# Enigmatisms/NeRF

Hardware: AMD Instinct MI355X
Metric: rays/s (64+128 samples), 800x800 (higher is better)
Workload: dtype bf16

## Files before the change

include/nerf_amd.h:

```cpp
#ifndef NERF_AMD_H
#define NERF_AMD_H

#include <stddef.h>
#include <stdint.h>

#ifdef __cplusplus
extern "C" {
#endif

#define NERF_AMD_OK            0
#define NERF_AMD_EINVAL       -1
#define NERF_AMD_EUNSUPPORTED -2
#define NERF_AMD_EHIP         -3

#define NERF_AMD_F32   0
#define NERF_AMD_BF16  1
#define NERF_AMD_BF16_F8 2

#define NERF_AMD_NET_PROPOSAL 0
#define NERF_AMD_NET_MIP      1
#define NERF_AMD_NET_REF      2
#define NERF_AMD_NET_PROPOSAL_128 3
#define NERF_AMD_PROP_W128 0x100
#define NERF_AMD_NET_MIP_128 4
#define NERF_AMD_FINE_W128 0x200

#define NERF_AMD_ACT_RELU     0
#define NERF_AMD_ACT_IDENTITY 1
#define NERF_AMD_ACT_SOFTPLUS 2

const char* nerf_amd_last_error(void);
int         nerf_amd_version(void);
int         nerf_amd_device_info(int* n_cu, int* arch_is_gfx950);

typedef struct nerf_amd_samples {
    int32_t      mode;
    int32_t      S;
    int64_t      M;
    const float* pts;
    int32_t      pts_stride;
    int32_t      z_stride;
    const float* rays;
    const float* z;
    const float* z_base;
    const float* u;
    float        z_jitter;
    int32_t      H, W;
    float        fx, fy;
    float        pose[12];
    int32_t      contract;
    int32_t      ipe;
    float        ipe_radius;
    const float* ipe_dir_norm;
    uint64_t     rng_seed;
    int64_t      rng_ray_offset;
} nerf_amd_samples;

size_t nerf_amd_packed_bytes(int net, int precision);
int    nerf_amd_pack_weights(int net, int precision, const float* const* weights, const float* const* biases,
                             int n_tensors, void* packed, void* stream);

int nerf_amd_proposal_forward(const void* packed, int precision, const nerf_amd_samples* src,
                              float* density, void* stream);
int nerf_amd_mip_forward(const void* packed, int precision, const nerf_amd_samples* src,
                         float* rgbo, void* stream);

int nerf_amd_mip_forward_composite(const void* packed, int precision, const nerf_amd_samples* src, int white_bkg,
                                   float near, float far, float* rgb, float* depth, float* weights, void* stream);

#define NERF_AMD_REF_SRGB 1
int nerf_amd_ref_forward(const void* packed, int precision, const nerf_amd_samples* src, int ref_flags,
                         float* rgbo, float* normal, void* stream);
int nerf_amd_ref_forward_train(const void* packed, int precision, const nerf_amd_samples* src, int ref_flags, const float* bn_noise,
                               float* rgbo, float* normal, void* stream);


int nerf_amd_positional_encoding(const float* x, int64_t M, int L, float* out, void* stream);

int nerf_amd_ipe_feature(const float* z, const float* rays, int64_t N, int S, int L, float r, const float* dir_norm,
                         float* feat, float* mu, float* mu_t, void* stream);
int nerf_amd_ipe_feature_contracted(const float* z, const float* rays, int64_t N, int S, int L, float r, const float* dir_norm,
                                    float* feat, float* mu, float* mu_t, void* stream);
int nerf_amd_cone_parameters(const float* z, int64_t N, int S, float r, float* mu_t, float* var_t, float* var_r, void* stream);
int nerf_amd_dirs_norm(const float* rays, int64_t N, float* out, void* stream);

int nerf_amd_generate_rays(const float* pose_host, int H, int W, float fx, float fy, int64_t ray_offset, int64_t N,
                           float* rays, void* stream);

int nerf_amd_length2pts(const float* rays, const float* z, int64_t N, int S, float* out, void* stream);

int nerf_amd_sigma_to_weights(const float* sigma, const float* z, const float* dirs, int64_t N, int S, int act,
                              float* w, void* stream);

int nerf_amd_max_blur(const float* w, int64_t N, int S, float alpha, float* out, void* stream);

int nerf_amd_inverse_sample(const float* w, const float* z, const float* u, int64_t N, int C, int K, int sort,
                            float* z_out, int64_t* below, void* stream);

int nerf_amd_sample_pdf(const float* bins, const float* weights, const float* u, int64_t N, int B, int K, float* samples,
                        int64_t* below, int64_t* above, void* stream);

int nerf_amd_pixel_rays(const float* pose_host, float fx, float fy, const int64_t* coords, int64_t N, float* rays, void* stream);

int nerf_amd_sample_training_rays(const float* rgbs, const int64_t* coords, int64_t n_pixels, const float* pose_host, float fx, float fy,
                                  float near, float far, int64_t N, int C, uint64_t rng_seed, float* pts, float* lengths, float* rgb,
                                  float* rays, void* stream);
int nerf_amd_sample_training_rays_dev(const float* rgbs, const int64_t* coords, int64_t n_pixels, const float* pose_dev, float fx, float fy,
                                      float near, float far, int64_t N, int C, const uint64_t* seed_dev, float* pts, float* lengths,
                                      float* rgb, float* rays, void* stream);
int nerf_amd_philox_uniforms(float* out, int64_t N, int K, uint64_t rng_seed, const uint64_t* seed_dev, void* stream);
#define NERF_AMD_PHILOX_INV 0
#define NERF_AMD_PHILOX_STRAT 1
int nerf_amd_philox_stream(float* out, int64_t N, int K, uint64_t rng_seed, const uint64_t* seed_dev, int64_t ray_offset, int stream_id,
                           void* stream);
int nerf_amd_advance_seed(uint64_t* seed_dev, void* stream);

int nerf_amd_stratified_points(const float* rays, const float* z_base, const float* u, float z_jitter, int64_t N, int S,
                               float* z_out, float* pts, void* stream);

int nerf_amd_resample(const float* density, const float* z, const float* z_base, const float* u_strat, float z_jitter,
                      const float* dirs, int dirs_stride, const float* u_inv, int64_t N, int C, int K,
                      int softplus_density, float blur_alpha, uint64_t rng_seed, int64_t rng_ray_offset,
                      float* z_fine, int64_t* below, float* w_prop, float* z_coarse, void* stream);

int nerf_amd_composite(const float* rgbo, const float* z, int z_stride, const float* dirs, int dirs_stride,
                       int64_t N, int S, int flags, int act, float sigma_shift, float near, float far,
                       const float* normal, const float* cam_dir,
                       float* rgb, float* weights, float* depth, float* normal_img, void* stream);

int nerf_amd_merge_depths(const float* z_fine, const float* z_coarse, int64_t N, int K, int C, float* z_out, void* stream);

int nerf_amd_merge_depths_order(const float* z_fine, const float* z_coarse, const int64_t* f_inds, int64_t N, int K, int C, float* z_out,
                                int64_t* order, int64_t* all_inds, void* stream);

int nerf_amd_coarse_grad_select(const float* grads, const int64_t* sort_inds, int64_t N, int T, int D, int c_pnum, float* out, void* stream);

#define NERF_AMD_DOT_LOSS_WORKSPACE_FLOATS 512
int nerf_amd_weighted_dot_loss(const float* w, const float* a, const float* b, int64_t M, int mode, float scale, float* out, float* workspace, void* stream);
int nerf_amd_weighted_dot_loss_backward(const float* g, const float* w, const float* a, const float* b, int64_t M, int mode, float scale, float* d_w,
                                        float* d_a, float* d_b, void* stream);

#define NERF_AMD_DISTORTION_MAX_S 1024
#define NERF_AMD_DISTORTION_WORKSPACE_FLOATS 4096
int nerf_amd_distortion_loss(const float* w, const float* t, int64_t N, int S, int mode, float scale, float* out, float* workspace, void* stream);
int nerf_amd_distortion_loss_backward(const float* w, const float* t, int64_t N, int S, int mode, float scale, const float* g, float* d_w,
                                      float* d_t, void* stream);

int nerf_amd_mfma_stream(int iters, int workgroups, int mode, float* sink, void* stream);

int nerf_amd_get_bounds(const float* w_prop, const int64_t* below, int64_t N, int C, int K, float* bounds, void* stream);

size_t nerf_amd_train_dump_bytes(int net, int precision, int64_t M);
int nerf_amd_proposal_forward_train(const void* packed, int precision, const nerf_amd_samples* src, float* density, void* dump,
                                    void* stream);
int nerf_amd_mip_forward_train(const void* packed, int precision, const nerf_amd_samples* src, float* rgbo, void* dump, void* stream);
int nerf_amd_train_dump_to_rows(const void* dump, int net, int precision, int64_t M, int layer, int n_features, void* out,
                                void* stream);
int nerf_amd_relu_mask(void* delta, const void* act, int precision, int64_t n, void* stream);
int64_t nerf_amd_relu_mask_bias_partials(int precision, int64_t rows, int cols);
int nerf_amd_relu_mask_bias(void* delta, const void* act, int precision, int64_t rows, int cols, float* col_sum, void* stream);

int64_t nerf_amd_train_dump_rows_mask_partials(void);
int nerf_amd_train_dump_rows_mask(const void* dump, int net, int precision, int64_t M, int layer, int n_features, void* act_out, void* delta,
                                  float* col_sum, void* stream);

int nerf_amd_encode_rows(const float* x, int x_stride, int64_t M, int L, int normalize, int precision, void* out, void* stream);

size_t nerf_amd_packed_backward_bytes(int net, int precision);
int    nerf_amd_pack_weights_backward(int net, int precision, const float* const* weights, int n_tensors, void* packed_bwd, void* stream);
int    nerf_amd_proposal_backward_chain(const void* packed_bwd, int precision, const float* g_density, int64_t M, const void* act_dump,
                                        void* delta_dump, void* stream);
int    nerf_amd_mip_backward_chain(const void* packed_bwd, int precision, const float* g_rgbo, const float* rgbo, int64_t M,
                                   const void* act_dump, void* delta_dump, void* stream);
size_t nerf_amd_weight_grads_workspace_bytes(int net, int precision, int64_t M);
int    nerf_amd_proposal_weight_grads(int precision, int64_t M, const void* act_dump, const void* delta_dump, float* const* d_weights,
                                      float* const* d_biases, void* workspace, void* stream);
int    nerf_amd_mip_weight_grads(int precision, int64_t M, const void* act_dump, const void* delta_dump, const float* const* weights,
                                 const float* const* biases, float* const* d_weights, float* const* d_biases, void* workspace, void* stream);
int    nerf_amd_ref_forward_train_dump(const void* packed, int precision, const nerf_amd_samples* src, int ref_flags, const float* bn_noise,
                                       float* rgbo, float* normal, void* dump, float* aux, void* stream);
int    nerf_amd_ref_forward_train_dump_rng(const void* packed, int precision, const nerf_amd_samples* src, int ref_flags, uint64_t noise_seed,
                                           const uint64_t* noise_seed_dev, float noise_std, float* rgbo, float* normal, void* dump, float* aux,
                                           void* stream);
int    nerf_amd_philox_normal(float* out, int64_t M, uint64_t rng_seed, const uint64_t* seed_dev, float std, int64_t sample_offset, void* stream);
#define NERF_AMD_CONTRACTED 0x100
size_t nerf_amd_density_grad_workspace_bytes(int net, int precision, int64_t M);
int    nerf_amd_density_grad(int net, const void* packed_bwd, int precision, int64_t M, const void* act_dump, const float* x, int x_stride,
                             const float* scale, int scale_stride, float* grad, void* workspace, void* stream);
size_t nerf_amd_ref_backward_workspace_bytes(int precision, int64_t M);
int    nerf_amd_ref_backward(const void* packed_bwd, int precision, int ref_flags, int64_t M, const void* act_dump, const float* aux,
                             const float* dirs, int dir_stride, const float* g_out, int g_stride, const float* ide_table,
                             float* const* d_weights, float* const* d_biases, void* workspace, void* stream);
int    nerf_amd_adam_step(float* const* params, const float* const* grads, float* const* exp_avg, float* const* exp_avg_sq,
                          const int64_t* numel, int n_tensors, float* step, double lr, const double* lr_dev, double beta1, double beta2,
                          double eps, float grad_scale, void* stream);

int nerf_amd_sigma_to_weights_backward(const float* sigma, const float* z, const float* dirs, int64_t N, int S, int act,
                                       const float* d_weights, float* d_sigma, void* stream);
int nerf_amd_composite_backward(const float* rgbo, const float* z, int z_stride, const float* dirs, int dirs_stride, int64_t N, int S,
                                int flags, int act, float sigma_shift, float near, float far, const float* d_rgb,
                                const float* d_weights, const float* d_depth, float* d_rgbo, void* stream);
int nerf_amd_max_blur_backward(const float* weights, const float* d_out, int64_t N, int S, float* d_weights, void* stream);
int nerf_amd_get_bounds_backward(const int64_t* below, const float* d_bounds, int64_t N, int C, int K, float* d_w_prop, void* stream);

size_t nerf_amd_render_workspace_bytes(int64_t N, int n_fine);
int    nerf_amd_render_rays(const void* packed_prop, const void* packed_mip, int precision,
                            const float* rays, const nerf_amd_samples* camera, int64_t ray_offset,
                            const float* z_base, const float* u_strat, const float* u_inv, int64_t N, int n_fine,
                            float near, float far, int white_bkg,
                            float* rgb, float* depth, float* weights, void* workspace, void* stream);

size_t nerf_amd_render_ref_workspace_bytes(int64_t N, int n_fine);
int    nerf_amd_render_rays_ref(const void* packed_prop, const void* packed_ref, int precision, int ref_flags, const float* rays,
                                const nerf_amd_samples* camera, int64_t ray_offset, const float* z_base, const float* u_strat,
                                const float* u_inv, int64_t N, int n_fine, float near, float far, int white_bkg, const float* cam_dir,
                                float* rgb, float* depth, float* normal_img, void* workspace, void* stream);

size_t nerf_amd_gemm_workspace_bytes(int64_t M, int64_t N, int64_t P);
// ... 31 lines not shown
```

nerf_amd/_lib.py:

```python
import ctypes as C
import os

import torch

_HERE = os.path.dirname(os.path.abspath(__file__))
LIB_PATH = os.environ.get("NERF_AMD_LIB") or os.path.join(_HERE, "libnerf_amd.so")

F32, BF16 = 0, 1
BF16_F8 = 2
EXPECTED_VERSION = 125
NET_PROPOSAL, NET_MIP, NET_REF, NET_PROPOSAL_128, NET_MIP_128 = 0, 1, 2, 3, 4
FINE_W128 = 0x200
PROP_W128 = 0x100
ACT_RELU, ACT_IDENTITY, ACT_SOFTPLUS = 0, 1, 2

c_float_p = C.POINTER(C.c_float)
c_void = C.c_void_p
i64 = C.c_int64


class Samples(C.Structure):
    _fields_ = [("mode", C.c_int32), ("S", C.c_int32), ("M", C.c_int64), ("pts", c_void), ("pts_stride", C.c_int32),
                ("z_stride", C.c_int32), ("rays", c_void), ("z", c_void), ("z_base", c_void), ("u", c_void),
                ("z_jitter", C.c_float), ("H", C.c_int32), ("W", C.c_int32), ("fx", C.c_float), ("fy", C.c_float),
                ("pose", C.c_float * 12), ("contract", C.c_int32), ("ipe", C.c_int32), ("ipe_radius", C.c_float),
                ("ipe_dir_norm", c_void), ("rng_seed", C.c_uint64), ("rng_ray_offset", C.c_int64)]


SIGNATURES = {
    "nerf_amd_last_error": (C.c_char_p, []),
    "nerf_amd_version": (C.c_int, []),
    "nerf_amd_device_info": (C.c_int, [C.POINTER(C.c_int), C.POINTER(C.c_int)]),
    "nerf_amd_packed_bytes": (C.c_size_t, [C.c_int, C.c_int]),
    "nerf_amd_pack_weights": (C.c_int, [C.c_int, C.c_int, C.POINTER(c_void), C.POINTER(c_void), C.c_int, c_void, c_void]),
    "nerf_amd_proposal_forward": (C.c_int, [c_void, C.c_int, C.POINTER(Samples), c_void, c_void]),
    "nerf_amd_mip_forward": (C.c_int, [c_void, C.c_int, C.POINTER(Samples), c_void, c_void]),
    "nerf_amd_mip_forward_composite": (C.c_int, [c_void, C.c_int, C.POINTER(Samples), C.c_int, C.c_float, C.c_float, c_void, c_void, c_void,
                                                 c_void]),
    "nerf_amd_ref_forward": (C.c_int, [c_void, C.c_int, C.POINTER(Samples), C.c_int, c_void, c_void, c_void]),
    "nerf_amd_ref_forward_train": (C.c_int, [c_void, C.c_int, C.POINTER(Samples), C.c_int, c_void, c_void, c_void, c_void]),
    "nerf_amd_positional_encoding": (C.c_int, [c_void, i64, C.c_int, c_void, c_void]),
    "nerf_amd_ipe_feature": (C.c_int, [c_void, c_void, i64, C.c_int, C.c_int, C.c_float, c_void, c_void, c_void, c_void, c_void]),
    "nerf_amd_ipe_feature_contracted": (C.c_int, [c_void, c_void, i64, C.c_int, C.c_int, C.c_float, c_void, c_void, c_void, c_void, c_void]),
    "nerf_amd_cone_parameters": (C.c_int, [c_void, i64, C.c_int, C.c_float, c_void, c_void, c_void, c_void]),
    "nerf_amd_dirs_norm": (C.c_int, [c_void, i64, c_void, c_void]),
    "nerf_amd_generate_rays": (C.c_int, [c_float_p, C.c_int, C.c_int, C.c_float, C.c_float, i64, i64, c_void, c_void]),
    "nerf_amd_length2pts": (C.c_int, [c_void, c_void, i64, C.c_int, c_void, c_void]),
    "nerf_amd_sigma_to_weights": (C.c_int, [c_void, c_void, c_void, i64, C.c_int, C.c_int, c_void, c_void]),
    "nerf_amd_max_blur": (C.c_int, [c_void, i64, C.c_int, C.c_float, c_void, c_void]),
    "nerf_amd_inverse_sample": (C.c_int, [c_void, c_void, c_void, i64, C.c_int, C.c_int, C.c_int, c_void, c_void, c_void]),
    "nerf_amd_sample_pdf": (C.c_int, [c_void, c_void, c_void, i64, C.c_int, C.c_int, c_void, c_void, c_void, c_void]),
    "nerf_amd_pixel_rays": (C.c_int, [c_float_p, C.c_float, C.c_float, c_void, i64, c_void, c_void]),
    "nerf_amd_sample_training_rays": (C.c_int, [c_void, c_void, i64, c_float_p, C.c_float, C.c_float, C.c_float, C.c_float, i64, C.c_int, C.c_uint64,
                                               c_void, c_void, c_void, c_void, c_void]),
    "nerf_amd_sample_training_rays_dev": (C.c_int, [c_void, c_void, i64, c_void, C.c_float, C.c_float, C.c_float, C.c_float, i64, C.c_int, c_void,
                                                   c_void, c_void, c_void, c_void, c_void]),
    "nerf_amd_philox_uniforms": (C.c_int, [c_void, i64, C.c_int, C.c_uint64, c_void, c_void]),
    "nerf_amd_philox_stream": (C.c_int, [c_void, i64, C.c_int, C.c_uint64, c_void, i64, C.c_int, c_void]),
    "nerf_amd_advance_seed": (C.c_int, [c_void, c_void]),
    "nerf_amd_stratified_points": (C.c_int, [c_void, c_void, c_void, C.c_float, i64, C.c_int, c_void, c_void, c_void]),
    "nerf_amd_resample": (C.c_int, [c_void, c_void, c_void, c_void, C.c_float, c_void, C.c_int, c_void, i64, C.c_int,
                                    C.c_int, C.c_int, C.c_float, C.c_uint64, i64, c_void, c_void, c_void, c_void, c_void]),
    "nerf_amd_composite": (C.c_int, [c_void, c_void, C.c_int, c_void, C.c_int, i64, C.c_int, C.c_int, C.c_int, C.c_float, C.c_float,
                                     C.c_float, c_void, c_void, c_void, c_void, c_void, c_void, c_void]),
    "nerf_amd_train_dump_rows_mask_partials": (i64, []),
    "nerf_amd_train_dump_rows_mask": (C.c_int, [c_void, C.c_int, C.c_int, i64, C.c_int, C.c_int, c_void, c_void, c_void, c_void]),
    "nerf_amd_render_ref_workspace_bytes": (C.c_size_t, [i64, C.c_int]),
    "nerf_amd_render_rays_ref": (C.c_int, [c_void, c_void, C.c_int, C.c_int, c_void, C.POINTER(Samples), i64, c_void, c_void, c_void, i64, C.c_int,
                                          C.c_float, C.c_float, C.c_int, c_void, c_void, c_void, c_void, c_void, c_void]),
    "nerf_amd_encode_rows": (C.c_int, [c_void, C.c_int, i64, C.c_int, C.c_int, C.c_int, c_void, c_void]),
    "nerf_amd_merge_depths": (C.c_int, [c_void, c_void, i64, C.c_int, C.c_int, c_void, c_void]),
    "nerf_amd_merge_depths_order": (C.c_int, [c_void, c_void, c_void, i64, C.c_int, C.c_int, c_void, c_void, c_void, c_void]),
    "nerf_amd_coarse_grad_select": (C.c_int, [c_void, c_void, i64, C.c_int, C.c_int, C.c_int, c_void, c_void]),
    "nerf_amd_mfma_stream": (C.c_int, [C.c_int, C.c_int, C.c_int, c_void, c_void]),
    "nerf_amd_weighted_dot_loss": (C.c_int, [c_void, c_void, c_void, i64, C.c_int, C.c_float, c_void, c_void, c_void]),
    "nerf_amd_weighted_dot_loss_backward": (C.c_int, [c_void, c_void, c_void, c_void, i64, C.c_int, C.c_float, c_void, c_void, c_void, c_void]),
    "nerf_amd_distortion_loss": (C.c_int, [c_void, c_void, i64, C.c_int, C.c_int, C.c_float, c_void, c_void, c_void]),
    "nerf_amd_distortion_loss_backward": (C.c_int, [c_void, c_void, i64, C.c_int, C.c_int, C.c_float, c_void, c_void, c_void, c_void]),
    "nerf_amd_get_bounds": (C.c_int, [c_void, c_void, i64, C.c_int, C.c_int, c_void, c_void]),
    "nerf_amd_train_dump_bytes": (C.c_size_t, [C.c_int, C.c_int, i64]),
    "nerf_amd_proposal_forward_train": (C.c_int, [c_void, C.c_int, C.POINTER(Samples), c_void, c_void, c_void]),
    "nerf_amd_mip_forward_train": (C.c_int, [c_void, C.c_int, C.POINTER(Samples), c_void, c_void, c_void]),
    "nerf_amd_train_dump_to_rows": (C.c_int, [c_void, C.c_int, C.c_int, i64, C.c_int, C.c_int, c_void, c_void]),
    "nerf_amd_relu_mask": (C.c_int, [c_void, c_void, C.c_int, i64, c_void]),
    "nerf_amd_relu_mask_bias_partials": (i64, [C.c_int, i64, C.c_int]),
    "nerf_amd_relu_mask_bias": (C.c_int, [c_void, c_void, C.c_int, i64, C.c_int, c_void, c_void]),
    "nerf_amd_packed_backward_bytes": (C.c_size_t, [C.c_int, C.c_int]),
    "nerf_amd_pack_weights_backward": (C.c_int, [C.c_int, C.c_int, C.POINTER(c_void), C.c_int, c_void, c_void]),
    "nerf_amd_proposal_backward_chain": (C.c_int, [c_void, C.c_int, c_void, i64, c_void, c_void, c_void]),
    "nerf_amd_mip_backward_chain": (C.c_int, [c_void, C.c_int, c_void, c_void, i64, c_void, c_void, c_void]),
    "nerf_amd_weight_grads_workspace_bytes": (C.c_size_t, [C.c_int, C.c_int, i64]),
    "nerf_amd_proposal_weight_grads": (C.c_int, [C.c_int, i64, c_void, c_void, C.POINTER(c_void), C.POINTER(c_void), c_void, c_void]),
    "nerf_amd_mip_weight_grads": (C.c_int, [C.c_int, i64, c_void, c_void, C.POINTER(c_void), C.POINTER(c_void), C.POINTER(c_void),
                                           C.POINTER(c_void), c_void, c_void]),
    "nerf_amd_ref_forward_train_dump": (C.c_int, [c_void, C.c_int, C.POINTER(Samples), C.c_int, c_void, c_void, c_void, c_void, c_void, c_void]),
    "nerf_amd_ref_forward_train_dump_rng": (C.c_int, [c_void, C.c_int, C.POINTER(Samples), C.c_int, C.c_uint64, c_void, C.c_float, c_void, c_void, c_void,
                                                      c_void, c_void]),
    "nerf_amd_philox_normal": (C.c_int, [c_void, i64, C.c_uint64, c_void, C.c_float, i64, c_void]),
    "nerf_amd_density_grad_workspace_bytes": (C.c_size_t, [C.c_int, C.c_int, i64]),
    "nerf_amd_density_grad": (C.c_int, [C.c_int, c_void, C.c_int, i64, c_void, c_void, C.c_int, c_void, C.c_int, c_void, c_void, c_void]),
    "nerf_amd_ref_backward_workspace_bytes": (C.c_size_t, [C.c_int, i64]),
    "nerf_amd_ref_backward": (C.c_int, [c_void, C.c_int, C.c_int, i64, c_void, c_void, c_void, C.c_int, c_void, C.c_int, c_void, C.POINTER(c_void),
                                       C.POINTER(c_void), c_void, c_void]),
    "nerf_amd_adam_step": (C.c_int, [C.POINTER(c_void), C.POINTER(c_void), C.POINTER(c_void), C.POINTER(c_void), C.POINTER(i64), C.c_int, c_void,
                                    C.c_double, c_void, C.c_double, C.c_double, C.c_double, C.c_float, c_void]),
    "nerf_amd_sigma_to_weights_backward": (C.c_int, [c_void, c_void, c_void, i64, C.c_int, C.c_int, c_void, c_void, c_void]),
    "nerf_amd_composite_backward": (C.c_int, [c_void, c_void, C.c_int, c_void, C.c_int, i64, C.c_int, C.c_int, C.c_int, C.c_float, C.c_float,
                                              C.c_float, c_void, c_void, c_void, c_void, c_void]),
    "nerf_amd_max_blur_backward": (C.c_int, [c_void, c_void, i64, C.c_int, c_void, c_void]),
    "nerf_amd_get_bounds_backward": (C.c_int, [c_void, c_void, i64, C.c_int, C.c_int, c_void, c_void]),
    "nerf_amd_render_workspace_bytes": (C.c_size_t, [i64, C.c_int]),
    "nerf_amd_render_rays": (C.c_int, [c_void, c_void, C.c_int, c_void, C.POINTER(Samples), i64, c_void, c_void, c_void, i64,
                                       C.c_int, C.c_float, C.c_float, C.c_int, c_void, c_void, c_void, c_void, c_void]),
    "nerf_amd_gemm_workspace_bytes": (C.c_size_t, [i64, i64, i64]),
    "nerf_amd_gemm": (C.c_int, [C.c_int, i64, i64, i64, c_void, i64, i64, c_void, i64, i64, c_void, i64, c_void, C.c_int, c_void, i64, c_void, c_void]),
    "nerf_amd_sigmoid_backward": (C.c_int, [c_void, i64, c_void, i64, i64, C.c_int, c_void, i64, c_void]),
    "nerf_amd_ref_dir_inputs": (C.c_int, [c_void, i64, c_void, i64, i64, C.c_int, c_void, c_void, i64, c_void, c_void]),
    "nerf_amd_ref_dir_inputs_backward": (C.c_int, [c_void, i64, c_void, i64, i64, C.c_int, c_void, c_void, i64, c_void, i64, c_void, i64, c_void]),
    "nerf_amd_ref_combine": (C.c_int, [c_void, i64, c_void, i64, i64, C.c_int, c_void, c_void]),
    "nerf_amd_ref_combine_backward": (C.c_int, [c_void, i64, c_void, i64, c_void, i64, i64, C.c_int, c_void, i64, c_void, i64, c_void]),
    "nerf_amd_positional_encoding_backward": (C.c_int, [c_void, i64, c_void, i64, i64, C.c_int, C.c_int, c_void, c_void]),
    "nerf_amd_contract_positions": (C.c_int, [c_void, i64, i64, c_void, i64, c_void, c_void]),
    "nerf_amd_add_rows": (C.c_int, [c_void, i64, c_void, i64, i64, C.c_int, c_void]),
    "nerf_amd_rows_gemm": (C.c_int, [i64, i64, i64, c_void, i64, c_void, i64, i64, c_void, C.c_int, c_void, i64, C.c_int, c_void]),
    "nerf_amd_rows_to_bf16": (C.c_int, [c_void, i64, i64, i64, C.c_int, C.c_int, c_void, i64, c_void]),
}


def _load():
    if not os.path.exists(LIB_PATH):
        raise ImportError(
            "nerf_amd: %s is missing. Build it with `python -c 'import __graft_entry__ as g; g.build()'` "
            "(or `make -C nerf_amd/csrc`). There is no CPU/torch fallback." % LIB_PATH)
    lib = C.CDLL(LIB_PATH)
    for name, (res, args) in SIGNATURES.items():
        fn = getattr(lib, name)
        fn.restype = res
        fn.argtypes = args
    got = lib.nerf_amd_version()
    if got != EXPECTED_VERSION and not os.environ.get("NERF_AMD_LIB"):
        raise ImportError("nerf_amd: %s is ABI version %d, this package expects %d -- rebuild it (`make -C nerf_amd/csrc`)" % (LIB_PATH, got, EXPECTED_VERSION))
    return lib


lib = _load()


class NerfAmdError(RuntimeError):
    pass


def check(rc: int, what: str = ""):
    if rc != 0:
        msg = lib.nerf_amd_last_error()
        raise NerfAmdError("%s failed (%d): %s" % (what or "nerf_amd call", rc, msg.decode() if msg else "?"))
```

nerf_amd/csrc/capi.hip:

```cpp
#include <hip/hip_runtime.h>
#include <stdio.h>
#include <string.h>

#include "../../include/nerf_amd.h"
#include "mlp_layout.h"

int mlp_launch_proposal(const void*, int, const nerf_amd_samples&, float*, hipStream_t);
int mlp_launch_proposal128(const void*, int, const nerf_amd_samples&, float*, hipStream_t);
int mlp_launch_mip(const void*, int, const nerf_amd_samples&, float*, hipStream_t);
int mlp_launch_mip128(const void*, int, const nerf_amd_samples&, float*, hipStream_t);
int mlp_launch_mip_composite(const void*, int, const nerf_amd_samples&, float*, float*, float*, int, float, float, hipStream_t);
int mlp_launch_ref(const void*, int, const nerf_amd_samples&, float*, float*, const float*, int, hipStream_t);
size_t mlp_train_layer_stride(int, int64_t);
size_t mlp_train_mask_stride(int, int64_t);
int mlp_launch_proposal_train(const void*, int, const nerf_amd_samples&, float*, void*, hipStream_t);
int mlp_launch_mip_train(const void*, int, const nerf_amd_samples&, float*, void*, hipStream_t);
int sk_frag_to_rows(const void*, int, int64_t, int, int64_t, void*, hipStream_t);
int sk_relu_mask(void*, const void*, int, int64_t, hipStream_t);
int sk_merge_sorted(const float*, const float*, int64_t, int, int, float*, hipStream_t);
int sk_merge_sorted_order(const float*, const float*, const int64_t*, int64_t, int, int, float*, int64_t*, int64_t*, hipStream_t);
int sk_coarse_grad_select(const float*, const int64_t*, int64_t, int, int, int, float*, hipStream_t);
int pack_mfma_stream(int, int, int, float*, hipStream_t);
int sk_weighted_dot_loss(const float*, const float*, const float*, int64_t, int, float, float*, float*, hipStream_t);
int sk_weighted_dot_loss_backward(const float*, const float*, const float*, const float*, int64_t, int, float, float*, float*, float*, hipStream_t);
int sk_distortion_loss(const float*, const float*, int64_t, int, int, float, float*, float*, hipStream_t);
int sk_distortion_loss_backward(const float*, const float*, int64_t, int, int, float, const float*, float*, float*, hipStream_t);
int sk_encode_rows(const float*, int, int64_t, int, int, int, void*, hipStream_t);
int sk_frag_rows_mask_blocks();
int sk_frag_rows_mask(const void*, int, int64_t, int, int64_t, void*, void*, float*, hipStream_t);
int sk_relu_mask_bias(void*, const void*, int, int64_t, int, float*, hipStream_t);
int pack_ref(int, const float* const*, const float* const*, void*, hipStream_t);
int pack_proposal_bwd(int, const float* const*, void*, hipStream_t);
int pack_mip_bwd(int, const float* const*, void*, hipStream_t);
int pack_ref_bwd(int, const float* const*, void*, hipStream_t);
int mlp_launch_ref_train(const void*, int, const nerf_amd_samples&, float*, float*, const float*, void*, float*, int, hipStream_t, unsigned long long, const unsigned long long*, float);
size_t bwd_density_grad_workspace_bytes(int, int64_t);
int bwd_density_grad(int, const void*, int, int64_t, const void*, const float*, int, const float*, int, float*, void*, hipStream_t, int);
size_t bwd_ref_workspace_bytes(int, int64_t);
int bwd_ref_backward(const void*, int, int64_t, const void*, const float*, const float*, int, const float*, int, const float*, float* const*,
                     float* const*, void*, int, hipStream_t);
int bwd_launch_prop_chain(const void*, int, const float*, int64_t, const void*, void*, hipStream_t);
int bwd_launch_mip_chain(const void*, int, const float*, const float*, int64_t, const void*, void*, hipStream_t);
size_t bwd_wgrad_workspace_bytes(int, int, int64_t);
int bwd_prop_weight_grads(int, int64_t, const void*, const void*, float* const*, float* const*, void*, hipStream_t);
int bwd_mip_weight_grads(int, int64_t, const void*, const void*, const float* const*, const float* const*, float* const*, float* const*, void*,
                         hipStream_t);
int bwd_launch_adam(float* const*, const float* const*, float* const*, float* const*, const long long*, int, float*, double, const double*, double,
                    double, double, float, hipStream_t);
int pack_proposal(int, const float* const*, const float* const*, void*, hipStream_t);
int pack_proposal128(int, const float* const*, const float* const*, void*, hipStream_t);
int pack_mip128(int, const float* const*, const float* const*, void*, hipStream_t);
int pack_mip(int, const float* const*, const float* const*, void*, hipStream_t);
int sk_positional_encoding(const float*, int64_t, int, float*, hipStream_t);
int sk_ipe_feature(const float*, const float*, int64_t, int, int, float, const float*, float*, float*, float*, int, hipStream_t);
int sk_dirs_norm(const float*, int64_t, float*, hipStream_t);
int sk_dirs_norm_scratch(const float*, int64_t, float*, void*, hipStream_t);
int sk_train_sampler(const float*, const int64_t*, int64_t, const float*, const float*, float, float, float, float, int64_t, int, uint64_t, const uint64_t*,
                     float*, float*, float*, float*, hipStream_t);
int sk_philox_uniforms(float*, int64_t, int, uint64_t, const uint64_t*, int64_t, int, hipStream_t);
int sk_philox_normal(float*, int64_t, uint64_t, const uint64_t*, float, int64_t, hipStream_t);
size_t gk_gemm_workspace_bytes(int64_t, int64_t, int64_t);
int gk_gemm(int, int64_t, int64_t, int64_t, const float*, int64_t, int64_t, const float*, int64_t, int64_t, float*, int64_t, const float*, int, const float*, int64_t,
            void*, hipStream_t);
int gk_sigmoid_backward(const float*, int64_t, const float*, int64_t, int64_t, int, float*, int64_t, hipStream_t);
int gr_dir_inputs(const float*, int64_t, const float*, int64_t, int64_t, int, const float*, float*, int64_t, float*, hipStream_t);
int gr_dir_inputs_backward(const float*, int64_t, const float*, int64_t, int64_t, int, const float*, const float*, int64_t, const float*, int64_t, float*, int64_t,
                           hipStream_t);
int gr_combine(const float*, int64_t, const float*, int64_t, int64_t, int, float*, hipStream_t);
int gr_combine_backward(const float*, int64_t, const float*, int64_t, const float*, int64_t, int64_t, int, float*, int64_t, float*, int64_t, hipStream_t);
int gr_pe_backward(const float*, int64_t, const float*, int64_t, int64_t, int, int, float*, hipStream_t);
int gr_add_rows(float*, int64_t, const float*, int64_t, int64_t, int, hipStream_t);
int gr_contract(const float*, int64_t, int64_t, const float*, int64_t, float*, hipStream_t);
int rg_rows_gemm(int64_t, int64_t, int64_t, const void*, int64_t, const void*, int64_t, int64_t, const float*, int, void*, int64_t, int, hipStream_t);
int rg_rows_to_bf16(const float*, int64_t, int64_t, int64_t, int, int, void*, int64_t, hipStream_t);
int sk_advance_seed(uint64_t*, hipStream_t);
int sk_cone_parameters(const float*, int64_t, int, float, float*, float*, float*, hipStream_t);
int sk_generate_rays(const float*, int, int, float, float, int64_t, int64_t, float*, hipStream_t);
int sk_length2pts(const float*, const float*, int64_t, int, float*, hipStream_t);
int sk_sigma_to_weights(const float*, const float*, const float*, int64_t, int, int, float*, hipStream_t);
int sk_max_blur(const float*, int64_t, int, float, float*, hipStream_t);
int sk_inverse_sample(const float*, const float*, const float*, int64_t, int, int, int, int, float*, int64_t*, int64_t*, hipStream_t);
int sk_pixel_rays(const float*, float, float, const int64_t*, int64_t, float*, hipStream_t);
int sk_stratified_points(const float*, const float*, const float*, float, int64_t, int, float*, float*, hipStream_t);
int sk_resample(const float*, const float*, const float*, const float*, float, const float*, int, const float*, int64_t, int,
                int, int, float, uint64_t, int64_t, float*, int64_t*, float*, float*, hipStream_t);
int sk_composite(const float*, const float*, int, const float*, int, int64_t, int, int, int, float, float, float, const float*,
                 const float*, float*, float*, float*, float*, hipStream_t);
int sk_get_bounds(const float*, const int64_t*, int64_t, int, int, float*, hipStream_t);
int sk_weights_backward(const float*, int, int, const float*, int, const float*, int, int64_t, int, int, int, float, const float*, const float*,
                        const float*, const float*, int, float, float, float*, int, int, float*, hipStream_t);
int sk_max_blur_backward(const float*, const float*, int64_t, int, float*, hipStream_t);
int sk_get_bounds_backward(const int64_t*, const float*, int64_t, int, int, float*, hipStream_t);

namespace {
thread_local char g_err[512] = "";

int fail(int code, const char* fmt, const char* a = "") {
    snprintf(g_err, sizeof(g_err), fmt, a);
    return code;
}
int hip_status(int e, const char* where) {
    if (e == 0) return NERF_AMD_OK;
    snprintf(g_err, sizeof(g_err), "%s: HIP error %d (%s)", where, e, hipGetErrorString((hipError_t)e));
    return NERF_AMD_EHIP;
}
inline hipStream_t S(void* s) { return reinterpret_cast<hipStream_t>(s); }

int check_samples(const nerf_amd_samples* s, bool need_dir) {
    if (!s) return fail(NERF_AMD_EINVAL, "samples descriptor is NULL");
    if (s->M < 0) return fail(NERF_AMD_EINVAL, "negative sample count");
    if (s->mode == 0) {
        if (!s->pts && s->M) return fail(NERF_AMD_EINVAL, "mode 0 needs pts");
        if (s->pts_stride < (need_dir ? 6 : 3)) return fail(NERF_AMD_EINVAL, "pts_stride too small for this network");
    } else if (s->mode == 1 || s->mode == 2) {
        if (s->S <= 0) return fail(NERF_AMD_EINVAL, "S must be positive");
        if (s->mode == 1 && !s->rays && s->M) return fail(NERF_AMD_EINVAL, "mode 1 needs rays");
        if (s->mode == 2 && (s->H <= 0 || s->W <= 0)) return fail(NERF_AMD_EINVAL, "mode 2 needs H, W");
        if (!s->z && !s->z_base && s->M) return fail(NERF_AMD_EINVAL, "need z, or z_base (with u, or without: in-kernel uniforms from rng_seed)");
    } else {
        return fail(NERF_AMD_EINVAL, "unknown sample mode");
    }
    if (s->ipe) {
        if (!need_dir) return fail(NERF_AMD_EUNSUPPORTED, "integrated PE is wired for the MipNeRF kernel only");
        if (s->mode != 1 || !s->z || s->z_stride < s->S + 1) return fail(NERF_AMD_EINVAL, "integrated PE needs mode 1 with S+1 depths per ray (z, z_stride > S)");
        if (!s->ipe_dir_norm || !(s->ipe_radius > 0.0f)) return fail(NERF_AMD_EINVAL, "integrated PE needs ipe_dir_norm (device) and a positive ipe_radius");
    }
    return NERF_AMD_OK;
}
bool bad_prec(int p) { return p != NERF_AMD_F32 && p != NERF_AMD_BF16; }
int check_distortion(int64_t N, int Sn, int mode) {
    if (N < 0) return fail(NERF_AMD_EINVAL, "negative ray count");
    if (mode != 0 && mode != 1) return fail(NERF_AMD_EINVAL, "unknown mode (0: Regularizer, 1: Mip-NeRF 360 L_dist)");
    if (Sn < 2 || Sn > NERF_AMD_DISTORTION_MAX_S) return fail(NERF_AMD_EINVAL, "bad size (S must be 2..1024 depths per row: a ray's rows live in LDS)");
    return NERF_AMD_OK;
}
}

extern "C" {

const char* nerf_amd_last_error(void) { return g_err; }
int nerf_amd_version(void) { return 125; }

int nerf_amd_device_info(int* n_cu, int* arch_is_gfx950) {
    int dev = 0;
    hipDeviceProp_t p;
    int e = (int)hipGetDevice(&dev);
    if (!e) e = (int)hipGetDeviceProperties(&p, dev);
    if (e) return hip_status(e, "nerf_amd_device_info");
    if (n_cu) *n_cu = p.multiProcessorCount;
    if (arch_is_gfx950) *arch_is_gfx950 = strncmp(p.gcnArchName, "gfx950", 6) == 0;
    return NERF_AMD_OK;
}

size_t nerf_amd_packed_bytes(int net, int precision) {
    if (bad_prec(precision)) return 0;
    if (net == NERF_AMD_NET_PROPOSAL) return PropLayout::packed_bytes(precision);
    if (net == NERF_AMD_NET_MIP) return MipLayout::packed_bytes(precision);
    if (net == NERF_AMD_NET_REF) return RefLayout::packed_bytes(precision);
    if (net == NERF_AMD_NET_PROPOSAL_128) return PropLayout128::packed_bytes(precision);
    if (net == NERF_AMD_NET_MIP_128) return MipLayout128::packed_bytes(precision);
    return 0;
}
static int launch_mip_any(int flags, const void* packed, int precision, const nerf_amd_samples& s, float* rgbo, hipStream_t st) {
    return (flags & NERF_AMD_FINE_W128) ? mlp_launch_mip128(packed, precision, s, rgbo, st) : mlp_launch_mip(packed, precision, s, rgbo, st);
}
static int launch_proposal_any(int flags, const void* packed, int precision, const nerf_amd_samples& s, float* density, hipStream_t st) {
    return (flags & NERF_AMD_PROP_W128) ? mlp_launch_proposal128(packed, precision, s, density, st) : mlp_launch_proposal(packed, precision, s, density, st);
}

int nerf_amd_pack_weights(int net, int precision, const float* const* weights, const float* const* biases, int n_tensors,
                          void* packed, void* stream) {
    if (bad_prec(precision)) return fail(NERF_AMD_EINVAL, "unknown precision");
    if (!weights || !biases || !packed) return fail(NERF_AMD_EINVAL, "NULL argument");
    const int want = (net == NERF_AMD_NET_PROPOSAL || net == NERF_AMD_NET_PROPOSAL_128) ? 5
                     : ((net == NERF_AMD_NET_MIP || net == NERF_AMD_NET_MIP_128) ? 11 : (net == NERF_AMD_NET_REF ? 20 : -1));
    if (want < 0) return fail(NERF_AMD_EINVAL, "unknown network");
    if (n_tensors != want) return fail(NERF_AMD_EINVAL, "wrong number of weight tensors for this network");
    for (int i = 0; i < want; ++i)
        if (!weights[i] || !biases[i]) return fail(NERF_AMD_EINVAL, "NULL weight or bias tensor");
    const int e = net == NERF_AMD_NET_PROPOSAL ? pack_proposal(precision, weights, biases, packed, S(stream))
                  : net == NERF_AMD_NET_PROPOSAL_128 ? pack_proposal128(precision, weights, biases, packed, S(stream))
                  : net == NERF_AMD_NET_MIP_128 ? pack_mip128(precision, weights, biases, packed, S(stream))
                  : (net == NERF_AMD_NET_MIP ? pack_mip(precision, weights, biases, packed, S(stream))
                                             : pack_ref(precision, weights, biases, packed, S(stream)));
    return hip_status(e, "nerf_amd_pack_weights");
}

int nerf_amd_proposal_forward(const void* packed, int precision, const nerf_amd_samples* src, float* density, void* stream) {
    const int lflags = precision & ~0xff;
    precision &= 0xff;
    if (bad_prec(precision) || (lflags & ~NERF_AMD_PROP_W128)) return fail(NERF_AMD_EINVAL, "unknown precision");
    if (int c = check_samples(src, false)) return c;
    if (src->M == 0) return NERF_AMD_OK;
    if (!packed || !density) return fail(NERF_AMD_EINVAL, "NULL argument");
    return hip_status(launch_proposal_any(lflags, packed, precision, *src, density, S(stream)), "nerf_amd_proposal_forward");
}

int nerf_amd_mip_forward(const void* packed, int precision, const nerf_amd_samples* src, float* rgbo, void* stream) {
    const int lflags = precision & ~0xff;
    precision &= 0xff;
    if (bad_prec(precision) || (lflags & ~NERF_AMD_FINE_W128)) return fail(NERF_AMD_EINVAL, "unknown precision");
    if (int c = check_samples(src, true)) return c;
    if (src->M == 0) return NERF_AMD_OK;
    if (!packed || !rgbo) return fail(NERF_AMD_EINVAL, "NULL argument");
    if ((lflags & NERF_AMD_FINE_W128) && src->ipe) return fail(NERF_AMD_EINVAL, "the 128-wide fine layout has no integrated-PE kernel: pack the network 256-wide");
    return hip_status(launch_mip_any(lflags, packed, precision, *src, rgbo, S(stream)), "nerf_amd_mip_forward");
}

int nerf_amd_mip_forward_composite(const void* packed, int precision, const nerf_amd_samples* src, int white_bkg, float near,
                                   float far, float* rgb, float* depth, float* weights, void* stream) {
    const int lflags = precision & ~0xff;
    precision &= 0xff;
    if (bad_prec(precision) || (lflags & ~NERF_AMD_FINE_W128)) return fail(NERF_AMD_EINVAL, "unknown precision");
    if (lflags & NERF_AMD_FINE_W128)
        return fail(NERF_AMD_EUNSUPPORTED, "the 128-wide fine layout has no fused-compositing kernel: use nerf_amd_mip_forward + nerf_amd_composite");
    if (int c = check_samples(src, true)) return c;
    if (src->mode != 1 || !src->z) return fail(NERF_AMD_EUNSUPPORTED, "fused compositing needs mode 1 (rays + z)");
    if (src->ipe) return fail(NERF_AMD_EUNSUPPORTED, "integrated PE: use nerf_amd_mip_forward + nerf_amd_composite");
    if (src->S != 32 && src->S != 64 && src->S != 128) return fail(NERF_AMD_EUNSUPPORTED, "fused compositing needs S in {32, 64, 128}");
    if (src->M == 0) return NERF_AMD_OK;
    if (!packed || !rgb) return fail(NERF_AMD_EINVAL, "NULL argument");
    return hip_status(mlp_launch_mip_composite(packed, precision, *src, rgb, depth, weights, white_bkg, near, far, S(stream)),
                      "nerf_amd_mip_forward_composite");
}

static bool bad_ref_flags(int f) { return (f & ~NERF_AMD_REF_SRGB) != 0; }
int nerf_amd_ref_forward(const void* packed, int precision, const nerf_amd_samples* src, int ref_flags, float* rgbo, float* normal, void* stream) {
    if (bad_prec(precision) || bad_ref_flags(ref_flags)) return fail(NERF_AMD_EINVAL, "unknown precision or ref_flags");
    if (int c = check_samples(src, true)) return c;
    if (src->M == 0) return NERF_AMD_OK;
    if (!packed || !rgbo) return fail(NERF_AMD_EINVAL, "NULL argument");
    return hip_status(mlp_launch_ref(packed, precision, *src, rgbo, normal, nullptr, ref_flags, S(stream)), "nerf_amd_ref_forward");
}
int nerf_amd_ref_forward_train(const void* packed, int precision, const nerf_amd_samples* src, int ref_flags, const float* bn_noise, float* rgbo,
                               float* normal, void* stream) {
    if (bad_prec(precision) || bad_ref_flags(ref_flags)) return fail(NERF_AMD_EINVAL, "unknown precision or ref_flags");
    if (int c = check_samples(src, true)) return c;
    if (src->M == 0) return NERF_AMD_OK;
    if (!packed || !rgbo || !bn_noise) return fail(NERF_AMD_EINVAL, "NULL argument");
    return hip_status(mlp_launch_ref(packed, precision, *src, rgbo, normal, bn_noise, ref_flags, S(stream)), "nerf_amd_ref_forward_train");
}

int nerf_amd_positional_encoding(const float* x, int64_t M, int L, float* out, void* stream) {
    if (M < 0 || L < 1 || L > 24) return fail(NERF_AMD_EINVAL, "bad M or L");
    if (M && (!x || !out)) return fail(NERF_AMD_EINVAL, "NULL argument");
    return hip_status(sk_positional_encoding(x, M, L, out, S(stream)), "nerf_amd_positional_encoding");
}

int nerf_amd_ipe_feature(const float* z, const float* rays, int64_t N, int Sn, int L, float r, const float* dir_norm, float* feat, float* mu,
                         float* mu_t, void* stream) {
    if (N < 0 || Sn < 0 || L < 1 || L > 15) return fail(NERF_AMD_EINVAL, "bad size or L (1..15)");
    if (N * Sn && (!z || !rays || !dir_norm || !feat)) return fail(NERF_AMD_EINVAL, "NULL argument");
    const float r2 = (float)((double)r * (double)r);
    return hip_status(sk_ipe_feature(z, rays, N, Sn, L, r2, dir_norm, feat, mu, mu_t, 0, S(stream)), "nerf_amd_ipe_feature");
}
int nerf_amd_ipe_feature_contracted(const float* z, const float* rays, int64_t N, int Sn, int L, float r, const float* dir_norm, float* feat, float* mu,
                                    float* mu_t, void* stream) {
    if (N < 0 || Sn < 0 || L < 1 || L > 15) return fail(NERF_AMD_EINVAL, "bad size or L (1..15)");
    if (N * Sn && (!z || !rays || !dir_norm || !feat)) return fail(NERF_AMD_EINVAL, "NULL argument");
    const float r2 = (float)((double)r * (double)r);
    return hip_status(sk_ipe_feature(z, rays, N, Sn, L, r2, dir_norm, feat, mu, mu_t, 1, S(stream)), "nerf_amd_ipe_feature_contracted");
}
int nerf_amd_cone_parameters(const float* z, int64_t N, int Sn, float r, float* mu_t, float* var_t, float* var_r, void* stream) {
    if (N < 0 || Sn < 0) return fail(NERF_AMD_EINVAL, "negative size");
    if (N * Sn && (!z || !mu_t || !var_t || !var_r)) return fail(NERF_AMD_EINVAL, "NULL argument");
    return hip_status(sk_cone_parameters(z, N, Sn, (float)((double)r * (double)r), mu_t, var_t, var_r, S(stream)), "nerf_amd_cone_parameters");
}
int nerf_amd_dirs_norm(const float* rays, int64_t N, float* out, void* stream) {
    if (N < 0 || !out || (N && !rays)) return fail(NERF_AMD_EINVAL, "bad argument");
    return hip_status(sk_dirs_norm(rays, N, out, S(stream)), "nerf_amd_dirs_norm");
}

int nerf_amd_generate_rays(const float* pose_host, int H, int W, float fx, float fy, int64_t ray_offset, int64_t N, float* rays,
                           void* stream) {
    if (!pose_host || !rays || H <= 0 || W <= 0) return fail(NERF_AMD_EINVAL, "bad argument");
    if (ray_offset < 0 || N < 0 || ray_offset + N > (int64_t)H * W) return fail(NERF_AMD_EINVAL, "ray range outside the image");
    return hip_status(sk_generate_rays(pose_host, H, W, fx, fy, ray_offset, N, rays, S(stream)), "nerf_amd_generate_rays");
}

int nerf_amd_length2pts(const float* rays, const float* z, int64_t N, int Sn, float* out, void* stream) {
    if (N < 0 || Sn < 0) return fail(NERF_AMD_EINVAL, "negative size");
    if (N * Sn && (!rays || !z || !out)) return fail(NERF_AMD_EINVAL, "NULL argument");
    return hip_status(sk_length2pts(rays, z, N, Sn, out, S(stream)), "nerf_amd_length2pts");
}

int nerf_amd_sigma_to_weights(const float* sigma, const float* z, const float* dirs, int64_t N, int Sn, int act, float* w,
                              void* stream) {
    if (N < 0 || Sn < 0 || act < 0 || act > 2) return fail(NERF_AMD_EINVAL, "bad size or activation");
    if (N * Sn && (!sigma || !z || !w)) return fail(NERF_AMD_EINVAL, "NULL argument");
    return hip_status(sk_sigma_to_weights(sigma, z, dirs, N, Sn, act, w, S(stream)), "nerf_amd_sigma_to_weights");
}

int nerf_amd_max_blur(const float* w, int64_t N, int Sn, float alpha, float* out, void* stream) {
    if (N < 0 || Sn < 0) return fail(NERF_AMD_EINVAL, "negative size");
    if (N * Sn && (!w || !out)) return fail(NERF_AMD_EINVAL, "NULL argument");
    return hip_status(sk_max_blur(w, N, Sn, alpha, out, S(stream)), "nerf_amd_max_blur");
}

int nerf_amd_inverse_sample(const float* w, const float* z, const float* u, int64_t N, int C, int K, int sort, float* z_out,
                            int64_t* below, void* stream) {
    if (N < 0 || C < 3 || C > 256 || K < 1 || K > 1024) return fail(NERF_AMD_EINVAL, "need 3 <= C <= 256 and 1 <= K <= 1024");
    if (N && (!w || !z || !u || !z_out)) return fail(NERF_AMD_EINVAL, "NULL argument");
    return hip_status(sk_inverse_sample(w, z, u, N, C, K, sort, 0, z_out, below, nullptr, S(stream)), "nerf_amd_inverse_sample");
}

int nerf_amd_sample_pdf(const float* bins, const float* weights, const float* u, int64_t N, int B, int K, float* samples,
                        int64_t* below, int64_t* above, void* stream) {
    if (N < 0 || B < 2 || B > 256 || K < 1 || K > 1024) return fail(NERF_AMD_EINVAL, "need 2 <= B <= 256 and 1 <= K <= 1024");
    if (N && (!bins || !weights || !u || !samples)) return fail(NERF_AMD_EINVAL, "NULL argument");
    return hip_status(sk_inverse_sample(weights, bins, u, N, B, K, 0, 1, samples, below, above, S(stream)), "nerf_amd_sample_pdf");
}

int nerf_amd_pixel_rays(const float* pose_host, float fx, float fy, const int64_t* coords, int64_t N, float* rays, void* stream) {
    if (!pose_host || N < 0 || (N && (!coords || !rays))) return fail(NERF_AMD_EINVAL, "bad argument");
    return hip_status(sk_pixel_rays(pose_host, fx, fy, coords, N, rays, S(stream)), "nerf_amd_pixel_rays");
}

int nerf_amd_sample_training_rays(const float* rgbs, const int64_t* coords, int64_t n_pixels, const float* pose_host, float fx, float fy,
                                  float near, float far, int64_t N, int C, uint64_t rng_seed, float* pts, float* lengths, float* rgb, float* rays,
                                  void* stream) {
    if (N < 0 || C < 0 || n_pixels < 1) return fail(NERF_AMD_EINVAL, "bad size");
    if (!pose_host || (N && (!rgbs || !coords || !rgb || !rays))) return fail(NERF_AMD_EINVAL, "NULL argument");
    if ((pts == nullptr) != (lengths == nullptr) || (pts && C < 1)) return fail(NERF_AMD_EINVAL, "pts and lengths go together (C >= 1)");
    return hip_status(sk_train_sampler(rgbs, coords, n_pixels, pose_host, nullptr, fx, fy, near, far, N, C, rng_seed, nullptr, pts, lengths, rgb, rays, S(stream)),
                      "nerf_amd_sample_training_rays");
}
int nerf_amd_sample_training_rays_dev(const float* rgbs, const int64_t* coords, int64_t n_pixels, const float* pose_dev, float fx, float fy,
                                      float near, float far, int64_t N, int C, const uint64_t* seed_dev, float* pts, float* lengths, float* rgb,
                                      float* rays, void* stream) {
    if (N < 0 || C < 0 || n_pixels < 1) return fail(NERF_AMD_EINVAL, "bad size");
    if (!pose_dev || !seed_dev || (N && (!rgbs || !coords || !rgb || !rays))) return fail(NERF_AMD_EINVAL, "NULL argument");
    if ((pts == nullptr) != (lengths == nullptr) || (pts && C < 1)) return fail(NERF_AMD_EINVAL, "pts and lengths go together (C >= 1)");
    return hip_status(sk_train_sampler(rgbs, coords, n_pixels, nullptr, pose_dev, fx, fy, near, far, N, C, 0, seed_dev, pts, lengths, rgb, rays, S(stream)),
                      "nerf_amd_sample_training_rays_dev");
}
int nerf_amd_philox_uniforms(float* out, int64_t N, int K, uint64_t rng_seed, const uint64_t* seed_dev, void* stream) {
    if (N < 0 || K < 0) return fail(NERF_AMD_EINVAL, "negative size");
    if (N * K && !out) return fail(NERF_AMD_EINVAL, "NULL argument");
    return hip_status(sk_philox_uniforms(out, N, K, rng_seed, seed_dev, 0, 0, S(stream)), "nerf_amd_philox_uniforms");
}
int nerf_amd_philox_stream(float* out, int64_t N, int K, uint64_t rng_seed, const uint64_t* seed_dev, int64_t ray_offset, int stream_id, void* stream) {
    if (N < 0 || K < 0 || ray_offset < 0) return fail(NERF_AMD_EINVAL, "negative size");
    if (stream_id != NERF_AMD_PHILOX_INV && stream_id != NERF_AMD_PHILOX_STRAT) return fail(NERF_AMD_EINVAL, "unknown stream_id");
    if (stream_id == NERF_AMD_PHILOX_STRAT && K > 64) return fail(NERF_AMD_EINVAL, "the stratified stream has 64 slots per ray");
    if (N * K && !out) return fail(NERF_AMD_EINVAL, "NULL argument");
    return hip_status(sk_philox_uniforms(out, N, K, rng_seed, seed_dev, ray_offset, stream_id == NERF_AMD_PHILOX_STRAT, S(stream)), "nerf_amd_philox_stream");
}
int nerf_amd_advance_seed(uint64_t* seed_dev, void* stream) {
    if (!seed_dev) return fail(NERF_AMD_EINVAL, "NULL argument");
    return hip_status(sk_advance_seed(seed_dev, S(stream)), "nerf_amd_advance_seed");
}

int nerf_amd_stratified_points(const float* rays, const float* z_base, const float* u, float z_jitter, int64_t N, int Sn,
                               float* z_out, float* pts, void* stream) {
    if (N < 0 || Sn < 0) return fail(NERF_AMD_EINVAL, "negative size");
    if (N * Sn && (!z_base || !u || !z_out || (pts && !rays))) return fail(NERF_AMD_EINVAL, "NULL argument");
    return hip_status(sk_stratified_points(rays, z_base, u, z_jitter, N, Sn, z_out, pts, S(stream)), "nerf_amd_stratified_points");
}

int nerf_amd_resample(const float* density, const float* z, const float* z_base, const float* u_strat, float z_jitter,
                      const float* dirs, int dirs_stride, const float* u_inv, int64_t N, int C, int K, int softplus_density,
// ... 155 lines not shown
    if (net == NERF_AMD_NET_MIP) return MipBwdLayout::packed_bytes(precision);
    if (net == NERF_AMD_NET_REF) return RefBwdLayout::packed_bytes(precision);
    return 0;
}
int nerf_amd_pack_weights_backward(int net, int precision, const float* const* weights, int n_tensors, void* packed_bwd, void* stream) {
    if (bad_prec(precision)) return fail(NERF_AMD_EINVAL, "unknown precision");
    if (!weights || !packed_bwd) return fail(NERF_AMD_EINVAL, "NULL argument");
    const int want = (net == NERF_AMD_NET_PROPOSAL || net == NERF_AMD_NET_PROPOSAL_128) ? 5 : (net == NERF_AMD_NET_MIP ? 11 : (net == NERF_AMD_NET_REF ? 20 : -1));
    if (want < 0) return fail(NERF_AMD_EINVAL, "unknown network");
    if (n_tensors != want) return fail(NERF_AMD_EINVAL, "wrong number of weight tensors for this network");
    for (int i = 0; i < want; ++i)
        if (!weights[i]) return fail(NERF_AMD_EINVAL, "NULL weight tensor");
    const int e = net == NERF_AMD_NET_PROPOSAL ? pack_proposal_bwd(precision, weights, packed_bwd, S(stream))
                  : (net == NERF_AMD_NET_MIP ? pack_mip_bwd(precision, weights, packed_bwd, S(stream)) : pack_ref_bwd(precision, weights, packed_bwd, S(stream)));
    return hip_status(e, "nerf_amd_pack_weights_backward");
}
int nerf_amd_proposal_backward_chain(const void* packed_bwd, int precision, const float* g_density, int64_t M, const void* act_dump,
                                     void* delta_dump, void* stream) {
    if (bad_train_prec(precision) || M < 0) return fail(NERF_AMD_EINVAL, "bad precision or size");
    if (M == 0) return NERF_AMD_OK;
    if (!packed_bwd || !g_density || !act_dump || !delta_dump) return fail(NERF_AMD_EINVAL, "NULL argument");
    return hip_status(bwd_launch_prop_chain(packed_bwd, precision, g_density, M, act_dump, delta_dump, S(stream)), "nerf_amd_proposal_backward_chain");
}
int nerf_amd_mip_backward_chain(const void* packed_bwd, int precision, const float* g_rgbo, const float* rgbo, int64_t M, const void* act_dump,
                                void* delta_dump, void* stream) {
    if (bad_train_prec(precision) || M < 0) return fail(NERF_AMD_EINVAL, "bad precision or size");
    if (M == 0) return NERF_AMD_OK;
    if (!packed_bwd || !g_rgbo || !rgbo || !act_dump || !delta_dump) return fail(NERF_AMD_EINVAL, "NULL argument");
    return hip_status(bwd_launch_mip_chain(packed_bwd, precision, g_rgbo, rgbo, M, act_dump, delta_dump, S(stream)), "nerf_amd_mip_backward_chain");
}
size_t nerf_amd_weight_grads_workspace_bytes(int net, int precision, int64_t M) {
    if (bad_train_prec(precision, net) || M < 0) return 0;
    return bwd_wgrad_workspace_bytes(net, precision == NERF_AMD_BF16_F8 ? NERF_AMD_BF16 : precision, M);
}
int nerf_amd_proposal_weight_grads(int precision, int64_t M, const void* act_dump, const void* delta_dump, float* const* d_weights,
                                   float* const* d_biases, void* workspace, void* stream) {
    if (bad_train_prec(precision) || M < 0) return fail(NERF_AMD_EINVAL, "bad precision or size");
    if (!d_weights || !d_biases) return fail(NERF_AMD_EINVAL, "NULL argument");
    for (int i = 0; i < 5; ++i)
        if (!d_weights[i] || !d_biases[i]) return fail(NERF_AMD_EINVAL, "NULL gradient tensor");
    if (M == 0) return fail(NERF_AMD_EINVAL, "no samples (the caller zero-fills the gradients of an empty batch)");
    if (!act_dump || !delta_dump || !workspace) return fail(NERF_AMD_EINVAL, "NULL argument");
    return hip_status(bwd_prop_weight_grads(precision, M, act_dump, delta_dump, d_weights, d_biases, workspace, S(stream)), "nerf_amd_proposal_weight_grads");
}
int nerf_amd_mip_weight_grads(int precision, int64_t M, const void* act_dump, const void* delta_dump, const float* const* weights,
                              const float* const* biases, float* const* d_weights, float* const* d_biases, void* workspace, void* stream) {
    if (bad_train_prec(precision) || M < 0) return fail(NERF_AMD_EINVAL, "bad precision or size");
    if (!weights || !biases || !d_weights || !d_biases) return fail(NERF_AMD_EINVAL, "NULL argument");
    for (int i = 0; i < 11; ++i)
        if (!weights[i] || !biases[i] || !d_weights[i] || !d_biases[i]) return fail(NERF_AMD_EINVAL, "NULL tensor");
    if (M == 0) return fail(NERF_AMD_EINVAL, "no samples (the caller zero-fills the gradients of an empty batch)");
    if (!act_dump || !delta_dump || !workspace) return fail(NERF_AMD_EINVAL, "NULL argument");
    return hip_status(bwd_mip_weight_grads(precision, M, act_dump, delta_dump, weights, biases, d_weights, d_biases, workspace, S(stream)),
                      "nerf_amd_mip_weight_grads");
}
int nerf_amd_ref_forward_train_dump(const void* packed, int precision, const nerf_amd_samples* src, int ref_flags, const float* bn_noise, float* rgbo,
                                    float* normal, void* dump, float* aux, void* stream) {
    if (bad_prec(precision) || bad_ref_flags(ref_flags)) return fail(NERF_AMD_EINVAL, "unknown precision or ref_flags");
    if (int c = check_samples(src, true)) return c;
    if (src->M == 0) return NERF_AMD_OK;
    if (!packed || !rgbo || !dump || !aux) return fail(NERF_AMD_EINVAL, "NULL argument");
    return hip_status(mlp_launch_ref_train(packed, precision, *src, rgbo, normal, bn_noise, dump, aux, ref_flags, S(stream), 0, nullptr, 0.0f), "nerf_amd_ref_forward_train_dump");
}
int nerf_amd_ref_forward_train_dump_rng(const void* packed, int precision, const nerf_amd_samples* src, int ref_flags, uint64_t noise_seed,
                                        const uint64_t* noise_seed_dev, float noise_std, float* rgbo, float* normal, void* dump, float* aux, void* stream) {
    if (bad_prec(precision) || bad_ref_flags(ref_flags)) return fail(NERF_AMD_EINVAL, "unknown precision or ref_flags");
    if (!(noise_std >= 0.0f)) return fail(NERF_AMD_EINVAL, "noise_std must be >= 0");
    if (int c = check_samples(src, true)) return c;
    if (src->M == 0) return NERF_AMD_OK;
    if (!packed || !rgbo || !dump || !aux) return fail(NERF_AMD_EINVAL, "NULL argument");
    return hip_status(mlp_launch_ref_train(packed, precision, *src, rgbo, normal, nullptr, dump, aux, ref_flags, S(stream), noise_seed,
                                           reinterpret_cast<const unsigned long long*>(noise_seed_dev), noise_std), "nerf_amd_ref_forward_train_dump_rng");
}
int nerf_amd_philox_normal(float* out, int64_t M, uint64_t rng_seed, const uint64_t* seed_dev, float std, int64_t sample_offset, void* stream) {
    if (M < 0 || sample_offset < 0 || !(std >= 0.0f)) return fail(NERF_AMD_EINVAL, "negative size or std");
    if (M && !out) return fail(NERF_AMD_EINVAL, "NULL argument");
    return hip_status(sk_philox_normal(out, M, rng_seed, seed_dev, std, sample_offset, S(stream)), "nerf_amd_philox_normal");
}
size_t nerf_amd_density_grad_workspace_bytes(int net, int precision, int64_t M) {
    if (bad_prec(precision) || M < 0 || (net != NERF_AMD_NET_PROPOSAL && net != NERF_AMD_NET_REF)) return 0;
    return bwd_density_grad_workspace_bytes(precision, M);
}
int nerf_amd_density_grad(int net, const void* packed_bwd, int precision, int64_t M, const void* act_dump, const float* x, int x_stride,
                          const float* scale, int scale_stride, float* grad, void* workspace, void* stream) {
    const int contract = (net & NERF_AMD_CONTRACTED) ? 1 : 0;
    net &= ~NERF_AMD_CONTRACTED;
    if (bad_prec(precision) || M < 0 || x_stride < 3) return fail(NERF_AMD_EINVAL, "bad precision, size or stride");
    if (net != NERF_AMD_NET_PROPOSAL && net != NERF_AMD_NET_REF) return fail(NERF_AMD_EUNSUPPORTED, "density gradients exist for the proposal and Ref-NeRF networks");
    if (M == 0) return NERF_AMD_OK;
    if (!packed_bwd || !act_dump || !x || !grad || !workspace) return fail(NERF_AMD_EINVAL, "NULL argument");
    return hip_status(bwd_density_grad(net, packed_bwd, precision, M, act_dump, x, x_stride, scale, scale_stride, grad, workspace, S(stream), contract), "nerf_amd_density_grad");
}
size_t nerf_amd_ref_backward_workspace_bytes(int precision, int64_t M) {
    if (bad_prec(precision) || M < 0) return 0;
    return bwd_ref_workspace_bytes(precision, M);
}
int nerf_amd_ref_backward(const void* packed_bwd, int precision, int ref_flags, int64_t M, const void* act_dump, const float* aux, const float* dirs,
                          int dir_stride, const float* g_out, int g_stride, const float* ide_table, float* const* d_weights, float* const* d_biases,
                          void* workspace, void* stream) {
    if (bad_prec(precision) || bad_ref_flags(ref_flags) || M < 0 || dir_stride < 3 || g_stride < 7) return fail(NERF_AMD_EINVAL, "bad precision, flags, size or stride");
    if (!d_weights || !d_biases) return fail(NERF_AMD_EINVAL, "NULL argument");
    for (int i = 0; i < 20; ++i)
        if (!d_weights[i] || !d_biases[i]) return fail(NERF_AMD_EINVAL, "NULL gradient tensor");
    if (M == 0) return fail(NERF_AMD_EINVAL, "no samples (the caller zero-fills the gradients of an empty batch)");
    if (!packed_bwd || !act_dump || !aux || !dirs || !g_out || !ide_table || !workspace) return fail(NERF_AMD_EINVAL, "NULL argument");
    return hip_status(bwd_ref_backward(packed_bwd, precision, M, act_dump, aux, dirs, dir_stride, g_out, g_stride, ide_table, d_weights, d_biases, workspace,
                                       ref_flags, S(stream)), "nerf_amd_ref_backward");
}

int nerf_amd_adam_step(float* const* params, const float* const* grads, float* const* exp_avg, float* const* exp_avg_sq, const int64_t* numel,
                       int n_tensors, float* step, double lr, const double* lr_dev, double beta1, double beta2, double eps, float grad_scale,
                       void* stream) {
    if (n_tensors < 0 || (n_tensors && (!params || !grads || !exp_avg || !exp_avg_sq || !numel)) || !step) return fail(NERF_AMD_EINVAL, "NULL argument");
    for (int i = 0; i < n_tensors; ++i)
        if (numel[i] < 0 || (numel[i] && (!params[i] || !grads[i] || !exp_avg[i] || !exp_avg_sq[i]))) return fail(NERF_AMD_EINVAL, "NULL tensor");
    static_assert(sizeof(long long) == sizeof(int64_t), "int64");
    return hip_status(bwd_launch_adam(params, grads, exp_avg, exp_avg_sq, reinterpret_cast<const long long*>(numel), n_tensors, step, lr, lr_dev,
                                      beta1, beta2, eps, grad_scale, S(stream)), "nerf_amd_adam_step");
}

int nerf_amd_sigma_to_weights_backward(const float* sigma, const float* z, const float* dirs, int64_t N, int Sn, int act,
                                       const float* d_weights, float* d_sigma, void* stream) {
    if (N < 0 || Sn < 1 || Sn > 1024) return fail(NERF_AMD_EINVAL, "bad size (S must be 1..1024)");
    if (N && (!sigma || !z || !d_weights || !d_sigma)) return fail(NERF_AMD_EINVAL, "NULL argument");
    return hip_status(sk_weights_backward(sigma, 1, 0, z, Sn, dirs, 3, N, Sn, dirs ? 1 : 0, act, 0.0f, nullptr, nullptr, d_weights, nullptr, 0, 0.0f,
                                          1.0f, d_sigma, 1, 0, nullptr, S(stream)), "nerf_amd_sigma_to_weights_backward");
}
int nerf_amd_composite_backward(const float* rgbo, const float* z, int z_stride, const float* dirs, int dirs_stride, int64_t N, int Sn,
                                int flags, int act, float sigma_shift, float near, float far, const float* d_rgb,
                                const float* d_weights, const float* d_depth, float* d_rgbo, void* stream) {
    if (N < 0 || Sn < 1 || Sn > 1024 || z_stride < Sn) return fail(NERF_AMD_EINVAL, "bad size (S must be 1..1024)");
    if (N && (!rgbo || !z || !dirs || !d_rgbo)) return fail(NERF_AMD_EINVAL, "NULL argument");
    if (N && !d_rgb) return fail(NERF_AMD_EINVAL, "d_rgb is required (pass zeros when only the weights carry a gradient)");
    return hip_status(sk_weights_backward(rgbo, 4, 3, z, z_stride, dirs, dirs_stride, N, Sn, flags & 1, act, sigma_shift, rgbo, d_rgb, d_weights,
                                          d_depth, (flags >> 1) & 1, near, far, d_rgbo, 4, 3, d_rgbo, S(stream)), "nerf_amd_composite_backward");
}
int nerf_amd_max_blur_backward(const float* weights, const float* d_out, int64_t N, int Sn, float* d_weights, void* stream) {
    if (N < 0 || Sn < 1) return fail(NERF_AMD_EINVAL, "bad size");
    if (N && (!weights || !d_out || !d_weights)) return fail(NERF_AMD_EINVAL, "NULL argument");
    return hip_status(sk_max_blur_backward(weights, d_out, N, Sn, d_weights, S(stream)), "nerf_amd_max_blur_backward");
}
int nerf_amd_get_bounds_backward(const int64_t* below, const float* d_bounds, int64_t N, int C, int K, float* d_w_prop, void* stream) {
    if (N < 0 || C < 1 || C > 4096 || K < 2 || K > 2048) return fail(NERF_AMD_EINVAL, "bad size (C <= 4096, 2 <= K <= 2048)");
    if (N && (!below || !d_bounds || !d_w_prop)) return fail(NERF_AMD_EINVAL, "NULL argument");
    return hip_status(sk_get_bounds_backward(below, d_bounds, N, C, K, d_w_prop, S(stream)), "nerf_amd_get_bounds_backward");
}

size_t nerf_amd_render_workspace_bytes(int64_t N, int n_fine) {
    if (N < 0 || n_fine < 1) return 0;
    const size_t a = ((size_t)N * 64 * 4 + 255) & ~(size_t)255;
    const size_t b = ((size_t)N * (n_fine + 1) * 4 + 255) & ~(size_t)255;
    const size_t c = ((size_t)N * n_fine * 16 + 255) & ~(size_t)255;
    const size_t d = ((size_t)N * 24 + 255) & ~(size_t)255;
    return a + b + c + d + 512;
}

int nerf_amd_render_rays(const void* packed_prop, const void* packed_mip, int precision, const float* rays,
                         const nerf_amd_samples* camera, int64_t ray_offset, const float* z_base, const float* u_strat,
                         const float* u_inv, int64_t N, int n_fine, float near, float far, int white_bkg, float* rgb,
                         float* depth, float* weights, void* workspace, void* stream) {
    const int lflags = precision & ~0xff;
    precision &= 0xff;
    if (bad_prec(precision) || (lflags & ~(NERF_AMD_PROP_W128 | NERF_AMD_FINE_W128))) return fail(NERF_AMD_EINVAL, "unknown precision");
    if ((lflags & NERF_AMD_FINE_W128) && camera && camera->ipe) return fail(NERF_AMD_EINVAL, "the 128-wide fine layout has no integrated-PE kernel: pack the network 256-wide");
    if (N < 0 || n_fine < 1 || n_fine > 1023) return fail(NERF_AMD_EINVAL, "bad N or n_fine");
    if (N == 0) return NERF_AMD_OK;
    if (!packed_prop || !packed_mip || !z_base || !rgb || !workspace) return fail(NERF_AMD_EINVAL, "NULL argument");
    if ((u_strat == nullptr) != (u_inv == nullptr)) return fail(NERF_AMD_EINVAL, "u_strat and u_inv are both given or both NULL (in-kernel uniforms)");
    if (!u_strat && !camera) return fail(NERF_AMD_EINVAL, "in-kernel uniforms need the descriptor (rng_seed, rng_ray_offset)");
    if (!rays && !camera) return fail(NERF_AMD_EINVAL, "need rays or camera");
    const uint64_t seed = camera ? camera->rng_seed : 0;
    const int64_t ray0 = camera ? camera->rng_ray_offset : 0;
    constexpr int C = 64;
    char* ws = reinterpret_cast<char*>((reinterpret_cast<uintptr_t>(workspace) + 255) & ~(uintptr_t)255);
    float* density = reinterpret_cast<float*>(ws);
    ws += ((size_t)N * C * 4 + 255) & ~(size_t)255;
    float* z_fine = reinterpret_cast<float*>(ws);
    ws += ((size_t)N * (n_fine + 1) * 4 + 255) & ~(size_t)255;
    float* rgbo = reinterpret_cast<float*>(ws);
    ws += ((size_t)N * n_fine * 16 + 255) & ~(size_t)255;
    hipStream_t st = S(stream);
    if (!rays) {
        if (camera->H <= 0 || camera->W <= 0 || ray_offset < 0 || ray_offset + N > (int64_t)camera->H * camera->W)
            return fail(NERF_AMD_EINVAL, "ray range outside the camera image");
        float* gen = reinterpret_cast<float*>(ws);
        if (int e = sk_generate_rays(camera->pose, camera->H, camera->W, camera->fx, camera->fy, ray_offset, N, gen, st))
            return hip_status(e, "ray generation");
        rays = gen;
    }
    ws += ((size_t)N * 24 + 255) & ~(size_t)255;
    float* dir_norm = reinterpret_cast<float*>(ws);
    const bool ipe = camera && camera->ipe;
    if (ipe) {
        if (!(camera->ipe_radius > 0.0f)) return fail(NERF_AMD_EINVAL, "integrated PE needs a positive ipe_radius");
        if (camera->ipe_dir_norm) dir_norm = const_cast<float*>(camera->ipe_dir_norm);
        else if (int e = (N >= 8) ? sk_dirs_norm_scratch(rays, N, dir_norm, density, st) : sk_dirs_norm(rays, N, dir_norm, st))
            return hip_status(e, "direction norm");
    }
    const float jitter = (far - near) / (float)n_fine;

    nerf_amd_samples sc{};
    sc.mode = 1; sc.rays = rays; sc.S = C; sc.M = N * C; sc.z = nullptr; sc.z_base = z_base; sc.u = u_strat;
    sc.z_jitter = jitter; sc.z_stride = C;
    sc.contract = camera ? camera->contract : 0;
    sc.rng_seed = seed; sc.rng_ray_offset = ray0;
    if (int e = launch_proposal_any(lflags, packed_prop, precision, sc, density, st)) return hip_status(e, "proposal MLP");
    if (int e = sk_resample(density, nullptr, z_base, u_strat, jitter, rays + 3, 6, u_inv, N, C, n_fine + 1, 0, 0.01f, seed, ray0, z_fine,
                            nullptr, nullptr, nullptr, st)) return hip_status(e, "resample");
    nerf_amd_samples sf{};
    sf.mode = 1; sf.rays = rays; sf.S = n_fine; sf.M = N * n_fine; sf.z = z_fine; sf.z_stride = n_fine + 1;
    sf.contract = sc.contract;
    if (ipe) { sf.ipe = 1; sf.ipe_radius = camera->ipe_radius; sf.ipe_dir_norm = dir_norm; }
    if (int e = launch_mip_any(lflags, packed_mip, precision, sf, rgbo, st)) return hip_status(e, "fine MLP");
    const int flags = 1 | (white_bkg ? 2 : 0);
    if (int e = sk_composite(rgbo, z_fine, n_fine + 1, rays + 3, 6, N, n_fine, flags, NERF_AMD_ACT_RELU, 0.0f, near, far, nullptr,
                             nullptr, rgb, weights, depth, nullptr, st)) return hip_status(e, "composite");
    return NERF_AMD_OK;
}

static size_t ref_ws_part(size_t bytes) { return (bytes + 255) & ~(size_t)255; }
size_t nerf_amd_render_ref_workspace_bytes(int64_t N, int n_fine) {
    if (N < 0 || n_fine < 1) return 0;
    const size_t n = (size_t)N, S = (size_t)n_fine + 64;
    return ref_ws_part(n * 64 * 4) * 2 + ref_ws_part(n * (n_fine + 1) * 4) + ref_ws_part(n * S * 4) + ref_ws_part(n * S * 16) + ref_ws_part(n * S * 12) +
           n * 24 + 256;
}

int nerf_amd_render_rays_ref(const void* packed_prop, const void* packed_ref, int precision, int ref_flags, const float* rays,
                             const nerf_amd_samples* camera, int64_t ray_offset, const float* z_base, const float* u_strat,
                             const float* u_inv, int64_t N, int n_fine, float near, float far, int white_bkg, const float* cam_dir,
                             float* rgb, float* depth, float* normal_img, void* workspace, void* stream) {
    const int lflags = precision & ~0xff;
    precision &= 0xff;
    if (bad_prec(precision) || (lflags & ~NERF_AMD_PROP_W128) || bad_ref_flags(ref_flags)) return fail(NERF_AMD_EINVAL, "unknown precision or ref_flags");
    if (N < 0 || n_fine < 1 || n_fine > 1023) return fail(NERF_AMD_EINVAL, "bad N or n_fine");
    if (N == 0) return NERF_AMD_OK;
    if (!packed_prop || !packed_ref || !z_base || !rgb || !workspace) return fail(NERF_AMD_EINVAL, "NULL argument");
    if ((u_strat == nullptr) != (u_inv == nullptr)) return fail(NERF_AMD_EINVAL, "u_strat and u_inv are both given or both NULL (in-kernel uniforms)");
    if (!u_strat && !camera) return fail(NERF_AMD_EINVAL, "in-kernel uniforms need the descriptor (rng_seed, rng_ray_offset)");
    if (!rays && !camera) return fail(NERF_AMD_EINVAL, "need rays or camera");
    const uint64_t seed = camera ? camera->rng_seed : 0;
    const int64_t ray0 = camera ? camera->rng_ray_offset : 0;
    if ((normal_img != nullptr) != (cam_dir != nullptr)) return fail(NERF_AMD_EINVAL, "normal_img and cam_dir go together");
    const int contract = camera ? camera->contract : 0;
    constexpr int C = 64;
    const int S_all = n_fine + C;
    char* ws = reinterpret_cast<char*>((reinterpret_cast<uintptr_t>(workspace) + 255) & ~(uintptr_t)255);
    auto take = [&](size_t bytes) { float* p = reinterpret_cast<float*>(ws); ws += ref_ws_part(bytes); return p; };
    float* density = take((size_t)N * C * 4);
    float* z_fine = take((size_t)N * (n_fine + 1) * 4);
    float* z_coarse = take((size_t)N * C * 4);
    float* z_all = take((size_t)N * S_all * 4);
    float* rgbo = take((size_t)N * S_all * 16);
    float* normals = take((size_t)N * S_all * 12);
    hipStream_t st = S(stream);
    if (!rays) {
        if (camera->H <= 0 || camera->W <= 0 || ray_offset < 0 || ray_offset + N > (int64_t)camera->H * camera->W)
            return fail(NERF_AMD_EINVAL, "ray range outside the camera image");
        float* gen = reinterpret_cast<float*>(ws);
        if (int e = sk_generate_rays(camera->pose, camera->H, camera->W, camera->fx, camera->fy, ray_offset, N, gen, st))
            return hip_status(e, "ray generation");
        rays = gen;
    }
    const float jitter = (far - near) / (float)n_fine;
    nerf_amd_samples sc{};
    sc.mode = 1; sc.rays = rays; sc.S = C; sc.M = N * C; sc.z = nullptr; sc.z_base = z_base; sc.u = u_strat;
    sc.z_jitter = jitter; sc.z_stride = C;
    sc.contract = contract;
    sc.rng_seed = seed; sc.rng_ray_offset = ray0;
    if (int e = launch_proposal_any(lflags, packed_prop, precision, sc, density, st)) return hip_status(e, "proposal MLP");
    if (int e = sk_resample(density, nullptr, z_base, u_strat, jitter, rays + 3, 6, u_inv, N, C, n_fine + 1, 0, 0.01f, seed, ray0, z_fine,
                            nullptr, nullptr, z_coarse, st)) return hip_status(e, "resample");
    if (int e = sk_merge_sorted(z_fine, z_coarse, N, n_fine + 1, C, z_all, st)) return hip_status(e, "depth merge");
    nerf_amd_samples sf{};
    sf.mode = 1; sf.rays = rays; sf.S = S_all; sf.M = N * S_all; sf.z = z_all; sf.z_stride = S_all;
    sf.contract = contract;
    if (int e = mlp_launch_ref(packed_ref, precision, sf, rgbo, normal_img ? normals : nullptr, nullptr, ref_flags, st)) return hip_status(e, "Ref-NeRF MLP");
    const int flags = 1 | (white_bkg ? 2 : 0);
    if (int e = sk_composite(rgbo, z_all, S_all, rays + 3, 6, N, S_all, flags, NERF_AMD_ACT_SOFTPLUS, 0.5f, near, far,
                             normal_img ? normals : nullptr, cam_dir, rgb, nullptr, depth, normal_img, st)) return hip_status(e, "composite");
    return NERF_AMD_OK;
}

size_t nerf_amd_gemm_workspace_bytes(int64_t M, int64_t N, int64_t P) {
    if (M <= 0 || N <= 0 || P <= 0) return 0;
    return gk_gemm_workspace_bytes(M, N, P);
}

int nerf_amd_gemm(int precision, int64_t M, int64_t N, int64_t P, const float* A, int64_t a_si, int64_t a_sp, const float* B, int64_t b_sp, int64_t b_sj,
                  float* C, int64_t ldc, const float* bias, int act, const float* mask, int64_t ldm, void* workspace, void* stream) {
    if (precision != NERF_AMD_F32 && precision != NERF_AMD_BF16) return fail(NERF_AMD_EINVAL, "nerf_amd_gemm: precision must be NERF_AMD_F32 or NERF_AMD_BF16");
    if (M < 0 || N < 0 || P < 0 || N > 65535LL * 128) return fail(NERF_AMD_EINVAL, "nerf_amd_gemm: bad size");
    if (M == 0 || N == 0) return 0;
    if (!C || (P && (!A || !B))) return fail(NERF_AMD_EINVAL, "nerf_amd_gemm: NULL argument");
    if ((a_si != 1 && a_sp != 1) || (b_sp != 1 && b_sj != 1)) return fail(NERF_AMD_EINVAL, "nerf_amd_gemm: one stride of each operand must be 1");
    if (ldc < N || (mask && ldm < N)) return fail(NERF_AMD_EINVAL, "nerf_amd_gemm: row stride smaller than N");
    if (act < 0 || act > 2) return fail(NERF_AMD_EINVAL, "nerf_amd_gemm: act must be 0 (none), 1 (ReLU) or 2 (sigmoid)");
    if (gk_gemm_workspace_bytes(M, N, P) && !workspace) return fail(NERF_AMD_EINVAL, "nerf_amd_gemm: this shape needs nerf_amd_gemm_workspace_bytes of workspace");
    return hip_status(gk_gemm(precision == NERF_AMD_BF16, M, N, P, A, a_si, a_sp, B, b_sp, b_sj, C, ldc, bias, act, mask, ldm, workspace, S(stream)), "nerf_amd_gemm");
}

int nerf_amd_sigmoid_backward(const float* g, int64_t g_stride, const float* y, int64_t y_stride, int64_t M, int cols, float* out, int64_t out_stride,
                              void* stream) {
    if (M < 0 || cols < 0) return fail(NERF_AMD_EINVAL, "nerf_amd_sigmoid_backward: bad size");
    if (M * cols && (!g || !y || !out)) return fail(NERF_AMD_EINVAL, "nerf_amd_sigmoid_backward: NULL argument");
    if (g_stride < cols || y_stride < cols || out_stride < cols) return fail(NERF_AMD_EINVAL, "nerf_amd_sigmoid_backward: row stride smaller than cols");
    return hip_status(gk_sigmoid_backward(g, g_stride, y, y_stride, M, cols, out, out_stride, S(stream)), "nerf_amd_sigmoid_backward");
}

int nerf_amd_ref_dir_inputs(const float* heads, int64_t heads_stride, const float* dirs, int64_t dirs_stride, int64_t M, int ide_level, const float* ide_table,
                            float* out, int64_t out_stride, float* normal, void* stream) {
    if (M < 0 || ide_level < 1 || ide_level > 5) return fail(NERF_AMD_EINVAL, "nerf_amd_ref_dir_inputs: bad size / ide_level (1..5)");
    if (M && (!heads || !dirs || !ide_table || !out || !normal)) return fail(NERF_AMD_EINVAL, "nerf_amd_ref_dir_inputs: NULL argument");
    const int T = (1 << ide_level) - 1 + ide_level;
    if (heads_stride < 11 || dirs_stride < 3 || out_stride < 2 * T + 1) return fail(NERF_AMD_EINVAL, "nerf_amd_ref_dir_inputs: row stride too small");
    return hip_status(gr_dir_inputs(heads, heads_stride, dirs, dirs_stride, M, ide_level, ide_table, out, out_stride, normal, S(stream)), "nerf_amd_ref_dir_inputs");
}

int nerf_amd_ref_dir_inputs_backward(const float* heads, int64_t heads_stride, const float* dirs, int64_t dirs_stride, int64_t M, int ide_level,
                                     const float* ide_table, const float* d_out, int64_t d_out_stride, const float* g_normal, int64_t g_normal_stride,
                                     float* d_heads, int64_t d_heads_stride, void* stream) {
    if (M < 0 || ide_level < 1 || ide_level > 5) return fail(NERF_AMD_EINVAL, "nerf_amd_ref_dir_inputs_backward: bad size / ide_level (1..5)");
    if (M && (!heads || !dirs || !ide_table || !d_out || !g_normal || !d_heads)) return fail(NERF_AMD_EINVAL, "nerf_amd_ref_dir_inputs_backward: NULL argument");
    const int T = (1 << ide_level) - 1 + ide_level;
    if (heads_stride < 11 || dirs_stride < 3 || d_out_stride < 2 * T + 1 || g_normal_stride < 3 || d_heads_stride < 11)
        return fail(NERF_AMD_EINVAL, "nerf_amd_ref_dir_inputs_backward: row stride too small");
    return hip_status(gr_dir_inputs_backward(heads, heads_stride, dirs, dirs_stride, M, ide_level, ide_table, d_out, d_out_stride, g_normal, g_normal_stride, d_heads,
                                             d_heads_stride, S(stream)), "nerf_amd_ref_dir_inputs_backward");
}

int nerf_amd_ref_combine(const float* heads, int64_t heads_stride, const float* spec, int64_t spec_stride, int64_t M, int ref_flags, float* rgbo, void* stream) {
    if (M < 0 || bad_ref_flags(ref_flags)) return fail(NERF_AMD_EINVAL, "nerf_amd_ref_combine: bad size / ref_flags");
    if (M && (!heads || !spec || !rgbo)) return fail(NERF_AMD_EINVAL, "nerf_amd_ref_combine: NULL argument");
    if (heads_stride < 11 || spec_stride < 3) return fail(NERF_AMD_EINVAL, "nerf_amd_ref_combine: row stride too small");
    return hip_status(gr_combine(heads, heads_stride, spec, spec_stride, M, (ref_flags & NERF_AMD_REF_SRGB) ? 1 : 0, rgbo, S(stream)), "nerf_amd_ref_combine");
}

int nerf_amd_ref_combine_backward(const float* g_rgbo, int64_t g_stride, const float* heads, int64_t heads_stride, const float* spec, int64_t spec_stride, int64_t M,
                                  int ref_flags, float* d_spec, int64_t d_spec_stride, float* d_heads, int64_t d_heads_stride, void* stream) {
    if (M < 0 || bad_ref_flags(ref_flags)) return fail(NERF_AMD_EINVAL, "nerf_amd_ref_combine_backward: bad size / ref_flags");
    if (M && (!g_rgbo || !heads || !spec || !d_spec || !d_heads)) return fail(NERF_AMD_EINVAL, "nerf_amd_ref_combine_backward: NULL argument");
    if (g_stride < 4 || heads_stride < 11 || spec_stride < 3 || d_spec_stride < 3 || d_heads_stride < 11)
        return fail(NERF_AMD_EINVAL, "nerf_amd_ref_combine_backward: row stride too small");
    return hip_status(gr_combine_backward(g_rgbo, g_stride, heads, heads_stride, spec, spec_stride, M, (ref_flags & NERF_AMD_REF_SRGB) ? 1 : 0, d_spec, d_spec_stride,
                                          d_heads, d_heads_stride, S(stream)), "nerf_amd_ref_combine_backward");
}

int nerf_amd_positional_encoding_backward(const float* d_enc, int64_t d_enc_stride, const float* x, int64_t x_stride, int64_t M, int L, int cat_origin, float* d_x,
                                          void* stream) {
    if (M < 0 || L < 0) return fail(NERF_AMD_EINVAL, "nerf_amd_positional_encoding_backward: bad size");
    if (M && (!d_enc || !x || !d_x)) return fail(NERF_AMD_EINVAL, "nerf_amd_positional_encoding_backward: NULL argument");
    if (d_enc_stride < 6 * L + (cat_origin ? 3 : 0) || x_stride < 3) return fail(NERF_AMD_EINVAL, "nerf_amd_positional_encoding_backward: row stride too small");
    return hip_status(gr_pe_backward(d_enc, d_enc_stride, x, x_stride, M, L, cat_origin ? 1 : 0, d_x, S(stream)), "nerf_amd_positional_encoding_backward");
}

int nerf_amd_contract_positions(const float* x, int64_t x_stride, int64_t M, const float* g, int64_t g_stride, float* out, void* stream) {
    if (M < 0 || x_stride < 3 || (g && g_stride < 3)) return fail(NERF_AMD_EINVAL, "nerf_amd_contract_positions: bad size or stride");
    if (M && (!x || !out)) return fail(NERF_AMD_EINVAL, "nerf_amd_contract_positions: NULL argument");
    return hip_status(gr_contract(x, x_stride, M, g, g_stride, out, S(stream)), "nerf_amd_contract_positions");
}

int nerf_amd_add_rows(float* dst, int64_t dst_stride, const float* src, int64_t src_stride, int64_t M, int cols, void* stream) {
    if (M < 0 || cols < 0) return fail(NERF_AMD_EINVAL, "nerf_amd_add_rows: bad size");
    if (M * cols && (!dst || !src)) return fail(NERF_AMD_EINVAL, "nerf_amd_add_rows: NULL argument");
    if (dst_stride < cols || src_stride < cols) return fail(NERF_AMD_EINVAL, "nerf_amd_add_rows: row stride smaller than cols");
    return hip_status(gr_add_rows(dst, dst_stride, src, src_stride, M, cols, S(stream)), "nerf_amd_add_rows");
// ... 28 lines not shown
```

nerf_amd/csrc/mlp_kernels.hip:

```cpp
#include "mlp_core.h"

namespace {

template <class P, int L, int NKG>
DEVINL void encode(float x, float y, float z, int h, typename P::BReg (&B)[NKG]) {
    if constexpr (P::FAST_PE) {
        float sv[3], cv[3];
        sincos_quadrant(x, sv[0], cv[0]); sincos_quadrant(y, sv[1], cv[1]); sincos_quadrant(z, sv[2], cv[2]);
#pragma unroll
        for (int f = 0; f < L; ++f) {
#pragma unroll
            for (int c = 0; c < 3; ++c) {
                const int q = 3 * f + c;
                P::set(B[q >> 3], q & 7, h ? cv[c] : sv[c]);
                if (f + 1 < L) {
                    const float s2 = 2.0f * sv[c];
                    const float ns = s2 * cv[c];
                    const float nc = __builtin_fmaf(-s2, sv[c], 1.0f);
                    sv[c] = ns; cv[c] = nc;
                }
            }
        }
#pragma unroll
        for (int q = 3 * L; q < 8 * NKG; ++q) {
            const float v = (q == 3 * L) ? (h ? z : x) : ((q == 3 * L + 1) ? (h ? 0.0f : y) : 0.0f);
            P::set(B[q >> 3], q & 7, v);
        }
        return;
    }
#pragma unroll
    for (int q = 0; q < 8 * NKG; ++q) {
        float v;
        if (q < 3 * L) {
            const int c = q % 3;
            const float comp = (c == 0) ? x : ((c == 1) ? y : z);
            v = sin_quadrant(comp * (float)(1 << (q / 3)), h);
        } else if (q == 3 * L) {
            v = h ? z : x;
        } else if (q == 3 * L + 1) {
            v = h ? 0.0f : y;
        } else {
            v = 0.0f;
        }
        P::set(B[q >> 3], q & 7, v);
    }
}

DEVINL void half_swap(uint32_t& a, uint32_t& b) {
    const auto r = __builtin_amdgcn_permlane32_swap(a, b, false, false);
    a = r[0]; b = r[1];
}
template <int NKG>
DEVINL void half_swap_groups(bf16x8 (&S)[NKG], bf16x8 (&C)[NKG]) {
    typedef __attribute__((ext_vector_type(4))) uint32_t u32x4_;
#pragma unroll
    for (int k = 0; k < NKG; ++k) {
        u32x4_ a = __builtin_bit_cast(u32x4_, S[k]), b = __builtin_bit_cast(u32x4_, C[k]);
#pragma unroll
        for (int i = 0; i < 4; ++i) { uint32_t x = a[i], y = b[i]; half_swap(x, y); a[i] = x; b[i] = y; }
        S[k] = __builtin_bit_cast(bf16x8, a); C[k] = __builtin_bit_cast(bf16x8, b);
    }
}
template <class P, int L, int NKG>
DEVINL void encode_pair(float x, float y, float z, typename P::BReg (&S)[NKG], typename P::BReg (&C)[NKG]) {
    static_assert(P::FAST_PE, "the paired prologue is the bf16 form (octaves by angle doubling)");
    float sv[3], cv[3];
    sincos_quadrant(x, sv[0], cv[0]); sincos_quadrant(y, sv[1], cv[1]); sincos_quadrant(z, sv[2], cv[2]);
#pragma unroll
    for (int f = 0; f < L; ++f) {
#pragma unroll
        for (int c = 0; c < 3; ++c) {
            const int q = 3 * f + c;
            P::set(S[q >> 3], q & 7, sv[c]);
            P::set(C[q >> 3], q & 7, cv[c]);
            if (f + 1 < L) {
                const float s2 = 2.0f * sv[c];
                const float ns = s2 * cv[c];
                const float nc = __builtin_fmaf(-s2, sv[c], 1.0f);
                sv[c] = ns; cv[c] = nc;
            }
        }
    }
#pragma unroll
    for (int q = 3 * L; q < 8 * NKG; ++q) {
        P::set(S[q >> 3], q & 7, (q == 3 * L) ? x : ((q == 3 * L + 1) ? y : 0.0f));
        P::set(C[q >> 3], q & 7, (q == 3 * L) ? z : 0.0f);
    }
}

template <class P, int L, int NKG>
DEVINL void encode_ipe(const float (&mu)[3], const float (&var)[3], int h, typename P::BReg (&B)[NKG]) {
    if constexpr (P::FAST_PE) {
        float sv[3], cv[3], at[3];
#pragma unroll
        for (int c = 0; c < 3; ++c) { sincos_quadrant(mu[c], sv[c], cv[c]); at[c] = expf(-0.5f * var[c]); }
#pragma unroll
        for (int f = 0; f < L; ++f) {
#pragma unroll
            for (int c = 0; c < 3; ++c) {
                const int q = 3 * f + c;
                P::set(B[q >> 3], q & 7, (h ? cv[c] : sv[c]) * at[c]);
                if (f + 1 < L) {
                    const float s2 = 2.0f * sv[c];
                    const float ns = s2 * cv[c];
                    const float nc = __builtin_fmaf(-s2, sv[c], 1.0f);
                    sv[c] = ns; cv[c] = nc;
                    const float a2 = at[c] * at[c];
                    at[c] = a2 * a2;
                }
            }
        }
    } else {
#pragma unroll
        for (int q = 0; q < 3 * L; ++q) {
            const int c = q % 3, f = q / 3;
            const float v = sin_quadrant(mu[c] * (float)(1 << f), h) * expf(-0.5f * (var[c] * (float)(1u << (2 * f))));
            P::set(B[q >> 3], q & 7, v);
        }
    }
#pragma unroll
    for (int q = 3 * L; q < 8 * NKG; ++q) {
        const float v = (q == 3 * L) ? (h ? mu[2] : mu[0]) : ((q == 3 * L + 1) ? (h ? 0.0f : mu[1]) : 0.0f);
        P::set(B[q >> 3], q & 7, v);
    }
}

struct Sample { float x, y, z, dx, dy, dz; };

DEVINL void contract_position(Sample& r) {
    const float n = norm3(r.x, r.y, r.z);
    if (n > 1.0f) {
        const float k = (2.0f - 1.0f / n) / n;
        r.x *= k; r.y *= k; r.z *= k;
    }
}

DEVINL void split_sample_index(const nerf_amd_samples& s, int64_t m, int64_t& n, int& si) {
    if (s.M <= 0x7fffffffll) {
        const uint32_t q = (uint32_t)m / (uint32_t)s.S;
        n = q; si = (int)((uint32_t)m - q * (uint32_t)s.S);
    } else {
        n = m / s.S; si = (int)(m - n * s.S);
    }
}
DEVINL Sample fetch_sample(const nerf_amd_samples& s, int64_t m, bool want_dir) {
    Sample r;
    if (s.mode == 0) {
        const float* p = s.pts + m * s.pts_stride;
        r.x = p[0]; r.y = p[1]; r.z = p[2];
        if (want_dir) { r.dx = p[3]; r.dy = p[4]; r.dz = p[5]; } else { r.dx = r.dy = r.dz = 0.0f; }
        if (s.contract) contract_position(r);
        return r;
    }
    int64_t n; int si;
    split_sample_index(s, m, n, si);
    float ox, oy, oz;
    if (s.mode == 1) {
        const float* ry = s.rays + n * 6;
        ox = ry[0]; oy = ry[1]; oz = ry[2]; r.dx = ry[3]; r.dy = ry[4]; r.dz = ry[5];
    } else {
        const int row = (int)(n / s.W), col = (int)(n - (int64_t)row * s.W);
        const float cx = (((float)col - (float)s.W * 0.5f) + 0.5f) / s.fx;
        const float cy = (((float)s.H * 0.5f - (float)row) + 0.5f) / s.fy;
        r.dx = (cx * s.pose[0] + cy * s.pose[1]) + (-1.0f) * s.pose[2];
        r.dy = (cx * s.pose[4] + cy * s.pose[5]) + (-1.0f) * s.pose[6];
        r.dz = (cx * s.pose[8] + cy * s.pose[9]) + (-1.0f) * s.pose[10];
        ox = s.pose[3]; oy = s.pose[7]; oz = s.pose[11];
    }
    float zv;
    if (s.z) zv = s.z[n * s.z_stride + si];
    else {
        const float uu = s.u ? s.u[n * s.S + si] : philox_u_strat(s.rng_seed, n + s.rng_ray_offset, si);
        zv = s.z_base[si] + uu * s.z_jitter;
    }
    r.x = ox + zv * r.dx; r.y = oy + zv * r.dy; r.z = oz + zv * r.dz;
    if (s.contract) contract_position(r);
    return r;
}

struct IpeSample { float mu[3], var[3], dx, dy, dz; };
DEVINL IpeSample fetch_sample_ipe(const nerf_amd_samples& s, int64_t m) {
    IpeSample r;
    int64_t n; int si;
    split_sample_index(s, m, n, si);
    const float* ry = s.rays + n * 6;
    const float* zz = s.z + n * s.z_stride + si;
    const float rr = s.ipe_radius;
    const ConeMoments c = cone_moments(zz[0], zz[1], (float)((double)rr * (double)rr));
    const float dn = s.ipe_dir_norm[0];
#pragma unroll
    for (int k = 0; k < 3; ++k) cone_mean_cov(c, ry[k], ry[3 + k], dn, r.mu[k], r.var[k]);
    r.dx = ry[3]; r.dy = ry[4]; r.dz = ry[5];
    if (s.contract) {
        Sample p{r.mu[0], r.mu[1], r.mu[2], 0.0f, 0.0f, 0.0f};
        contract_position(p);
        r.mu[0] = p.x; r.mu[1] = p.y; r.mu[2] = p.z;
    }
    return r;
}

constexpr uint32_t LDS_BIAS = MLP_RING_BYTES;
constexpr uint32_t LDS_STASH = MLP_RING_BYTES + 9216;
template <class P> constexpr uint32_t lds_dir() { return LDS_STASH + P::NW * P::NT * 4 * P::BREG_LDS; }
template <class P> constexpr uint32_t lds_tile() { return lds_dir<P>() + P::NW * P::NT * 1024; }
template <class P> constexpr uint32_t lds_total() { return lds_tile<P>() + P::NW * P::NT * 32 * 32 + P::NW * P::NT * 8 + 64; }

DEVINL void load_biases(const void* packed, size_t stream_bytes, int n_bias, uint32_t lds_off = MLP_RING_BYTES) {
    const float* b = reinterpret_cast<const float*>(reinterpret_cast<const char*>(packed) + stream_bytes);
    float* dst = reinterpret_cast<float*>(smem + lds_off);
    for (int i = threadIdx.x; i < n_bias; i += blockDim.x) dst[i] = b[i];
    __syncthreads();
}

struct ActDump {
    char* base;
    unsigned long long layer_stride;
    char* mask_base;
    unsigned long long mask_layer_stride;
};
template <class P>
DEVINL void dump_breg(const ActDump& d, int layer, int64_t subtile, int kg, int lane, const typename P::BReg& r) {
#ifndef ABL_NODUMPST
    P::store_global(d.base + (size_t)layer * d.layer_stride + ((size_t)subtile * 16 + kg) * (size_t)P::BREG_LDS, lane, r);
#endif
}

template <class P> constexpr uint32_t lds_maskacc() { return lds_total<P>(); }
template <class P> constexpr uint32_t lds_total_train() { return lds_total<P>() + P::NW * 2 * P::NT * 1024; }
template <class P> constexpr uint32_t lds_scaleacc() { return lds_total_train<P>(); }
template <class P> constexpr uint32_t lds_total_train_f8() { return lds_total_train<P>() + P::NW * 2 * P::NT * 1024; }
template <class P, bool F8>
DEVINL void dump_hidden(const ActDump& d, uint32_t sacc_wave, int layer, int64_t subtile, int t, int kg, int lane, const typename P::BReg& r) {
    if constexpr (F8) {
        const uint32_t E = f8_group_exponent<false>(r);
        f8_store_group(d.base + (size_t)layer * d.layer_stride + (size_t)subtile * F8_SUB_BYTES, kg, lane, f8_encode_group(r, E), E,
                       sacc_wave + ((layer & 1) * P::NT + t) * 1024);
    } else {
        dump_breg<P>(d, layer, subtile, kg, lane, r);
    }
}
DEVINL uint32_t breg_bits(const bf16x8& v) {
    typedef __attribute__((ext_vector_type(4))) uint32_t u32x4;
    const u32x4 d = __builtin_bit_cast(u32x4, v);
    uint32_t m = 0;
#pragma unroll
    for (int i = 0; i < 4; ++i) {
        const uint32_t x = d[i];
        uint32_t on;
        asm("v_pk_min_u16 %0, %1, %2" : "=v"(on) : "v"(x), "v"(0x00010001u));
        m |= on << i;
    }
    return m;
}
DEVINL uint32_t breg_bits(const f32x8& v) {
    uint32_t m = 0;
#pragma unroll
    for (int e = 0; e < 8; ++e) m |= (v[e] > 0.0f ? 1u : 0u) << ((e >> 1) + 16 * (e & 1));
    return m;
}
template <class P>
DEVINL void mask_or(uint32_t acc_wave, int layer, int t, int kg, int lane, const typename P::BReg& v) {
    unsigned* w = reinterpret_cast<unsigned*>(smem + acc_wave + ((layer & 1) * P::NT + t) * 1024 + lane * 16 + (kg >> 2) * 4);
    __hip_atomic_fetch_or(w, breg_bits(v) << (4 * (kg & 3)), __ATOMIC_RELAXED, __HIP_MEMORY_SCOPE_WORKGROUP);
}
template <class P, bool F8 = false>
DEVINL void mask_flush(const ActDump& d, uint32_t acc_wave, int layer, int64_t sub0, int lane, uint32_t sacc_wave = 0) {
    asm volatile("" ::: "memory");
#pragma unroll
    for (int t = 0; t < P::NT; ++t) {
        f32x4* rec = reinterpret_cast<f32x4*>(smem + acc_wave + ((layer & 1) * P::NT + t) * 1024 + lane * 16);
        const f32x4 v = *rec;
        *reinterpret_cast<f32x4*>(d.mask_base + (size_t)layer * d.mask_layer_stride + (size_t)(sub0 + t) * 1024 + lane * 16) = v;
        *rec = f32x4{0.0f, 0.0f, 0.0f, 0.0f};
        if constexpr (F8)
            f8_flush_scales(d.base + (size_t)layer * d.layer_stride + (size_t)(sub0 + t) * F8_SUB_BYTES, lane, sacc_wave + ((layer & 1) * P::NT + t) * 1024);
    }
    asm volatile("" ::: "memory");
}
template <class P>
DEVINL void mask_acc_init(uint32_t acc_wave, int lane) {
#pragma unroll
    for (int i = 0; i < 2 * P::NT; ++i) *reinterpret_cast<f32x4*>(smem + acc_wave + i * 1024 + lane * 16) = f32x4{0.0f, 0.0f, 0.0f, 0.0f};
}

template <class P, bool TRAIN, bool F8 = false>
__global__ __launch_bounds__(P::NW * 64) void proposal_kernel(const void* __restrict__ packed, nerf_amd_samples s,
                                                              float* __restrict__ density, ActDump dump) {
    using L = PropLayout;
    using BReg = typename P::BReg;
    constexpr int FPC = P::FPC;
    load_biases(packed, L::stream_bytes(P::PREC), L::N_BIAS);
    WeightStream<P, MLP_NSLOT> ws;
    ws.init(packed, L::N_FRAGS / FPC);
    const int lane = lane_id(), h = lane >> 5, j = lane & 31;
    const int wave = __builtin_amdgcn_readfirstlane((int)(threadIdx.x >> 6));
    constexpr int NT = P::NT;
    constexpr int TS = P::NW * NT * 32;
    const int64_t n_tiles = (s.M + TS - 1) / TS;
    const uint32_t bias0 = MLP_RING_BYTES;
    const uint32_t macc = lds_maskacc<P>() + wave * 2 * NT * 1024;
    const uint32_t sacc = lds_scaleacc<P>() + wave * 2 * NT * 1024;
    if constexpr (TRAIN) mask_acc_init<P>(macc, lane);

    for (int64_t tile = blockIdx.x; tile < n_tiles; tile += gridDim.x) {
        int64_t m[NT];
        BReg enc[NT][4];
        if constexpr (NT == 2 && P::FAST_PE) {
            m[0] = tile * TS + (wave * NT) * 32 + j;
            m[1] = m[0] + 32;
            const int64_t mo = h ? m[1] : m[0];
            const Sample sm = fetch_sample(s, mo < s.M ? mo : s.M - 1, false);
            encode_pair<P, 10, 4>(sm.x, sm.y, sm.z, enc[0], enc[1]);
            half_swap_groups<4>(enc[0], enc[1]);
            if constexpr (TRAIN) {
#pragma unroll
                for (int t = 0; t < NT; ++t)
#pragma unroll
                    for (int k = 0; k < 4; ++k) dump_breg<P>(dump, 4, tile * (TS / 32) + wave * NT + t, k, lane, enc[t][k]);
            }
        } else {
#pragma unroll
        for (int t = 0; t < NT; ++t) {
            m[t] = tile * TS + (wave * NT + t) * 32 + j;
            const Sample sm = fetch_sample(s, m[t] < s.M ? m[t] : s.M - 1, false);
            encode<P, 10, 4>(sm.x, sm.y, sm.z, h, enc[t]);
            if constexpr (TRAIN) {
#pragma unroll
                for (int k = 0; k < 4; ++k) dump_breg<P>(dump, 4, tile * (TS / 32) + wave * NT + t, k, lane, enc[t][k]);
            }
        }
        }
        BReg a[NT][16], b[NT][16];
        int lay = 0, lay_pend = 0;
        const int64_t sub0 = tile * (TS / 32) + wave * NT;
        auto put = [&](BReg (&buf)[NT][16], int layer, int fb, int t, const f32x16& acc, int half) {
            buf[t][2 * fb + half] = to_breg_half<P, true>(acc, half);
            if constexpr (TRAIN) {
                dump_hidden<P, F8>(dump, sacc, layer, sub0 + t, t, 2 * fb + half, lane, buf[t][2 * fb + half]);
                mask_or<P>(macc, layer, t, 2 * fb + half, lane, buf[t][2 * fb + half]);
            }
        };
        auto OA = [&](int fb, int t, const f32x16& acc, int half) { put(a, lay, fb, t, acc, half); };
        auto OB = [&](int fb, int t, const f32x16& acc, int half) { put(b, lay, fb, t, acc, half); };
        auto OA_pend = [&](int fb, int t, const f32x16& acc, int half) { put(a, lay_pend, fb, t, acc, half); };
        auto OB_pend = [&](int fb, int t, const f32x16& acc, int half) { put(b, lay_pend, fb, t, acc, half); };
        auto IN_A = [&](int kg, int t) -> BReg { return a[t][kg]; };
        Deferred<P, 6, 2> d = dense<P, 4, 8, L::START[0]>(ws, bias0 + L::BIAS_OFF[0] * 4,
            [&](int kg, int t) -> BReg { return enc[t][kg]; }, OA, NoPrev{});
        static_assert(L::START[1] % (2 * FPC) == L::START[3] % (2 * FPC), "chunk parity");
        auto IN_B = [&](int kg, int t) -> BReg { return b[t][kg]; };
#pragma unroll 1
        for (int r = 0; r < 2; ++r) {
            lay_pend = lay; lay = 1 + 2 * r;
            d = dense<P, 16, 8, L::START[1]>(ws, bias0 + (L::BIAS_OFF[1] + r * 512) * 4, IN_A, OB, prev_of(d, OA_pend));
            if constexpr (TRAIN) mask_flush<P, F8>(dump, macc, lay_pend, sub0, lane, sacc);
            if (r == 0) {
                lay_pend = lay; lay = 2;
                d = dense<P, 16, 8, L::START[2]>(ws, bias0 + L::BIAS_OFF[2] * 4, IN_B, OA, prev_of(d, OB_pend));
                if constexpr (TRAIN) mask_flush<P, F8>(dump, macc, lay_pend, sub0, lane, sacc);
            }
        }
        lay_pend = lay;
        float dens[NT];
        auto OH = [&](int, int t, const f32x16& acc, int half) { if (half == 0) dens[t] = acc[0]; };
        dense<P, 16, 1, L::START[4]>(ws, bias0 + L::BIAS_OFF[4] * 4, IN_B, OH, prev_of(d, OB_pend)).flush(OH);
        if constexpr (TRAIN) mask_flush<P, F8>(dump, macc, lay_pend, sub0, lane, sacc);
#pragma unroll
        for (int t = 0; t < NT; ++t)
            if (h == 0 && m[t] < s.M) density[m[t]] = dens[t];
    }
    ws.drain();
}

constexpr uint32_t lds_total_narrow() { return MLP_RING_BYTES + 9216; }
template <class P>
__global__ __launch_bounds__(P::NW * 64) void proposal128_kernel(const void* __restrict__ packed, nerf_amd_samples s, float* __restrict__ density) {
    using L = PropLayout128;
    using BReg = typename P::BReg;
    constexpr int HK = L::HK, HFB = L::HFB;
    load_biases(packed, L::stream_bytes(P::PREC), L::N_BIAS);
    WeightStream<P, MLP_NSLOT> ws;
    ws.init(packed, L::N_FRAGS / P::FPC);
    const int lane = lane_id(), h = lane >> 5, j = lane & 31;
    const int wave = __builtin_amdgcn_readfirstlane((int)(threadIdx.x >> 6));
    constexpr int NT = P::NT;
    constexpr int TS = P::NW * NT * 32;
    const int64_t n_tiles = (s.M + TS - 1) / TS;
    const uint32_t bias0 = MLP_RING_BYTES;
    for (int64_t tile = blockIdx.x; tile < n_tiles; tile += gridDim.x) {
        int64_t m[NT];
        BReg a[NT][HK], b[NT][HK];
        auto OA = [&](int fb, int t, const f32x16& acc, int half) { a[t][2 * fb + half] = to_breg_half<P, true>(acc, half); };
        auto OB = [&](int fb, int t, const f32x16& acc, int half) { b[t][2 * fb + half] = to_breg_half<P, true>(acc, half); };
        auto IN_A = [&](int kg, int t) -> BReg { return a[t][kg]; };
        auto IN_B = [&](int kg, int t) -> BReg { return b[t][kg]; };
        Deferred<P, HFB - 2, 2> d;
        {
            BReg enc[NT][4];
            constexpr int PAIRED = (NT >= 2 && P::FAST_PE) ? 2 : 0;
#pragma unroll
            for (int t = 0; t < NT; ++t) m[t] = tile * TS + (wave * NT + t) * 32 + j;
            if constexpr (PAIRED) {
                const int64_t mo = h ? m[1] : m[0];
                const Sample sm = fetch_sample(s, mo < s.M ? mo : s.M - 1, false);
                encode_pair<P, 10, 4>(sm.x, sm.y, sm.z, enc[0], enc[1]);
                half_swap_groups<4>(enc[0], enc[1]);
            }
#pragma unroll
            for (int t = PAIRED; t < NT; ++t) {
                const Sample sm = fetch_sample(s, m[t] < s.M ? m[t] : s.M - 1, false);
                encode<P, 10, 4>(sm.x, sm.y, sm.z, h, enc[t]);
            }
            d = dense<P, 4, HFB, L::START[0]>(ws, bias0 + L::BIAS_OFF[0] * 4, [&](int kg, int t) -> BReg { return enc[t][kg]; }, OA, NoPrev{});
        }
        d = dense<P, HK, HFB, L::START[1]>(ws, bias0 + L::BIAS_OFF[1] * 4, IN_A, OB, prev_of(d, OA));
        d = dense<P, HK, HFB, L::START[2]>(ws, bias0 + L::BIAS_OFF[2] * 4, IN_B, OA, prev_of(d, OB));
        d = dense<P, HK, HFB, L::START[3]>(ws, bias0 + L::BIAS_OFF[3] * 4, IN_A, OB, prev_of(d, OA));
        float dens[NT];
        auto OH = [&](int, int t, const f32x16& acc, int half) { if (half == 0) dens[t] = acc[0]; };
        dense<P, HK, 1, L::START[4]>(ws, bias0 + L::BIAS_OFF[4] * 4, IN_B, OH, prev_of(d, OB)).flush(OH);
        skip_frags<P, L::USED_FRAGS, L::N_FRAGS - L::USED_FRAGS>(ws);
#pragma unroll
        for (int t = 0; t < NT; ++t)
            if (h == 0 && m[t] < s.M) density[m[t]] = dens[t];
    }
    ws.drain();
}

struct FusedComposite {
    float* rgb;
    float* depth;
    float* weights;
    int white_bkg;
    float near, far;
};

template <class P, bool TRAIN, bool IPE = false, bool F8 = false, bool FUSED = false>
__global__ __launch_bounds__(P::NW * 64) void mip_kernel(const void* __restrict__ packed, nerf_amd_samples s,
                                                         float* __restrict__ rgbo, FusedComposite fc, ActDump dump) {
    using L = MipLayout;
    using BReg = typename P::BReg;
    constexpr int FPC = P::FPC;
#ifdef MLP_CLOCKPROBE
    const uint64_t probe_c0 = __builtin_readcyclecounter(), probe_r0 = __builtin_amdgcn_s_memrealtime();
#endif
    if constexpr (FUSED) { if (threadIdx.x < 16) reinterpret_cast<unsigned*>(smem + lds_tile<P>() + P::NW * P::NT * 32 * 32 + P::NW * P::NT * 8)[threadIdx.x] = 0u; }
    load_biases(packed, L::stream_bytes(P::PREC), L::N_BIAS);
    WeightStream<P, MLP_NSLOT> ws;
    ws.init(packed, L::N_FRAGS / FPC);
    const int lane = lane_id(), h = lane >> 5, j = lane & 31;
    const int wave = __builtin_amdgcn_readfirstlane((int)(threadIdx.x >> 6));
    constexpr int NT = P::NT;
    constexpr int TS = P::NW * NT * 32;
    const int64_t n_tiles = (s.M + TS - 1) / TS;
    const uint32_t bias0 = LDS_BIAS;
    const uint32_t macc = lds_maskacc<P>() + wave * 2 * NT * 1024;
    const uint32_t sacc = lds_scaleacc<P>() + wave * 2 * NT * 1024;
    if constexpr (TRAIN) mask_acc_init<P>(macc, lane);
    const uint32_t enc_lds0 = LDS_STASH + wave * NT * 4 * P::BREG_LDS + lane * 16;
    const uint32_t dir_lds0 = lds_dir<P>() + wave * NT * 1024 + lane * 16;
    auto enc_lds = [&](int t) -> uint32_t { return enc_lds0 + t * 4 * P::BREG_LDS; };
    auto dir_lds = [&](int t) -> uint32_t { return dir_lds0 + t * 1024; };

    for (int64_t tile = blockIdx.x; tile < n_tiles; tile += gridDim.x) {
        int64_t m[NT];
        BReg a[NT][16], b[NT][16];
        int lay = 0, lay_pend = 0;
        const int64_t sub0 = tile * (TS / 32) + wave * NT;
        auto put = [&](BReg (&buf)[NT][16], int layer, int fb, int t, const f32x16& acc, int half) {
            buf[t][2 * fb + half] = to_breg_half<P, true>(acc, half);
            if constexpr (TRAIN) {
                dump_hidden<P, F8>(dump, sacc, layer, sub0 + t, t, 2 * fb + half, lane, buf[t][2 * fb + half]);
                mask_or<P>(macc, layer, t, 2 * fb + half, lane, buf[t][2 * fb + half]);
            }
        };
        auto OA = [&](int fb, int t, const f32x16& acc, int half) { put(a, lay, fb, t, acc, half); };
        auto OB = [&](int fb, int t, const f32x16& acc, int half) { put(b, lay, fb, t, acc, half); };
        auto OA_pend = [&](int fb, int t, const f32x16& acc, int half) { put(a, lay_pend, fb, t, acc, half); };
        auto OB_pend = [&](int fb, int t, const f32x16& acc, int half) { put(b, lay_pend, fb, t, acc, half); };
        auto IN_A = [&](int kg, int t) -> BReg { return a[t][kg]; };
        Deferred<P, 6, 2> d;
        {
            BReg enc[NT][4];
            if constexpr (NT == 2 && P::FAST_PE && !IPE && !FUSED) {
                m[0] = tile * TS + (wave * NT) * 32 + j;
                m[1] = m[0] + 32;
                const int64_t mo = h ? m[1] : m[0];
                const Sample sm = fetch_sample(s, mo < s.M ? mo : s.M - 1, true);
                encode_pair<P, 10, 4>(sm.x, sm.y, sm.z, enc[0], enc[1]);
                half_swap_groups<4>(enc[0], enc[1]);
                uint32_t d0[3] = {__builtin_bit_cast(uint32_t, sm.dx), __builtin_bit_cast(uint32_t, sm.dy), __builtin_bit_cast(uint32_t, sm.dz)};
                uint32_t d1[3] = {d0[0], d0[1], d0[2]};
#pragma unroll
                for (int c = 0; c < 3; ++c) half_swap(d0[c], d1[c]);
#pragma unroll
                for (int t = 0; t < NT; ++t) {
#pragma unroll
                    for (int k = 0; k < 4; ++k) P::stash(enc_lds(t) + k * P::BREG_LDS, enc[t][k]);
                    if constexpr (TRAIN) {
#pragma unroll
                        for (int k = 0; k < 4; ++k) dump_breg<P>(dump, 8, sub0 + t, k, lane, enc[t][k]);
                    }
                    const uint32_t* dd = t ? d1 : d0;
                    const f32x4 dv = {__builtin_bit_cast(float, dd[0]), __builtin_bit_cast(float, dd[1]), __builtin_bit_cast(float, dd[2]), 0.0f};
                    *reinterpret_cast<f32x4*>(smem + dir_lds(t)) = dv;
                }
            } else {
#pragma unroll
            for (int t = 0; t < NT; ++t) {
                m[t] = tile * TS + (wave * NT + t) * 32 + j;
                Sample sm;
                if constexpr (IPE) {
                    const IpeSample is = fetch_sample_ipe(s, m[t] < s.M ? m[t] : s.M - 1);
                    encode_ipe<P, 10, 4>(is.mu, is.var, h, enc[t]);
                    sm.dx = is.dx; sm.dy = is.dy; sm.dz = is.dz;
                } else {
                    sm = fetch_sample(s, m[t] < s.M ? m[t] : s.M - 1, true);
                    encode<P, 10, 4>(sm.x, sm.y, sm.z, h, enc[t]);
                }
#pragma unroll
                for (int k = 0; k < 4; ++k) P::stash(enc_lds(t) + k * P::BREG_LDS, enc[t][k]);
                if constexpr (TRAIN) {
#pragma unroll
                    for (int k = 0; k < 4; ++k) dump_breg<P>(dump, 8, sub0 + t, k, lane, enc[t][k]);
                }
                f32x4 dv = {sm.dx, sm.dy, sm.dz, 0.0f};
                if constexpr (FUSED) {
                    const int64_t mm_ = m[t] < s.M ? m[t] : s.M - 1;
                    const int64_t n_ = mm_ / s.S;
                    const int si_ = (int)(mm_ - n_ * s.S);
                    const float nrm_ = norm3(sm.dx, sm.dy, sm.dz);
                    const float* zz_ = s.z + n_ * s.z_stride;
                    const float zn0 = zz_[si_] * nrm_;
                    const float dl = (si_ + 1 < s.S) ? (zz_[si_ + 1] * nrm_ - zn0) : 1e10f;
                    dv[3] = h ? dl : zn0;
                }
                *reinterpret_cast<f32x4*>(smem + dir_lds(t)) = dv;
            }
            }
            d = dense<P, 4, 8, L::START[0]>(ws, bias0 + L::BIAS_OFF[0] * 4,
                [&](int kg, int t) -> BReg { return enc[t][kg]; }, OA, NoPrev{});
        }
        static_assert(L::START[1] % (2 * FPC) == L::START[3] % (2 * FPC) && L::START[1] % (2 * FPC) == L::START[5] % (2 * FPC) &&
                      L::START[2] % (2 * FPC) == L::START[6] % (2 * FPC) && L::BIAS_OFF[6] == 6 * 256, "uniform layer loop");
        auto IN_B = [&](int kg, int t) -> BReg { return b[t][kg]; };
#pragma unroll 1
        for (int r = 0; r < 3; ++r) {
            lay_pend = lay; lay = 1 + 2 * r;
            d = dense<P, 16, 8, L::START[1]>(ws, bias0 + (1 + 2 * r) * 256 * 4, IN_A, OB, prev_of(d, OA_pend));
            if constexpr (TRAIN) mask_flush<P, F8>(dump, macc, lay_pend, sub0, lane, sacc);
            lay_pend = lay; lay = 2 + 2 * r;
            if (r == 1) {
                d = dense<P, 20, 8, L::START[4]>(ws, bias0 + L::BIAS_OFF[4] * 4,
                    [&](int kg, int t) -> BReg { if (kg < 4) return P::unstash(enc_lds(t) + kg * P::BREG_LDS); return b[t][kg >= 4 ? kg - 4 : 0]; },
                    OA, prev_of(d, OB_pend));
            } else {
                d = dense<P, 16, 8, L::START[2]>(ws, bias0 + (2 + 2 * r) * 256 * 4, IN_B, OA, prev_of(d, OB_pend));
            }
            if constexpr (TRAIN) mask_flush<P, F8>(dump, macc, lay_pend, sub0, lane, sacc);
        }
        lay_pend = lay;
        float sigma[NT];
        auto OSIG = [&](int, int t, const f32x16& acc, int half) { if (half == 0) sigma[t] = acc[0]; };
        const auto dsig = dense<P, 16, 1, L::START[7]>(ws, bias0 + L::BIAS_OFF[7] * 4, IN_A, OSIG, prev_of(d, OA_pend));
        if constexpr (TRAIN) mask_flush<P, F8>(dump, macc, 6, sub0, lane, sacc);
        BReg denc[NT][2];
#pragma unroll
        for (int t = 0; t < NT; ++t) {
            const f32x4 dv = *reinterpret_cast<const f32x4*>(smem + dir_lds(t));
            const float nrm = norm3(dv[0], dv[1], dv[2]);
            encode<P, 4, 2>(dv[0] / nrm, dv[1] / nrm, dv[2] / nrm, h, denc[t]);
            if constexpr (TRAIN) {
                dump_breg<P>(dump, 8, sub0 + t, 4, lane, denc[t][0]);
                dump_breg<P>(dump, 8, sub0 + t, 5, lane, denc[t][1]);
            }
        }
        BReg c[NT][8];
        auto OC = [&](int fb, int t, const f32x16& acc, int half) {
            c[t][2 * fb + half] = to_breg_half<P, true>(acc, half);
            if constexpr (TRAIN) {
                dump_hidden<P, F8>(dump, sacc, 7, sub0 + t, t, 2 * fb + half, lane, c[t][2 * fb + half]);
                mask_or<P>(macc, 7, t, 2 * fb + half, lane, c[t][2 * fb + half]);
            }
        };
        const auto dc = dense<P, 18, 4, L::START[8]>(ws, bias0 + L::BIAS_OFF[8] * 4,
            [&](int kg, int t) -> BReg { if (kg < 16) return a[t][kg < 16 ? kg : 0]; return denc[t][kg >= 16 ? kg - 16 : 0]; },
            OC, prev_of(dsig, OSIG));
        float r[NT], g[NT], bl[NT];
        auto ORGB = [&](int, int t, const f32x16& acc, int half) { if (half == 0) { r[t] = acc[0]; g[t] = acc[1]; bl[t] = acc[2]; } };
        dense<P, 8, 1, L::START[9]>(ws, bias0 + L::BIAS_OFF[9] * 4,
            [&](int kg, int t) -> BReg { return c[t][kg]; }, ORGB, prev_of(dc, OC)).flush(ORGB);
        if constexpr (TRAIN) mask_flush<P, F8>(dump, macc, 7, sub0, lane, sacc);
        f32x4 o[NT];
#pragma unroll
        for (int t = 0; t < NT; ++t) {
            o[t][0] = 1.0f / (1.0f + expf(-r[t]));
            o[t][1] = 1.0f / (1.0f + expf(-g[t]));
            o[t][2] = 1.0f / (1.0f + expf(-bl[t]));
            o[t][3] = sigma[t];
            if constexpr (!FUSED) {
                if (h == 0 && m[t] < s.M) *reinterpret_cast<f32x4*>(rgbo + m[t] * 4) = o[t];
            }
        }
        if constexpr (FUSED) {
            const int S = s.S;
            const int spr = S >> 5;
            char* tb = smem + lds_tile<P>();
            f32x4* t_ca = reinterpret_cast<f32x4*>(tb);
            u32x4* t_pz = reinterpret_cast<u32x4*>(tb + TS * 16);
            double* t_seg = reinterpret_cast<double*>(tb + TS * 32);
            unsigned* tickets = reinterpret_cast<unsigned*>(tb + TS * 32 + (TS / 32) * 8);
            {
                const int tt = (NT > 1) ? h : 0;
                const bool live = (NT > 1) || h == 0;
                const float k0 = (*reinterpret_cast<const f32x4*>(smem + dir_lds(0)))[3];
                const float k1 = (NT > 1) ? (*reinterpret_cast<const f32x4*>(smem + dir_lds(NT - 1)))[3] : 0.0f;
                float cr, cg, cb, sg, zn, dl;
                if (NT > 1) {
                    const float s0 = __shfl(o[NT - 1][0], j, 64), s1 = __shfl(o[NT - 1][1], j, 64), s2 = __shfl(o[NT - 1][2], j, 64),
                                s3 = __shfl(o[NT - 1][3], j, 64), sz = __shfl(k1, j, 64), d0 = __shfl(k0, j + 32, 64);
                    cr = h ? s0 : o[0][0]; cg = h ? s1 : o[0][1]; cb = h ? s2 : o[0][2]; sg = h ? s3 : o[0][3];
                    zn = h ? sz : k0;
                    dl = h ? k1 : d0;
                } else {
                    cr = o[0][0]; cg = o[0][1]; cb = o[0][2]; sg = o[0][3]; zn = k0; dl = __shfl(k0, j + 32, 64);
                }
                const float mm = expf(-fmaxf(sg, 0.0f) * dl);
                const float al = live ? 1.0f - mm : 0.0f;
                const double p = live ? (double)(mm + 1e-10f) : 1.0;
                const double incl = seg32_incl_scan_mul(p);
                double excl = wave_shift_up1(incl, 1.0);
                if (lane == 32) excl = 1.0;
                const int sub = wave * NT + tt;
                if (live) {
                    const int ts = sub * 32 + j;
                    t_ca[ts] = f32x4{cr, cg, cb, al};
                    const u32x2 eb = __builtin_bit_cast(u32x2, excl);
                    t_pz[ts] = u32x4{eb[0], eb[1], __builtin_bit_cast(uint32_t, zn), 0u};
                }
                if (j == 31 && live) t_seg[sub] = incl;
            }
            asm volatile("" ::: "memory");
#pragma unroll
            for (int t = 0; t < NT; ++t) {
                const int sub = wave * NT + t;
                const int ray_in_tile = sub / spr;
                const int64_t n = (tile * TS) / S + ray_in_tile;
                unsigned old = 0;
                if (lane == 0) old = __hip_atomic_fetch_add(&tickets[ray_in_tile], 1u, __ATOMIC_RELAXED, __HIP_MEMORY_SCOPE_WORKGROUP);
                old = __builtin_amdgcn_readfirstlane(old);
                asm volatile("" ::: "memory");
                if (((old + 1) % (unsigned)spr) != 0 || n * S >= s.M) continue;
                const int seg0 = ray_in_tile * spr;
                float ar = 0.0f, ag = 0.0f, abl = 0.0f, aw = 0.0f, ad = 0.0f;
                float* wout = fc.weights ? fc.weights + n * S : nullptr;
                double carry = 1.0;
                for (int base = 0; base < S; base += 64) {
                    const int q = base + lane;
                    const int sg0 = seg0 + (base >> 5);
                    const bool two = base + 32 < S;
                    const double T0 = t_seg[sg0], T1 = two ? t_seg[sg0 + (two ? 1 : 0)] : 1.0;
                    float w = 0.0f;
                    f32x4 ca = {0.0f, 0.0f, 0.0f, 0.0f};
                    float zn = 0.0f;
                    if (q < S) {
                        const int ts = seg0 * 32 + q;
                        ca = t_ca[ts];
                        const u32x4 pz = t_pz[ts];
                        const u32x2 eb = {pz[0], pz[1]};
                        double excl = __builtin_bit_cast(double, eb);
                        if (h) excl = excl * T0;
                        zn = __builtin_bit_cast(float, (uint32_t)pz[2]);
                        w = ca[3] * (float)(carry * excl);
                    }
                    carry *= (T1 * T0);
                    if (q < S) {
                        ar += w * ca[0]; ag += w * ca[1]; abl += w * ca[2]; aw += w; ad += w * zn;
                        if (wout) wout[q] = w;
                    }
                }
                ar = wave_sum(ar); ag = wave_sum(ag); abl = wave_sum(abl); aw = wave_sum(aw); ad = wave_sum(ad);
                if (lane == 0) {
                    if (fc.white_bkg) { const float bg = 1.0f - aw; ar += bg; ag += bg; abl += bg; }
                    fc.rgb[n * 3] = ar; fc.rgb[n * 3 + 1] = ag; fc.rgb[n * 3 + 2] = abl;
                    if (fc.depth) fc.depth[n] = (ad - fc.near) / (fc.far - fc.near);
                }
            }
        }
    }
    ws.drain();
#ifdef MLP_CLOCKPROBE
    if (blockIdx.x == 0 && threadIdx.x == 0 && rgbo != nullptr) {
        reinterpret_cast<uint64_t*>(rgbo)[0] = __builtin_readcyclecounter() - probe_c0;
        reinterpret_cast<uint64_t*>(rgbo)[1] = __builtin_amdgcn_s_memrealtime() - probe_r0;
    }
#endif
}


template <class P>
__global__ __launch_bounds__(P::NW * 64) void mip128_kernel(const void* __restrict__ packed, nerf_amd_samples s, float* __restrict__ rgbo) {
    using L = MipLayout128;
    using BReg = typename P::BReg;
    load_biases(packed, L::stream_bytes(P::PREC), L::N_BIAS);
    WeightStream<P, MLP_NSLOT> ws;
    ws.init(packed, L::N_FRAGS / P::FPC);
    const int lane = lane_id(), h = lane >> 5, j = lane & 31;
    const int wave = __builtin_amdgcn_readfirstlane((int)(threadIdx.x >> 6));
    constexpr int NT = P::NT;
    constexpr int TS = P::NW * NT * 32;
    const int64_t n_tiles = (s.M + TS - 1) / TS;
    const uint32_t bias0 = LDS_BIAS;
    const uint32_t enc_lds0 = LDS_STASH + wave * NT * 4 * P::BREG_LDS + lane * 16;
    const uint32_t dir_lds0 = lds_dir<P>() + wave * NT * 1024 + lane * 16;
    auto enc_lds = [&](int t) -> uint32_t { return enc_lds0 + t * 4 * P::BREG_LDS; };
    auto dir_lds = [&](int t) -> uint32_t { return dir_lds0 + t * 1024; };
    auto bias = [&](int l) -> uint32_t { return bias0 + L::BIAS_OFF[l] * 4; };
    for (int64_t tile = blockIdx.x; tile < n_tiles; tile += gridDim.x) {
        int64_t m[NT];
        BReg a[NT][8], b[NT][8], g[NT][16];
        auto OA = [&](int fb, int t, const f32x16& acc, int half) { a[t][2 * fb + half] = to_breg_half<P, true>(acc, half); };
        auto OB = [&](int fb, int t, const f32x16& acc, int half) { b[t][2 * fb + half] = to_breg_half<P, true>(acc, half); };
        auto OG = [&](int fb, int t, const f32x16& acc, int half) { g[t][2 * fb + half] = to_breg_half<P, true>(acc, half); };
        auto IN_A = [&](int kg, int t) -> BReg { return a[t][kg]; };
        auto IN_B = [&](int kg, int t) -> BReg { return b[t][kg]; };
        auto IN_G = [&](int kg, int t) -> BReg { return g[t][kg]; };
        Deferred<P, 2, 2> d;
        {
            BReg enc[NT][4];
#pragma unroll
            for (int t = 0; t < NT; ++t) m[t] = tile * TS + (wave * NT + t) * 32 + j;
            if constexpr (NT == 2 && P::FAST_PE) {
                const int64_t mo = h ? m[1] : m[0];
                const Sample sm = fetch_sample(s, mo < s.M ? mo : s.M - 1, true);
                encode_pair<P, 10, 4>(sm.x, sm.y, sm.z, enc[0], enc[1]);
                half_swap_groups<4>(enc[0], enc[1]);
                uint32_t d0[3] = {__builtin_bit_cast(uint32_t, sm.dx), __builtin_bit_cast(uint32_t, sm.dy), __builtin_bit_cast(uint32_t, sm.dz)};
                uint32_t d1[3] = {d0[0], d0[1], d0[2]};
#pragma unroll
                for (int c = 0; c < 3; ++c) half_swap(d0[c], d1[c]);
#pragma unroll
                for (int t = 0; t < NT; ++t) {
#pragma unroll
                    for (int k = 0; k < 4; ++k) P::stash(enc_lds(t) + k * P::BREG_LDS, enc[t][k]);
                    const uint32_t* dd = t ? d1 : d0;
                    const f32x4 dv = {__builtin_bit_cast(float, dd[0]), __builtin_bit_cast(float, dd[1]), __builtin_bit_cast(float, dd[2]), 0.0f};
                    *reinterpret_cast<f32x4*>(smem + dir_lds(t)) = dv;
                }
            } else {
#pragma unroll
                for (int t = 0; t < NT; ++t) {
                    const Sample sm = fetch_sample(s, m[t] < s.M ? m[t] : s.M - 1, true);
                    encode<P, 10, 4>(sm.x, sm.y, sm.z, h, enc[t]);
#pragma unroll
                    for (int k = 0; k < 4; ++k) P::stash(enc_lds(t) + k * P::BREG_LDS, enc[t][k]);
                    const f32x4 dv = {sm.dx, sm.dy, sm.dz, 0.0f};
                    *reinterpret_cast<f32x4*>(smem + dir_lds(t)) = dv;
                }
            }
            d = dense<P, 4, 4, L::START[0]>(ws, bias(0), [&](int kg, int t) -> BReg { return enc[t][kg]; }, OA, NoPrev{});
        }
        static_assert(L::START[1] % (2 * P::FPC) == L::START[3] % (2 * P::FPC) && L::BIAS_OFF[3] == L::BIAS_OFF[1] + 256, "shared a -> b instance");
#pragma unroll 1
        for (int r = 0; r < 2; ++r) {
            d = dense<P, 8, 4, L::START[1]>(ws, bias0 + (L::BIAS_OFF[1] + r * 256) * 4, IN_A, OB, prev_of(d, OA));
            if (r == 0) d = dense<P, 8, 4, L::START[2]>(ws, bias(2), IN_B, OA, prev_of(d, OB));
        }
        d = dense<P, 12, 4, L::START[4]>(ws, bias(4),
            [&](int kg, int t) -> BReg { if (kg < 4) return P::unstash(enc_lds(t) + kg * P::BREG_LDS); return b[t][kg >= 4 ? kg - 4 : 0]; }, OA, prev_of(d, OB));
        d = dense<P, 8, 4, L::START[5]>(ws, bias(5), IN_A, OB, prev_of(d, OA));
        const auto dg = dense<P, 8, 8, L::START[6]>(ws, bias(6), IN_B, OG, prev_of(d, OB));
        float sigma[NT];
        auto OSIG = [&](int, int t, const f32x16& acc, int half) { if (half == 0) sigma[t] = acc[0]; };
        const auto dsig = dense<P, 16, 1, L::START[7]>(ws, bias(7), IN_G, OSIG, prev_of(dg, OG));
        BReg denc[NT][2];
#pragma unroll
        for (int t = 0; t < NT; ++t) {
            const f32x4 dv = *reinterpret_cast<const f32x4*>(smem + dir_lds(t));
            const float nrm = norm3(dv[0], dv[1], dv[2]);
            encode<P, 4, 2>(dv[0] / nrm, dv[1] / nrm, dv[2] / nrm, h, denc[t]);
        }
        BReg c[NT][8];
        auto OC = [&](int fb, int t, const f32x16& acc, int half) { c[t][2 * fb + half] = to_breg_half<P, true>(acc, half); };
        const auto dc = dense<P, 18, 4, L::START[8]>(ws, bias(8),
            [&](int kg, int t) -> BReg { if (kg < 16) return g[t][kg < 16 ? kg : 0]; return denc[t][kg >= 16 ? kg - 16 : 0]; }, OC, prev_of(dsig, OSIG));
        float r[NT], gg[NT], bl[NT];
        auto ORGB = [&](int, int t, const f32x16& acc, int half) { if (half == 0) { r[t] = acc[0]; gg[t] = acc[1]; bl[t] = acc[2]; } };
        dense<P, 8, 1, L::START[9]>(ws, bias(9), [&](int kg, int t) -> BReg { return c[t][kg]; }, ORGB, prev_of(dc, OC)).flush(ORGB);
#pragma unroll
        for (int t = 0; t < NT; ++t) {
            f32x4 o;
            o[0] = 1.0f / (1.0f + expf(-r[t]));
            o[1] = 1.0f / (1.0f + expf(-gg[t]));
            o[2] = 1.0f / (1.0f + expf(-bl[t]));
            o[3] = sigma[t];
            if (h == 0 && m[t] < s.M) *reinterpret_cast<f32x4*>(rgbo + m[t] * 4) = o;
        }
    }
    ws.drain();
}

constexpr uint32_t REF_LDS_BIAS = MLP_CHUNK_BYTES * MLP_NSLOT_REF;
constexpr uint32_t REF_LDS_STASH = REF_LDS_BIAS + RefLayout::N_BIAS * 4;
template <class P> constexpr uint32_t ref_lds_total() { return REF_LDS_STASH + P::NW * P::NT * 11 * P::BREG_LDS; }

template <class P>
DEVINL void ide_encode(float x, float y, float z, float kappa_inv, float nv_dot, int h, const float* __restrict__ mat,
                       typename P::BReg (&out)[3]) {
    constexpr int TM[19] = {0, 1, 0, 1, 2, 0, 1, 2, 3, 4, 0, 1, 2, 3, 4, 5, 6, 7, 8};
    constexpr int TL[19] = {1, 1, 2, 2, 2, 4, 4, 4, 4, 4, 8, 8, 8, 8, 8, 8, 8, 8, 8};
    float zp[9], re[9], im[9];
    zp[0] = 1.0f; re[0] = 1.0f; im[0] = 0.0f;
#pragma unroll
    for (int k = 1; k < 9; ++k) {
        zp[k] = zp[k - 1] * z;
        re[k] = re[k - 1] * x - im[k - 1] * y;
        im[k] = re[k - 1] * y + im[k - 1] * x;
    }
    const float att1 = expf(-1.0f * kappa_inv), att2 = expf(-3.0f * kappa_inv), att4 = expf(-10.0f * kappa_inv),
                att8 = expf(-36.0f * kappa_inv);
#pragma unroll
    for (int t = 0; t < 19; ++t) {
        const int m = TM[t], l = TL[t];
        float poly = 0.0f;
#pragma unroll
        for (int k = 0; k <= l - m; ++k) poly = __builtin_fmaf(mat[k * 19 + t], zp[k], poly);
        const float att = (l == 1) ? att1 : ((l == 2) ? att2 : ((l == 4) ? att4 : att8));
        const float v = ((h ? im[m] : re[m]) * poly) * att;
        P::set(out[t >> 3], t & 7, v);
    }
    P::set(out[2], 3, h ? 0.0f : nv_dot);
#pragma unroll
    for (int e = 4; e < 8; ++e) P::set(out[2], e, 0.0f);
}

template <class P, bool TRAIN>
__global__ __launch_bounds__(P::NW * 64) void ref_kernel(const void* __restrict__ packed, nerf_amd_samples s,
                                                         float* __restrict__ rgbo, float* __restrict__ normal_out,
                                                         const float* __restrict__ bn_noise, ActDump dump, float* __restrict__ aux, int flags,
                                                         unsigned long long noise_seed, const unsigned long long* __restrict__ noise_seed_dev, float noise_std) {
    using L = RefLayout;
    if (noise_seed_dev != nullptr) noise_seed = noise_seed_dev[0];
    using BReg = typename P::BReg;
    constexpr int FPC = P::FPC;
    load_biases(packed, L::stream_bytes(P::PREC), L::N_BIAS, REF_LDS_BIAS);
    const float* ide_mat = reinterpret_cast<const float*>(reinterpret_cast<const char*>(packed) + L::stream_bytes(P::PREC)) + L::N_BIAS;
    WeightStream<P, MLP_NSLOT_REF> ws;
    ws.init(packed, L::N_FRAGS / FPC);
// ... 76 lines not shown
                    for (int k = 0; k < 4; ++k) dump_breg<P>(dump, 8, sub0 + t, 11 + k, lane, enc[t][k]);
                }
                f32x4 dv = {sm.dx, sm.dy, sm.dz, 0.0f};
                *reinterpret_cast<f32x4*>(smem + dir_lds(t)) = dv;
            }
            }
            d = dense<P, 4, 8, L::START[0]>(ws, bias0 + L::BIAS_OFF[0] * 4,
                [&](int kg, int t) -> BReg { return enc[t][kg]; }, OA, NoPrev{});
        }
        static_assert(L::START[1] % (2 * FPC) == L::START[3] % (2 * FPC) && L::START[5] % (2 * FPC) == L::START[7] % (2 * FPC) &&
                      L::BIAS_OFF[3] == L::BIAS_OFF[1] + 512 && L::BIAS_OFF[7] == L::BIAS_OFF[5] + 512, "chunk parity / bias spacing of the shared a -> b instance");
#pragma unroll 1
        for (int r = 0; r < 2; ++r) {
            lay_pend = lay; lay = 1 + 2 * r;
            d = dense<P, 16, 8, L::START[1]>(ws, bias0 + (L::BIAS_OFF[1] + 2 * r * 256) * 4, IN_A, OB, prev_of(d, OA_pend));
            if (r == 0) {
                lay_pend = lay; lay = 2;
                d = dense<P, 16, 8, L::START[2]>(ws, bias0 + L::BIAS_OFF[2] * 4, IN_B, OA, prev_of(d, OB_pend));
            }
        }
        lay_pend = lay; lay = 4;
        d = dense<P, 20, 8, L::START[4]>(ws, bias0 + L::BIAS_OFF[4] * 4,
            [&](int kg, int t) -> BReg { if (kg < 4) return P::unstash(stash(t) + kg * P::BREG_LDS); return b[t][kg >= 4 ? kg - 4 : 0]; },
            OA, prev_of(d, OB_pend));
#pragma unroll 1
        for (int r = 0; r < 2; ++r) {
            lay_pend = lay; lay = 5 + 2 * r;
            d = dense<P, 16, 8, L::START[5]>(ws, bias0 + (L::BIAS_OFF[5] + 2 * r * 256) * 4, IN_A, OB, prev_of(d, OA_pend));
            if (r == 0) {
                lay_pend = lay; lay = 6;
                d = dense<P, 16, 8, L::START[6]>(ws, bias0 + L::BIAS_OFF[6] * 4, IN_B, OA, prev_of(d, OB_pend));
            }
        }
        lay_pend = lay;
        BReg bn[NT][8];
        f32x16 hd[NT];
        auto OHD = [&](int fb, int t, const f32x16& acc, int half) {
            if (fb < 4) {
                f32x16 v = acc;
                if (bn_noise != nullptr) {
                    const int64_t mm = m[t] < s.M ? m[t] : s.M - 1;
                    const float* np_ = bn_noise + mm * 128 + 32 * (fb < 4 ? fb : 0) + 16 * half + 4 * h;
                    const f32x4 n0 = *reinterpret_cast<const f32x4*>(np_), n1 = *reinterpret_cast<const f32x4*>(np_ + 8);
#pragma unroll
                    for (int e = 0; e < 4; ++e) { v[8 * half + e] += n0[e]; v[8 * half + 4 + e] += n1[e]; }
                } else if (noise_std > 0.0f) {
                    float z[8];
                    philox_normal8(noise_seed, m[t] < s.M ? m[t] : s.M - 1, 2 * (2 * (fb < 4 ? fb : 0) + half) + h, noise_std, z);
#pragma unroll
                    for (int e = 0; e < 8; ++e) v[8 * half + e] += z[e];
                }
                bn[t][2 * (fb < 4 ? fb : 0) + half] = to_breg_half<P, false>(v, half);
                if constexpr (TRAIN) dump_breg<P>(dump, 8, sub0 + t, 2 * (fb < 4 ? fb : 0) + half, lane, bn[t][2 * (fb < 4 ? fb : 0) + half]);
            } else if (half == 0) hd[t] = acc;
        };
        dense<P, 16, 5, L::START[8]>(ws, bias0 + L::BIAS_OFF[8] * 4, IN_B, OHD, prev_of(d, OB_pend)).flush(OHD);
        float keep[NT][4];
        BReg ide[NT][3];
#pragma unroll
        for (int t = 0; t < NT; ++t) {
            const float nx0 = __shfl(hd[t][0], j, 64), ny0 = __shfl(hd[t][1], j, 64), nz0 = __shfl(hd[t][2], j, 64);
            const float rough = softplus_f(__shfl(hd[t][3], j, 64) - 1.0f);
            const float nn = norm3(nx0, ny0, nz0) + 1e-7f;
            const float nx = -nx0 / nn, ny = -ny0 / nn, nz = -nz0 / nn;
            const f32x4 dv = *reinterpret_cast<const f32x4*>(smem + dir_lds(t));
            const float dot = (dv[0] * nx + dv[1] * ny) + dv[2] * nz;
            const float t2 = 2.0f * dot;
            const float rx = dv[0] - t2 * nx, ry = dv[1] - t2 * ny, rz = dv[2] - t2 * nz;
            ide_encode<P>(rx, ry, rz, rough, dot, h, ide_mat, ide[t]);
            if (normal_out && h == 0 && m[t] < s.M) { normal_out[m[t] * 3] = nx; normal_out[m[t] * 3 + 1] = ny; normal_out[m[t] * 3 + 2] = nz; }
            keep[t][0] = h ? hd[t][0] : hd[t][4]; keep[t][1] = h ? hd[t][1] : hd[t][5]; keep[t][2] = h ? hd[t][2] : hd[t][6]; keep[t][3] = hd[t][3];
            if constexpr (TRAIN) {
#pragma unroll
                for (int k = 0; k < 3; ++k) dump_breg<P>(dump, 8, sub0 + t, 8 + k, lane, ide[t][k]);
                if (m[t] < s.M) {
                    float* ax = aux + m[t] * 16;
                    if (h == 0) {
                        *reinterpret_cast<f32x4*>(ax) = f32x4{hd[t][0], hd[t][1], hd[t][2], hd[t][3]};
                        ax[8] = hd[t][4]; ax[9] = hd[t][5]; ax[10] = hd[t][6];
                    } else {
                        *reinterpret_cast<f32x4*>(ax + 4) = f32x4{hd[t][0], hd[t][1], hd[t][2], hd[t][3]};
                    }
                }
            }
#pragma unroll
            for (int k = 0; k < 8; ++k) P::stash(stash(t) + k * P::BREG_LDS, bn[t][k]);
#pragma unroll
            for (int k = 0; k < 3; ++k) P::stash(stash(t) + (8 + k) * P::BREG_LDS, ide[t][k]);
        }
        lay = lay_pend = 9;
        d = dense<P, 11, 8, L::START[9]>(ws, bias0 + L::BIAS_OFF[9] * 4,
            [&](int kg, int t) -> BReg { if (kg < 8) return bn[t][kg < 8 ? kg : 0]; return ide[t][kg >= 8 ? kg - 8 : 0]; },
            OA, NoPrev{});
        static_assert(L::START[10] % (2 * FPC) == L::START[12] % (2 * FPC) && L::START[14] % (2 * FPC) == L::START[16] % (2 * FPC) &&
                      L::BIAS_OFF[12] == L::BIAS_OFF[10] + 512 && L::BIAS_OFF[16] == L::BIAS_OFF[14] + 512, "chunk parity / bias spacing of the shared a -> b instance");
#pragma unroll 1
        for (int r = 0; r < 2; ++r) {
            lay_pend = lay; lay = 10 + 2 * r;
            d = dense<P, 16, 8, L::START[10]>(ws, bias0 + (L::BIAS_OFF[10] + 2 * r * 256) * 4, IN_A, OB, prev_of(d, OA_pend));
            if (r == 0) {
                lay_pend = lay; lay = 11;
                d = dense<P, 16, 8, L::START[11]>(ws, bias0 + L::BIAS_OFF[11] * 4, IN_B, OA, prev_of(d, OB_pend));
            }
        }
        lay_pend = lay; lay = 13;
        d = dense<P, 27, 8, L::START[13]>(ws, bias0 + L::BIAS_OFF[13] * 4,
            [&](int kg, int t) -> BReg { if (kg < 11) return P::unstash(stash(t) + kg * P::BREG_LDS); return b[t][kg >= 11 ? kg - 11 : 0]; },
            OA, prev_of(d, OB_pend));
#pragma unroll 1
        for (int r = 0; r < 2; ++r) {
            lay_pend = lay; lay = 14 + 2 * r;
            d = dense<P, 16, 8, L::START[14]>(ws, bias0 + (L::BIAS_OFF[14] + 2 * r * 256) * 4, IN_A, OB, prev_of(d, OA_pend));
            if (r == 0) {
                lay_pend = lay; lay = 15;
                d = dense<P, 16, 8, L::START[15]>(ws, bias0 + L::BIAS_OFF[15] * 4, IN_B, OA, prev_of(d, OB_pend));
            }
        }
        lay_pend = lay;
        float sr[NT], sg[NT], sb[NT];
        auto OSPEC = [&](int, int t, const f32x16& acc, int half) { if (half == 0) { sr[t] = acc[0]; sg[t] = acc[1]; sb[t] = acc[2]; } };
        dense<P, 16, 1, L::START[17]>(ws, bias0 + L::BIAS_OFF[17] * 4, IN_B, OSPEC, prev_of(d, OB_pend)).flush(OSPEC);
#pragma unroll
        for (int t = 0; t < NT; ++t) {
            const float d0 = __shfl(keep[t][0], j + 32, 64), d1 = __shfl(keep[t][1], j + 32, 64), d2 = __shfl(keep[t][2], j + 32, 64),
                        dens = __shfl(keep[t][3], j + 32, 64);
            if (h == 0 && m[t] < s.M) {
                auto sig = [](float v) { return 1.0f / (1.0f + expf(-v)); };
                f32x4 o;
                if (flags & NERF_AMD_REF_SRGB) {
                    o[0] = srgb_from_linear(sig(sr[t]) * sig(keep[t][0]) + sig(d0 - SRGB_LOG3));
                    o[1] = srgb_from_linear(sig(sg[t]) * sig(keep[t][1]) + sig(d1 - SRGB_LOG3));
                    o[2] = srgb_from_linear(sig(sb[t]) * sig(keep[t][2]) + sig(d2 - SRGB_LOG3));
                } else {
                    o[0] = sig(sr[t]) * sig(keep[t][0]) + sig(d0);
                    o[1] = sig(sg[t]) * sig(keep[t][1]) + sig(d1);
                    o[2] = sig(sb[t]) * sig(keep[t][2]) + sig(d2);
                }
                o[3] = dens;
                *reinterpret_cast<f32x4*>(rgbo + m[t] * 4) = o;
                if constexpr (TRAIN) { float* ax = aux + m[t] * 16; ax[11] = sr[t]; ax[12] = sg[t]; ax[13] = sb[t]; ax[14] = 0.0f; ax[15] = 0.0f; }
            }
        }
    }
    ws.drain();
}

int grid_for(int64_t n_tiles) {
    const int n_cu = nerf_host::cu_count();
    return (int)(n_tiles < n_cu ? n_tiles : n_cu);
}

int allow_dynamic_lds(const void* fn, size_t lds) { return nerf_host::allow_dynamic_lds(fn, lds); }

template <class P, class Lay, bool TRAIN = false, bool F8 = false, class K, class... Extra>
int launch(K kernel, const void* packed, const nerf_amd_samples& s, float* out, hipStream_t st, Extra... extra) {
    constexpr int TS = P::NW * P::NT * 32;
    const int64_t n_tiles = (s.M + TS - 1) / TS;
    if (n_tiles == 0) return 0;
    const size_t lds = F8 ? lds_total_train_f8<P>() : (TRAIN ? lds_total_train<P>() : lds_total<P>());
    if (int e = allow_dynamic_lds(reinterpret_cast<const void*>(kernel), lds)) return e;
    hipLaunchKernelGGL(kernel, dim3(grid_for(n_tiles)), dim3(P::NW * 64), lds, st, packed, s, out, extra...);
    return (int)hipGetLastError();
}
const ActDump NO_DUMP{nullptr, 0ull, nullptr, 0ull};

using PB16 = PBF16W;

}

#ifndef MLP_TU
#define MLP_TU 0
#endif
#if MLP_TU == 0 || MLP_TU == 1
int mlp_launch_proposal(const void* packed, int precision, const nerf_amd_samples& s, float* density, hipStream_t st) {
    if (precision == NERF_AMD_BF16) return launch<PB16, PropLayout>(proposal_kernel<PB16, false>, packed, s, density, st, NO_DUMP);
    return launch<PF32, PropLayout>(proposal_kernel<PF32, false>, packed, s, density, st, NO_DUMP);
}
#endif
#if MLP_TU == 0 || MLP_TU == 2
int mlp_launch_mip(const void* packed, int precision, const nerf_amd_samples& s, float* rgbo, hipStream_t st) {
    const FusedComposite off{nullptr, nullptr, nullptr, 0, 0.0f, 1.0f};
    if (s.ipe) {
        if (precision == NERF_AMD_BF16) return launch<PB16, MipLayout>(mip_kernel<PB16, false, true>, packed, s, rgbo, st, off, NO_DUMP);
        return launch<PF32, MipLayout>(mip_kernel<PF32, false, true>, packed, s, rgbo, st, off, NO_DUMP);
    }
    if (precision == NERF_AMD_BF16) return launch<PB16, MipLayout>(mip_kernel<PB16, false>, packed, s, rgbo, st, off, NO_DUMP);
    return launch<PF32, MipLayout>(mip_kernel<PF32, false>, packed, s, rgbo, st, off, NO_DUMP);
}
int mlp_launch_mip128(const void* packed, int precision, const nerf_amd_samples& s, float* rgbo, hipStream_t st) {
    if (precision == NERF_AMD_BF16) return launch<PB16, MipLayout128>(mip128_kernel<PB16>, packed, s, rgbo, st);
    return launch<PF32, MipLayout128>(mip128_kernel<PF32>, packed, s, rgbo, st);
}
int mlp_launch_mip_composite(const void* packed, int precision, const nerf_amd_samples& s, float* rgb, float* depth, float* weights,
                             int white_bkg, float near, float far, hipStream_t st) {
    const FusedComposite fc{rgb, depth, weights, white_bkg, near, far};
    if (precision == NERF_AMD_BF16) return launch<PB16, MipLayout>(mip_kernel<PB16, false, false, false, true>, packed, s, (float*)nullptr, st, fc, NO_DUMP);
    return launch<PF32, MipLayout>(mip_kernel<PF32, false, false, false, true>, packed, s, (float*)nullptr, st, fc, NO_DUMP);
}
#endif
#if MLP_TU == 0 || MLP_TU == 1
template <class P>
static int launch_proposal128(const void* packed, const nerf_amd_samples& s, float* density, hipStream_t st) {
    constexpr int TS = P::NW * P::NT * 32;
    const int64_t n_tiles = (s.M + TS - 1) / TS;
    if (n_tiles == 0) return 0;
    const size_t lds = lds_total_narrow();
    if (int e = allow_dynamic_lds(reinterpret_cast<const void*>(proposal128_kernel<P>), lds)) return e;
    hipLaunchKernelGGL(proposal128_kernel<P>, dim3(grid_for(n_tiles)), dim3(P::NW * 64), lds, st, packed, s, density);
    return (int)hipGetLastError();
}
int mlp_launch_proposal128(const void* packed, int precision, const nerf_amd_samples& s, float* density, hipStream_t st) {
    if (precision == NERF_AMD_BF16) return launch_proposal128<PBF16N>(packed, s, density, st);
    return launch_proposal128<PF32>(packed, s, density, st);
}
#endif
#if MLP_TU == 0 || MLP_TU == 1
size_t mlp_train_layer_stride(int precision, int64_t M) {
    const int64_t ts = (precision != NERF_AMD_F32) ? (int64_t)PB16::NW * PB16::NT * 32 : (int64_t)PF32::NW * PF32::NT * 32;
    const int64_t n_sub = ((M + ts - 1) / ts) * (ts / 32);
    return (size_t)n_sub * 16 * (precision != NERF_AMD_F32 ? 1024 : 2048);
}
size_t mlp_train_mask_stride(int precision, int64_t M) { return mlp_train_layer_stride(precision, M) / (16 * (precision != NERF_AMD_F32 ? 1024 : 2048)) * 1024; }
#else
size_t mlp_train_layer_stride(int precision, int64_t M);
size_t mlp_train_mask_stride(int precision, int64_t M);
#endif
static ActDump make_dump(void* dump, int precision, int64_t M, int slots) {
    const unsigned long long ls = mlp_train_layer_stride(precision, M);
    return ActDump{reinterpret_cast<char*>(dump), ls, reinterpret_cast<char*>(dump) + (size_t)slots * ls, (unsigned long long)mlp_train_mask_stride(precision, M)};
}
#if MLP_TU == 0 || MLP_TU == 1
int mlp_launch_proposal_train(const void* packed, int precision, const nerf_amd_samples& s, float* density, void* dump, hipStream_t st) {
    if (precision == NERF_AMD_BF16_F8) {
        const ActDump d8 = make_dump(dump, NERF_AMD_BF16, s.M, PROP_DUMP_SLOTS);
        return launch<PB16, PropLayout, true, true>(proposal_kernel<PB16, true, true>, packed, s, density, st, d8);
    }
    const ActDump d = make_dump(dump, precision, s.M, PROP_DUMP_SLOTS);
    if (precision == NERF_AMD_BF16) return launch<PBF16, PropLayout, true>(proposal_kernel<PBF16, true>, packed, s, density, st, d);
    return launch<PF32, PropLayout, true>(proposal_kernel<PF32, true>, packed, s, density, st, d);
}
#endif
#if MLP_TU == 0 || MLP_TU == 2
int mlp_launch_mip_train(const void* packed, int precision, const nerf_amd_samples& s, float* rgbo, void* dump, hipStream_t st) {
    const FusedComposite off{nullptr, nullptr, nullptr, 0, 0.0f, 1.0f};
    if (precision == NERF_AMD_BF16_F8) {
        const ActDump d8 = make_dump(dump, NERF_AMD_BF16, s.M, MIP_DUMP_SLOTS);
        if (s.ipe) return launch<PB16, MipLayout, true, true>(mip_kernel<PB16, true, true, true>, packed, s, rgbo, st, off, d8);
        return launch<PB16, MipLayout, true, true>(mip_kernel<PB16, true, false, true>, packed, s, rgbo, st, off, d8);
    }
    const ActDump d = make_dump(dump, precision, s.M, MIP_DUMP_SLOTS);
    if (s.ipe) {
        if (precision == NERF_AMD_BF16) return launch<PB16, MipLayout, true>(mip_kernel<PB16, true, true>, packed, s, rgbo, st, off, d);
        return launch<PF32, MipLayout, true>(mip_kernel<PF32, true, true>, packed, s, rgbo, st, off, d);
    }
    if (precision == NERF_AMD_BF16) return launch<PB16, MipLayout, true>(mip_kernel<PB16, true>, packed, s, rgbo, st, off, d);
    return launch<PF32, MipLayout, true>(mip_kernel<PF32, true>, packed, s, rgbo, st, off, d);
}

#endif
#if MLP_TU == 0 || MLP_TU == 3
template <class P, bool TRAIN>
static int launch_ref(const void* packed, const nerf_amd_samples& s, float* rgbo, float* normal, const float* bn_noise, ActDump dump, float* aux,
                      int flags, hipStream_t st, unsigned long long seed = 0, const unsigned long long* seed_dev = nullptr, float noise_std = 0.0f) {
    constexpr int TS = P::NW * P::NT * 32;
    const int64_t n_tiles = (s.M + TS - 1) / TS;
    if (n_tiles == 0) return 0;
    const size_t lds = ref_lds_total<P>();
    if (int e = allow_dynamic_lds(reinterpret_cast<const void*>(ref_kernel<P, TRAIN>), lds)) return e;
    hipLaunchKernelGGL((ref_kernel<P, TRAIN>), dim3(grid_for(n_tiles)), dim3(P::NW * 64), lds, st, packed, s, rgbo, normal, bn_noise, dump, aux, flags, seed, seed_dev, noise_std);
    return (int)hipGetLastError();
}
int mlp_launch_ref(const void* packed, int precision, const nerf_amd_samples& s, float* rgbo, float* normal, const float* bn_noise,
                   int flags, hipStream_t st) {
    if (precision == NERF_AMD_BF16) return launch_ref<PB16, false>(packed, s, rgbo, normal, bn_noise, NO_DUMP, nullptr, flags, st);
    return launch_ref<PF32, false>(packed, s, rgbo, normal, bn_noise, NO_DUMP, nullptr, flags, st);
}
int mlp_launch_ref_train(const void* packed, int precision, const nerf_amd_samples& s, float* rgbo, float* normal, const float* bn_noise,
                         void* dump, float* aux, int flags, hipStream_t st, unsigned long long seed, const unsigned long long* seed_dev, float noise_std) {
    const ActDump d = make_dump(dump, precision, s.M, REF_DUMP_SLOTS);
#ifndef REF_TRAIN_WIDE
    if (precision == NERF_AMD_BF16) return launch_ref<PBF16, true>(packed, s, rgbo, normal, bn_noise, d, aux, flags, st, seed, seed_dev, noise_std);
#endif
    if (precision == NERF_AMD_BF16) return launch_ref<PB16, true>(packed, s, rgbo, normal, bn_noise, d, aux, flags, st, seed, seed_dev, noise_std);
    return launch_ref<PF32, true>(packed, s, rgbo, normal, bn_noise, d, aux, flags, st, seed, seed_dev, noise_std);
}
#endif
```

nerf_amd/ops.py:

```python
import ctypes as C
from typing import Optional, Sequence

import torch

from . import _lib
from ._lib import lib, check, Samples, F32, BF16, BF16_F8, NET_PROPOSAL, NET_MIP, NET_REF, NET_PROPOSAL_128, NET_MIP_128, PROP_W128, FINE_W128, ACT_RELU, ACT_IDENTITY, ACT_SOFTPLUS

_PRECISION_OVERRIDE = None


def set_precision(p: Optional[str]):
    global _PRECISION_OVERRIDE
    if p not in (None, "fp32", "bf16"):
        raise ValueError("precision must be None, 'fp32' or 'bf16'")
    _PRECISION_OVERRIDE = p


_TRAIN_DUMPS = __import__("os").environ.get("NERF_AMD_TRAIN_DUMPS", "bf16")


def set_train_dumps(fmt: str):
    global _TRAIN_DUMPS
    if fmt not in ("bf16", "fp8"):
        raise ValueError("train dumps: 'bf16' or 'fp8'")
# ... 40 lines not shown
_ARENA = {}
_ARENA_BUSY = {}
ARENA_STATS = {"persistent": 0, "fresh": 0, "grown": 0}


def set_persistent_buffers(on: bool) -> None:
    global _PERSISTENT
    _PERSISTENT = bool(on)
    if not on:
        release_buffers()


def release_buffers() -> None:
    _ARENA.clear()
    _ARENA_BUSY.clear()


def _arena_key(tag, device):
    return (device.index if device.index is not None else torch.cuda.current_device(), torch.cuda.current_stream(device).cuda_stream, tag)


def _arena_buffer(key, nbytes: int, device) -> torch.Tensor:
    buf = _ARENA.get(key)
    if buf is None or buf.numel() < nbytes:
        _ARENA.pop(key, None)
        buf = None
        buf = _ARENA[key] = torch.empty(nbytes, dtype=torch.uint8, device=device)
        ARENA_STATS["grown"] += 1
    return buf


def scratch(tag, nbytes: int, device) -> torch.Tensor:
    nbytes = int(nbytes)
    device = torch.device(device)
    if nbytes == 0 or not _PERSISTENT or torch.cuda.is_current_stream_capturing():
        ARENA_STATS["fresh"] += 1
        return torch.empty(nbytes, dtype=torch.uint8, device=device)
    ARENA_STATS["persistent"] += 1
    return _arena_buffer(_arena_key(tag, device), nbytes, device)[:nbytes]


class _Lease:
    __slots__ = ("key",)

    def __init__(self, key):
        self.key = key
        _ARENA_BUSY[key] = id(self)

    def __del__(self):
        try:
            if _ARENA_BUSY.get(self.key) == id(self):
                del _ARENA_BUSY[self.key]
        except Exception:
            pass


def leased(tag, nbytes: int, device) -> torch.Tensor:
    nbytes = int(nbytes)
    device = torch.device(device)
    if nbytes == 0 or not _PERSISTENT or torch.cuda.is_current_stream_capturing():
        ARENA_STATS["fresh"] += 1
        return torch.empty(nbytes, dtype=torch.uint8, device=device)
    key = _arena_key(tag, device)
    if key in _ARENA_BUSY:
        ARENA_STATS["fresh"] += 1
        return torch.empty(nbytes, dtype=torch.uint8, device=device)
    view = _arena_buffer(key, nbytes, device)[:nbytes]
    view._nerf_amd_lease = _Lease(key)
    ARENA_STATS["persistent"] += 1
    return view


def _raw(t: torch.Tensor, name: str) -> torch.Tensor:
    if t.is_cuda and t.dtype is torch.float32 and t.is_contiguous():
        return t
    return _dev(t.detach(), name)


def pack_weights(net: int, precision: int, weights: Sequence[torch.Tensor], biases: Sequence[torch.Tensor]) -> torch.Tensor:
    ws = [_raw(w, "weight") for w in weights]
    bs = [_raw(b, "bias") for b in biases]
    nbytes = lib.nerf_amd_packed_bytes(net, precision)
    packed = torch.empty(nbytes, dtype=torch.uint8, device=ws[0].device)
    n = len(ws)
    wp = (C.c_void_p * n)(*[w.data_ptr() for w in ws])
    bp = (C.c_void_p * n)(*[b.data_ptr() for b in bs])
    check(lib.nerf_amd_pack_weights(net, precision, wp, bp, n, _ptr(packed), _stream()), "nerf_amd_pack_weights")
    return packed


def _samples_pts(pts: torch.Tensor, stride: int, contract: bool = False) -> Samples:
    s = Samples()
    s.mode = 0
    s.M = pts.numel() // stride
    s.pts = pts.data_ptr()
    s.pts_stride = stride
    s.contract = int(bool(contract))
    return s


def samples_rays(rays: torch.Tensor, S: int, z: Optional[torch.Tensor] = None, z_base: Optional[torch.Tensor] = None,
                 u: Optional[torch.Tensor] = None, z_jitter: float = 0.0, contract: bool = False, ipe_radius: Optional[float] = None,
                 ipe_dir_norm: Optional[torch.Tensor] = None, seed: int = 0, rng_ray_offset: int = 0) -> Samples:
    s = Samples()
    s.contract = int(bool(contract))
    if ipe_radius is not None:
        if z is None or z.shape[-1] < S + 1 or ipe_dir_norm is None:
            raise ValueError("nerf_amd: integrated PE needs explicit z with S+1 depths per ray and ipe_dir_norm")
        s.ipe, s.ipe_radius, s.ipe_dir_norm = 1, float(ipe_radius), ipe_dir_norm.data_ptr()
    s.mode = 1
    s.S = S
    s.M = rays.shape[0] * S
    s.rays = rays.data_ptr()
    if z is not None:
        s.z = z.data_ptr()
        s.z_stride = z.shape[-1]
    else:
        s.z_base = z_base.data_ptr()
        if u is not None:
            s.u = u.data_ptr()
        else:
            s.rng_seed, s.rng_ray_offset = int(seed) & 0xFFFFFFFFFFFFFFFF, int(rng_ray_offset)
        s.z_jitter = z_jitter
        s.z_stride = S
    return s


def proposal_forward(packed: torch.Tensor, precision: int, pts: torch.Tensor, contract: bool = False) -> torch.Tensor:
    pts = _dev(pts, "pts")
    out = torch.empty(pts.shape[:-1], dtype=torch.float32, device=pts.device)
    if out.numel() == 0:
        return out
    s = _samples_pts(pts, 3, contract)
    check(lib.nerf_amd_proposal_forward(_ptr(packed), _prop_prec(packed, precision), C.byref(s), _ptr(out), _stream()), "nerf_amd_proposal_forward")
    return out


def proposal_forward_samples(packed, precision, s: Samples, shape, device) -> torch.Tensor:
    out = torch.empty(shape, dtype=torch.float32, device=device)
    check(lib.nerf_amd_proposal_forward(_ptr(packed), _prop_prec(packed, precision), C.byref(s), _ptr(out), _stream()), "nerf_amd_proposal_forward")
    return out


def mip_forward(packed: torch.Tensor, precision: int, pts: torch.Tensor, contract: bool = False) -> torch.Tensor:
    pts = _dev(pts, "pts")
    out = torch.empty(pts.shape[:-1] + (4,), dtype=torch.float32, device=pts.device)
    if out.numel() == 0:
        return out
    s = _samples_pts(pts, 6, contract)
    check(lib.nerf_amd_mip_forward(_ptr(packed), _prop_prec(None, precision, packed), C.byref(s), _ptr(out), _stream()), "nerf_amd_mip_forward")
    return out


def mip_forward_samples(packed, precision, s: Samples, shape, device) -> torch.Tensor:
    out = torch.empty(tuple(shape) + (4,), dtype=torch.float32, device=device)
    check(lib.nerf_amd_mip_forward(_ptr(packed), _prop_prec(None, precision, packed), C.byref(s), _ptr(out), _stream()), "nerf_amd_mip_forward")
    return out


def mip_forward_composite(packed, precision, rays: torch.Tensor, z: torch.Tensor, n_samples: int, white_bkg: bool, near: float,
                          far: float, want_depth: bool = True, want_weights: bool = False):
    N = rays.shape[0]
    dev = rays.device
    if int(getattr(packed, "_nerf_amd_layout", 0)) & FINE_W128:
        rgbo = mip_forward_samples(packed, precision, samples_rays(rays, n_samples, z=z), (N, n_samples), dev)
        rgb, w, depth, _ = composite(rgbo, z, rays, True, bool(white_bkg), ACT_RELU, (near, far), want_weights=want_weights)
        return rgb, (depth if want_depth else None), (w if want_weights else None)
    rgb = torch.empty((N, 3), dtype=torch.float32, device=dev)
    depth = torch.empty((N,), dtype=torch.float32, device=dev) if want_depth else None
    w = torch.empty((N, n_samples), dtype=torch.float32, device=dev) if want_weights else None
    s = samples_rays(rays, n_samples, z=z)
    check(lib.nerf_amd_mip_forward_composite(_ptr(packed), _prop_prec(None, precision, packed), C.byref(s), int(white_bkg), float(near), float(far), _ptr(rgb),
                                             _ptr(depth), _ptr(w), _stream()), "nerf_amd_mip_forward_composite")
    return rgb, depth, w


def _ref_out(shape, device, want_normal):
    rgbo = torch.empty(tuple(shape) + (4,), dtype=torch.float32, device=device)
    normal = torch.empty(tuple(shape) + (3,), dtype=torch.float32, device=device) if want_normal else None
    return rgbo, normal


REF_SRGB = 1


def ref_forward(packed: torch.Tensor, precision: int, pts: torch.Tensor, want_normal: bool = True, noise: Optional[torch.Tensor] = None,
                flags: int = 0, contract: bool = False):
    pts = _dev(pts, "pts")
    rgbo, normal = _ref_out(pts.shape[:-1], pts.device, want_normal)
    if rgbo.numel() == 0:
        return rgbo, normal
    s = _samples_pts(pts, 6, contract)
    if noise is None:
        check(lib.nerf_amd_ref_forward(_ptr(packed), precision, C.byref(s), int(flags), _ptr(rgbo), _ptr(normal), _stream()), "nerf_amd_ref_forward")
    else:
        noise = _dev(noise, "noise")
        if noise.numel() != s.M * 128:
            raise ValueError("nerf_amd: bottle-neck noise must be (..., 128) over the same samples")
        check(lib.nerf_amd_ref_forward_train(_ptr(packed), precision, C.byref(s), int(flags), _ptr(noise), _ptr(rgbo), _ptr(normal), _stream()),
              "nerf_amd_ref_forward_train")
    return rgbo, normal


def ref_forward_samples(packed, precision, s: Samples, shape, device, want_normal: bool = True, flags: int = 0):
    rgbo, normal = _ref_out(shape, device, want_normal)
    check(lib.nerf_amd_ref_forward(_ptr(packed), precision, C.byref(s), int(flags), _ptr(rgbo), _ptr(normal), _stream()), "nerf_amd_ref_forward")
    return rgbo, normal


def positional_encoding(x: torch.Tensor, L: int) -> torch.Tensor:
    x = _dev(x, "x")
    out = torch.empty(x.shape[:-1] + (6 * L,), dtype=torch.float32, device=x.device)
    check(lib.nerf_amd_positional_encoding(_ptr(x), x.numel() // 3, L, _ptr(out), _stream()), "nerf_amd_positional_encoding")
    return out


def dirs_norm(rays: torch.Tensor) -> torch.Tensor:
    rays = _dev(rays, "rays")
    out = torch.empty((1,), dtype=torch.float32, device=rays.device)
    check(lib.nerf_amd_dirs_norm(_ptr(rays), rays.shape[0], _ptr(out), _stream()), "nerf_amd_dirs_norm")
    return out


def cone_parameters(z: torch.Tensor, r: float):
    z = _dev(z, "zvals")
    N, S = z.shape[0], z.shape[1] - 1
    out = [torch.empty((N, S), dtype=torch.float32, device=z.device) for _ in range(3)]
    check(lib.nerf_amd_cone_parameters(_ptr(z), N, S, float(r), _ptr(out[0]), _ptr(out[1]), _ptr(out[2]), _stream()), "nerf_amd_cone_parameters")
    return tuple(out)


def ipe_feature(z: torch.Tensor, rays: torch.Tensor, L: int, r: float, dir_norm: Optional[torch.Tensor] = None, contract: bool = False):
    z, rays = _dev(z, "zvals"), _dev(rays, "cam_rays")
    N, S = z.shape[0], z.shape[1] - 1
    if dir_norm is None:
        dir_norm = dirs_norm(rays)
    feat = torch.empty((N, S, 6 * L), dtype=torch.float32, device=z.device)
    mu = torch.empty((N, S, 3), dtype=torch.float32, device=z.device)
    mu_t = torch.empty((N, S), dtype=torch.float32, device=z.device)
    fn, name = (lib.nerf_amd_ipe_feature_contracted, "nerf_amd_ipe_feature_contracted") if contract else (lib.nerf_amd_ipe_feature, "nerf_amd_ipe_feature")
    check(fn(_ptr(z), _ptr(rays), N, S, L, float(r), _ptr(dir_norm), _ptr(feat), _ptr(mu), _ptr(mu_t), _stream()), name)
    return feat, mu, mu_t


def generate_rays(pose: torch.Tensor, H: int, W: int, fx: float, fy: float, device, ray_offset: int = 0,
                  n: Optional[int] = None) -> torch.Tensor:
    n = H * W - ray_offset if n is None else n
    host = (C.c_float * 12)(*pose.detach().float().cpu().reshape(-1).tolist()[:12])
    rays = torch.empty((n, 6), dtype=torch.float32, device=device)
    check(lib.nerf_amd_generate_rays(host, H, W, float(fx), float(fy), ray_offset, n, _ptr(rays), _stream()), "nerf_amd_generate_rays")
    return rays


def length2pts(rays: torch.Tensor, z: torch.Tensor) -> torch.Tensor:
    rays, z = _dev(rays, "rays"), _dev(z, "z")
    N, S = z.shape
    out = torch.empty((N, S, 6), dtype=torch.float32, device=z.device)
    check(lib.nerf_amd_length2pts(_ptr(rays), _ptr(z), N, S, _ptr(out), _stream()), "nerf_amd_length2pts")
    return out


def sigma_to_weights(sigma: torch.Tensor, z: torch.Tensor, dirs: Optional[torch.Tensor], act: int = ACT_RELU) -> torch.Tensor:
    sigma, z = _dev(sigma, "sigma"), _dev(z, "z")
    dirs = None if dirs is None else _dev(dirs, "dirs")
    N, S = z.shape
    w = torch.empty((N, S), dtype=torch.float32, device=z.device)
    check(lib.nerf_amd_sigma_to_weights(_ptr(sigma), _ptr(z), _ptr(dirs), N, S, act, _ptr(w), _stream()), "nerf_amd_sigma_to_weights")
    return w


def max_blur(w: torch.Tensor, alpha: float) -> torch.Tensor:
    w = _dev(w, "weights")
    S = w.shape[-1]
    out = torch.empty_like(w)
    check(lib.nerf_amd_max_blur(_ptr(w), w.numel() // S, S, float(alpha), _ptr(out), _stream()), "nerf_amd_max_blur")
    return out


def inverse_sample(w: torch.Tensor, z: torch.Tensor, u: torch.Tensor, sort: bool, want_below: bool = True):
    w, z, u = _dev(w, "weights"), _dev(z, "z"), _dev(u, "u")
    N, Cn = z.shape
    K = u.shape[-1]
    z_out = torch.empty((N, K), dtype=torch.float32, device=z.device)
    below = torch.empty((N, K), dtype=torch.int64, device=z.device) if want_below else None
    check(lib.nerf_amd_inverse_sample(_ptr(w), _ptr(z), _ptr(u), N, Cn, K, int(sort), _ptr(z_out), _ptr(below), _stream()),
          "nerf_amd_inverse_sample")
    return z_out, below


def sample_pdf(bins: torch.Tensor, weights: torch.Tensor, u: torch.Tensor):
    bins, weights, u = _dev(bins, "bins"), _dev(weights, "weights"), _dev(u, "u")
    N, B = bins.shape
    K = u.shape[-1]
    out = torch.empty((N, K), dtype=torch.float32, device=bins.device)
    below = torch.empty((N, K), dtype=torch.int64, device=bins.device)
    above = torch.empty((N, K), dtype=torch.int64, device=bins.device)
    check(lib.nerf_amd_sample_pdf(_ptr(bins), _ptr(weights), _ptr(u), N, B, K, _ptr(out), _ptr(below), _ptr(above), _stream()),
          "nerf_amd_sample_pdf")
    return out, below, above


def pixel_rays(coords: torch.Tensor, pose: torch.Tensor, fx: float, fy: float) -> torch.Tensor:
    if not coords.is_cuda:
        raise RuntimeError("nerf_amd: 'coords' must live on the HIP device")
    coords = coords.to(torch.int64).contiguous()
    host = (C.c_float * 12)(*pose.detach().float().cpu().reshape(-1).tolist()[:12])
    rays = torch.empty((coords.shape[0], 6), dtype=torch.float32, device=coords.device)
    check(lib.nerf_amd_pixel_rays(host, float(fx), float(fy), _ptr(coords), coords.shape[0], _ptr(rays), _stream()), "nerf_amd_pixel_rays")
    return rays
# ... 760 lines not shown
```

Before: 9.195 million.

## Precompute per-ray direction encoding table for the bf16 fine MLP

Adds a small pre-pass kernel that normalizes each ray direction and stores its bf16 positional encoding in a 64-byte-per-ray table. The fine MIP kernel then loads the encoded direction from this table instead of recomputing the direction encoding for every sample, removing redundant per-sample transcendental work. In exchange it costs an extra kernel launch, extra global memory traffic, and more LDS per block, which may lower occupancy. It also adds workspace APIs and clock-probe instrumentation behind an ifdef.

```diff
diff --git a/include/nerf_amd.h b/include/nerf_amd.h
--- a/include/nerf_amd.h
+++ b/include/nerf_amd.h
@@ -64,6 +64,11 @@
                               float* density, void* stream);
 int nerf_amd_mip_forward(const void* packed, int precision, const nerf_amd_samples* src,
                          float* rgbo, void* stream);
+
+size_t nerf_amd_mip_forward_workspace_bytes(int64_t n_rays);
+int nerf_amd_mip_forward_ws(const void* packed, int precision, const nerf_amd_samples* src,
+                            float* rgbo, void* workspace, size_t workspace_bytes, void* stream);
+int nerf_amd_mip_dir_table(const nerf_amd_samples* src, void* table, void* stream);
 
 int nerf_amd_mip_forward_composite(const void* packed, int precision, const nerf_amd_samples* src, int white_bkg,
                                    float near, float far, float* rgb, float* depth, float* weights, void* stream);
diff --git a/nerf_amd/_lib.py b/nerf_amd/_lib.py
--- a/nerf_amd/_lib.py
+++ b/nerf_amd/_lib.py
@@ -35,6 +35,9 @@
     "nerf_amd_pack_weights": (C.c_int, [C.c_int, C.c_int, C.POINTER(c_void), C.POINTER(c_void), C.c_int, c_void, c_void]),
     "nerf_amd_proposal_forward": (C.c_int, [c_void, C.c_int, C.POINTER(Samples), c_void, c_void]),
     "nerf_amd_mip_forward": (C.c_int, [c_void, C.c_int, C.POINTER(Samples), c_void, c_void]),
+    "nerf_amd_mip_forward_workspace_bytes": (C.c_size_t, [i64]),
+    "nerf_amd_mip_forward_ws": (C.c_int, [c_void, C.c_int, C.POINTER(Samples), c_void, c_void, C.c_size_t, c_void]),
+    "nerf_amd_mip_dir_table": (C.c_int, [C.POINTER(Samples), c_void, c_void]),
     "nerf_amd_mip_forward_composite": (C.c_int, [c_void, C.c_int, C.POINTER(Samples), C.c_int, C.c_float, C.c_float, c_void, c_void, c_void,
                                                  c_void]),
     "nerf_amd_ref_forward": (C.c_int, [c_void, C.c_int, C.POINTER(Samples), C.c_int, c_void, c_void, c_void]),
diff --git a/nerf_amd/csrc/capi.hip b/nerf_amd/csrc/capi.hip
--- a/nerf_amd/csrc/capi.hip
+++ b/nerf_amd/csrc/capi.hip
@@ -9,6 +9,9 @@
 int mlp_launch_proposal128(const void*, int, const nerf_amd_samples&, float*, hipStream_t);
 int mlp_launch_mip(const void*, int, const nerf_amd_samples&, float*, hipStream_t);
 int mlp_launch_mip128(const void*, int, const nerf_amd_samples&, float*, hipStream_t);
+size_t mlp_mip_dir_table_bytes(int64_t);
+int mlp_launch_mip_dir_table(const nerf_amd_samples&, void*, hipStream_t);
+int mlp_launch_mip_dirtab(const void*, const nerf_amd_samples&, float*, void*, hipStream_t);
 int mlp_launch_mip_composite(const void*, int, const nerf_amd_samples&, float*, float*, float*, int, float, float, hipStream_t);
 int mlp_launch_ref(const void*, int, const nerf_amd_samples&, float*, float*, const float*, int, hipStream_t);
 size_t mlp_train_layer_stride(int, int64_t);
@@ -164,6 +167,10 @@
 static int launch_mip_any(int flags, const void* packed, int precision, const nerf_amd_samples& s, float* rgbo, hipStream_t st) {
     return (flags & NERF_AMD_FINE_W128) ? mlp_launch_mip128(packed, precision, s, rgbo, st) : mlp_launch_mip(packed, precision, s, rgbo, st);
 }
+static bool dir_table_applies(int flags, int precision, const nerf_amd_samples& s) {
+    return precision == NERF_AMD_BF16 && !(flags & NERF_AMD_FINE_W128) && !s.ipe && (s.mode == 1 || s.mode == 2);
+}
+static void* align256(void* p) { return reinterpret_cast<void*>((reinterpret_cast<uintptr_t>(p) + 255) & ~(uintptr_t)255); }
 static int launch_proposal_any(int flags, const void* packed, int precision, const nerf_amd_samples& s, float* density, hipStream_t st) {
     return (flags & NERF_AMD_PROP_W128) ? mlp_launch_proposal128(packed, precision, s, density, st) : mlp_launch_proposal(packed, precision, s, density, st);
 }
@@ -207,6 +214,33 @@
     return hip_status(launch_mip_any(lflags, packed, precision, *src, rgbo, S(stream)), "nerf_amd_mip_forward");
 }
 
+size_t nerf_amd_mip_forward_workspace_bytes(int64_t n_rays) {
+    return n_rays > 0 ? mlp_mip_dir_table_bytes(n_rays) + 256 : 0;
+}
+
+int nerf_amd_mip_forward_ws(const void* packed, int precision, const nerf_amd_samples* src, float* rgbo, void* workspace,
+                            size_t workspace_bytes, void* stream) {
+    if (!workspace) return nerf_amd_mip_forward(packed, precision, src, rgbo, stream);
+    const int lflags = precision & ~0xff;
+    const int prec = precision & 0xff;
+    if (bad_prec(prec) || (lflags & ~NERF_AMD_FINE_W128)) return fail(NERF_AMD_EINVAL, "unknown precision");
+    if (int c = check_samples(src, true)) return c;
+    if (!dir_table_applies(lflags, prec, *src)) return nerf_amd_mip_forward(packed, precision, src, rgbo, stream);
+    if (src->M == 0) return NERF_AMD_OK;
+    if (!packed || !rgbo) return fail(NERF_AMD_EINVAL, "NULL argument");
+    if (workspace_bytes < nerf_amd_mip_forward_workspace_bytes((src->M + src->S - 1) / src->S))
+        return fail(NERF_AMD_EINVAL, "workspace smaller than nerf_amd_mip_forward_workspace_bytes(rays)");
+    return hip_status(mlp_launch_mip_dirtab(packed, *src, rgbo, align256(workspace), S(stream)), "nerf_amd_mip_forward_ws");
+}
+
+int nerf_amd_mip_dir_table(const nerf_amd_samples* src, void* table, void* stream) {
+    if (int c = check_samples(src, true)) return c;
+    if (src->mode != 1 && src->mode != 2) return fail(NERF_AMD_EINVAL, "the direction table is per ray: modes 1 and 2 only");
+    if (src->M == 0) return NERF_AMD_OK;
+    if (!table) return fail(NERF_AMD_EINVAL, "NULL argument");
+    return hip_status(mlp_launch_mip_dir_table(*src, table, S(stream)), "nerf_amd_mip_dir_table");
+}
+
 int nerf_amd_mip_forward_composite(const void* packed, int precision, const nerf_amd_samples* src, int white_bkg, float near,
                                    float far, float* rgb, float* depth, float* weights, void* stream) {
     const int lflags = precision & ~0xff;
@@ -668,7 +702,8 @@
     const size_t b = ((size_t)N * (n_fine + 1) * 4 + 255) & ~(size_t)255;
     const size_t c = ((size_t)N * n_fine * 16 + 255) & ~(size_t)255;
     const size_t d = ((size_t)N * 24 + 255) & ~(size_t)255;
-    return a + b + c + d + 512;
+    const size_t e = (mlp_mip_dir_table_bytes(N) + 255) & ~(size_t)255;
+    return a + b + c + d + 512 + e;
 }
 
 int nerf_amd_render_rays(const void* packed_prop, const void* packed_mip, int precision, const float* rays,
@@ -706,6 +741,7 @@
     }
     ws += ((size_t)N * 24 + 255) & ~(size_t)255;
     float* dir_norm = reinterpret_cast<float*>(ws);
+    void* dir_table = ws + 256;
     const bool ipe = camera && camera->ipe;
     if (ipe) {
         if (!(camera->ipe_radius > 0.0f)) return fail(NERF_AMD_EINVAL, "integrated PE needs a positive ipe_radius");
@@ -727,7 +763,9 @@
     sf.mode = 1; sf.rays = rays; sf.S = n_fine; sf.M = N * n_fine; sf.z = z_fine; sf.z_stride = n_fine + 1;
     sf.contract = sc.contract;
     if (ipe) { sf.ipe = 1; sf.ipe_radius = camera->ipe_radius; sf.ipe_dir_norm = dir_norm; }
-    if (int e = launch_mip_any(lflags, packed_mip, precision, sf, rgbo, st)) return hip_status(e, "fine MLP");
+    if (dir_table_applies(lflags, precision, sf)) {
+        if (int e = mlp_launch_mip_dirtab(packed_mip, sf, rgbo, dir_table, st)) return hip_status(e, "fine MLP");
+    } else if (int e = launch_mip_any(lflags, packed_mip, precision, sf, rgbo, st)) return hip_status(e, "fine MLP");
     const int flags = 1 | (white_bkg ? 2 : 0);
     if (int e = sk_composite(rgbo, z_fine, n_fine + 1, rays + 3, 6, N, n_fine, flags, NERF_AMD_ACT_RELU, 0.0f, near, far, nullptr,
                              nullptr, rgb, weights, depth, nullptr, st)) return hip_status(e, "composite");
diff --git a/nerf_amd/csrc/mlp_kernels.hip b/nerf_amd/csrc/mlp_kernels.hip
--- a/nerf_amd/csrc/mlp_kernels.hip
+++ b/nerf_amd/csrc/mlp_kernels.hip
@@ -143,8 +143,22 @@
         n = m / s.S; si = (int)(m - n * s.S);
     }
 }
-DEVINL Sample fetch_sample(const nerf_amd_samples& s, int64_t m, bool want_dir) {
+DEVINL void ray_direction(const nerf_amd_samples& s, int64_t n, float& dx, float& dy, float& dz) {
+    if (s.mode == 1) {
+        const float* ry = s.rays + n * 6;
+        dx = ry[3]; dy = ry[4]; dz = ry[5];
+    } else {
+        const int row = (int)(n / s.W), col = (int)(n - (int64_t)row * s.W);
+        const float cx = (((float)col - (float)s.W * 0.5f) + 0.5f) / s.fx;
+        const float cy = (((float)s.H * 0.5f - (float)row) + 0.5f) / s.fy;
+        dx = (cx * s.pose[0] + cy * s.pose[1]) + (-1.0f) * s.pose[2];
+        dy = (cx * s.pose[4] + cy * s.pose[5]) + (-1.0f) * s.pose[6];
+        dz = (cx * s.pose[8] + cy * s.pose[9]) + (-1.0f) * s.pose[10];
+    }
+}
+DEVINL Sample fetch_sample(const nerf_amd_samples& s, int64_t m, bool want_dir, int64_t* ray = nullptr) {
     Sample r;
+    if (ray) *ray = 0;
     if (s.mode == 0) {
         const float* p = s.pts + m * s.pts_stride;
         r.x = p[0]; r.y = p[1]; r.z = p[2];
@@ -154,17 +168,13 @@
     }
     int64_t n; int si;
     split_sample_index(s, m, n, si);
+    if (ray) *ray = n;
     float ox, oy, oz;
+    ray_direction(s, n, r.dx, r.dy, r.dz);
     if (s.mode == 1) {
         const float* ry = s.rays + n * 6;
-        ox = ry[0]; oy = ry[1]; oz = ry[2]; r.dx = ry[3]; r.dy = ry[4]; r.dz = ry[5];
+        ox = ry[0]; oy = ry[1]; oz = ry[2];
     } else {
-        const int row = (int)(n / s.W), col = (int)(n - (int64_t)row * s.W);
-        const float cx = (((float)col - (float)s.W * 0.5f) + 0.5f) / s.fx;
-        const float cy = (((float)s.H * 0.5f - (float)row) + 0.5f) / s.fy;
-        r.dx = (cx * s.pose[0] + cy * s.pose[1]) + (-1.0f) * s.pose[2];
-        r.dy = (cx * s.pose[4] + cy * s.pose[5]) + (-1.0f) * s.pose[6];
-        r.dz = (cx * s.pose[8] + cy * s.pose[9]) + (-1.0f) * s.pose[10];
         ox = s.pose[3]; oy = s.pose[7]; oz = s.pose[11];
     }
     float zv;
@@ -204,6 +214,23 @@
 template <class P> constexpr uint32_t lds_dir() { return LDS_STASH + P::NW * P::NT * 4 * P::BREG_LDS; }
 template <class P> constexpr uint32_t lds_tile() { return lds_dir<P>() + P::NW * P::NT * 1024; }
 template <class P> constexpr uint32_t lds_total() { return lds_tile<P>() + P::NW * P::NT * 32 * 32 + P::NW * P::NT * 8 + 64; }
+
+template <class P> constexpr uint32_t lds_dir2() { return lds_total<P>(); }
+template <class P> constexpr uint32_t lds_total_dirtab() { return lds_total<P>() + P::NW * P::NT * 1024; }
+constexpr int DIR_TABLE_RAY_BYTES = 64;
+static_assert(lds_total_dirtab<PBF16W>() <= 160 * 1024, "LDS of the DIRTAB fine kernel");
+
+#ifdef MLP_CLOCKPROBE
+__device__ unsigned long long mlp_probe_phase[8];
+DEVINL uint64_t probe_now() {
+    uint64_t t;
+    asm volatile("s_memtime %0\n\ts_waitcnt lgkmcnt(0)" : "=s"(t) : : "memory");
+    return t;
+}
+#define MLP_PROBE(var) const uint64_t var = probe_now()
+#else
+#define MLP_PROBE(var)
+#endif
 
 DEVINL void load_biases(const void* packed, size_t stream_bytes, int n_bias, uint32_t lds_off = MLP_RING_BYTES) {
     const float* b = reinterpret_cast<const float*>(reinterpret_cast<const char*>(packed) + stream_bytes);
@@ -435,12 +462,32 @@
     float near, far;
 };
 
-template <class P, bool TRAIN, bool IPE = false, bool F8 = false, bool FUSED = false>
+template <class P>
+__global__ __launch_bounds__(256) void mip_dir_table_kernel(nerf_amd_samples s, int64_t n_rays, char* __restrict__ table) {
+    static_assert(sizeof(typename P::BReg) == 16 && DIR_TABLE_RAY_BYTES == 4 * 16, "bf16 B register groups");
+    const int64_t n = (int64_t)blockIdx.x * 256 + threadIdx.x;
+    if (n >= n_rays) return;
+    float dx, dy, dz;
+    ray_direction(s, n, dx, dy, dz);
+    const float nrm = norm3(dx, dy, dz);
+    const float x = dx / nrm, y = dy / nrm, z = dz / nrm;
+#pragma unroll
+    for (int h = 0; h < 2; ++h) {
+        typename P::BReg g[2];
+        encode<P, 4, 2>(x, y, z, h, g);
+        *reinterpret_cast<typename P::BReg*>(table + n * DIR_TABLE_RAY_BYTES + h * 32) = g[0];
+        *reinterpret_cast<typename P::BReg*>(table + n * DIR_TABLE_RAY_BYTES + h * 32 + 16) = g[1];
+    }
+}
+
+template <class P, bool TRAIN, bool IPE = false, bool F8 = false, bool FUSED = false, bool DIRTAB = false>
 __global__ __launch_bounds__(P::NW * 64) void mip_kernel(const void* __restrict__ packed, nerf_amd_samples s,
-                                                         float* __restrict__ rgbo, FusedComposite fc, ActDump dump) {
+                                                         float* __restrict__ rgbo, FusedComposite fc, ActDump dump,
+                                                         const char* __restrict__ dir_table) {
     using L = MipLayout;
     using BReg = typename P::BReg;
     constexpr int FPC = P::FPC;
+    static_assert(!DIRTAB || (P::NT == 2 && P::FAST_PE && !TRAIN && !IPE && !FUSED), "the direction table feeds the paired bf16 inference prologue");
 #ifdef MLP_CLOCKPROBE
     const uint64_t probe_c0 = __builtin_readcyclecounter(), probe_r0 = __builtin_amdgcn_s_memrealtime();
 #endif
@@ -461,8 +508,14 @@
     const uint32_t dir_lds0 = lds_dir<P>() + wave * NT * 1024 + lane * 16;
     auto enc_lds = [&](int t) -> uint32_t { return enc_lds0 + t * 4 * P::BREG_LDS; };
     auto dir_lds = [&](int t) -> uint32_t { return dir_lds0 + t * 1024; };
+    const uint32_t dir2_lds0 = lds_dir2<P>() + wave * NT * 1024 + lane * 16;
+    auto dir2_lds = [&](int t) -> uint32_t { return dir2_lds0 + t * 1024; };
+#ifdef MLP_CLOCKPROBE
+    uint64_t probe_acc[5] = {0, 0, 0, 0, 0};
+#endif
 
     for (int64_t tile = blockIdx.x; tile < n_tiles; tile += gridDim.x) {
+        MLP_PROBE(probe_t0);
         int64_t m[NT];
         BReg a[NT][16], b[NT][16];
         int lay = 0, lay_pend = 0;
@@ -486,13 +539,28 @@
                 m[0] = tile * TS + (wave * NT) * 32 + j;
                 m[1] = m[0] + 32;
                 const int64_t mo = h ? m[1] : m[0];
-                const Sample sm = fetch_sample(s, mo < s.M ? mo : s.M - 1, true);
+                const int64_t moc = mo < s.M ? mo : s.M - 1;
+                BReg dtab[NT][2];
+                int64_t n = 0;
+                const Sample sm = fetch_sample(s, moc, true, DIRTAB ? &n : nullptr);
+                if constexpr (DIRTAB) {
+                    uint32_t nl[2] = {(uint32_t)n, (uint32_t)n}, nh[2] = {(uint32_t)((uint64_t)n >> 32), (uint32_t)((uint64_t)n >> 32)};
+                    half_swap(nl[0], nl[1]); half_swap(nh[0], nh[1]);
+#pragma unroll
+                    for (int t = 0; t < NT; ++t) {
+                        const char* e = dir_table + (((uint64_t)nh[t] << 32) | nl[t]) * DIR_TABLE_RAY_BYTES + h * 32;
+                        dtab[t][0] = *reinterpret_cast<const BReg*>(e);
+                        dtab[t][1] = *reinterpret_cast<const BReg*>(e + 16);
+                    }
+                }
                 encode_pair<P, 10, 4>(sm.x, sm.y, sm.z, enc[0], enc[1]);
                 half_swap_groups<4>(enc[0], enc[1]);
                 uint32_t d0[3] = {__builtin_bit_cast(uint32_t, sm.dx), __builtin_bit_cast(uint32_t, sm.dy), __builtin_bit_cast(uint32_t, sm.dz)};
                 uint32_t d1[3] = {d0[0], d0[1], d0[2]};
-#pragma unroll
-                for (int c = 0; c < 3; ++c) half_swap(d0[c], d1[c]);
+                if constexpr (!DIRTAB) {
+#pragma unroll
+                    for (int c = 0; c < 3; ++c) half_swap(d0[c], d1[c]);
+                }
 #pragma unroll
                 for (int t = 0; t < NT; ++t) {
 #pragma unroll
@@ -501,9 +569,14 @@
 #pragma unroll
                         for (int k = 0; k < 4; ++k) dump_breg<P>(dump, 8, sub0 + t, k, lane, enc[t][k]);
                     }
-                    const uint32_t* dd = t ? d1 : d0;
-                    const f32x4 dv = {__builtin_bit_cast(float, dd[0]), __builtin_bit_cast(float, dd[1]), __builtin_bit_cast(float, dd[2]), 0.0f};
-                    *reinterpret_cast<f32x4*>(smem + dir_lds(t)) = dv;
+                    if constexpr (DIRTAB) {
+                        P::stash(dir_lds(t), dtab[t][0]);
+                        P::stash(dir2_lds(t), dtab[t][1]);
+                    } else {
+                        const uint32_t* dd = t ? d1 : d0;
+                        const f32x4 dv = {__builtin_bit_cast(float, dd[0]), __builtin_bit_cast(float, dd[1]), __builtin_bit_cast(float, dd[2]), 0.0f};
+                        *reinterpret_cast<f32x4*>(smem + dir_lds(t)) = dv;
+                    }
                 }
             } else {
 #pragma unroll
@@ -538,6 +611,10 @@
                 *reinterpret_cast<f32x4*>(smem + dir_lds(t)) = dv;
             }
             }
+            MLP_PROBE(probe_t1);
+#ifdef MLP_CLOCKPROBE
+            probe_acc[0] += probe_t1 - probe_t0;
+#endif
             d = dense<P, 4, 8, L::START[0]>(ws, bias0 + L::BIAS_OFF[0] * 4,
                 [&](int kg, int t) -> BReg { return enc[t][kg]; }, OA, NoPrev{});
         }
@@ -564,17 +641,29 @@
         auto OSIG = [&](int, int t, const f32x16& acc, int half) { if (half == 0) sigma[t] = acc[0]; };
         const auto dsig = dense<P, 16, 1, L::START[7]>(ws, bias0 + L::BIAS_OFF[7] * 4, IN_A, OSIG, prev_of(d, OA_pend));
         if constexpr (TRAIN) mask_flush<P, F8>(dump, macc, 6, sub0, lane, sacc);
+        MLP_PROBE(probe_t2);
         BReg denc[NT][2];
 #pragma unroll
         for (int t = 0; t < NT; ++t) {
-            const f32x4 dv = *reinterpret_cast<const f32x4*>(smem + dir_lds(t));
-            const float nrm = norm3(dv[0], dv[1], dv[2]);
-            encode<P, 4, 2>(dv[0] / nrm, dv[1] / nrm, dv[2] / nrm, h, denc[t]);
+            if constexpr (DIRTAB) {
+                denc[t][0] = P::unstash(dir_lds(t));
+                denc[t][1] = P::unstash(dir2_lds(t));
+            } else {
+                const f32x4 dv = *reinterpret_cast<const f32x4*>(smem + dir_lds(t));
+                const float nrm = norm3(dv[0], dv[1], dv[2]);
+                encode<P, 4, 2>(dv[0] / nrm, dv[1] / nrm, dv[2] / nrm, h, denc[t]);
+            }
             if constexpr (TRAIN) {
                 dump_breg<P>(dump, 8, sub0 + t, 4, lane, denc[t][0]);
                 dump_breg<P>(dump, 8, sub0 + t, 5, lane, denc[t][1]);
             }
         }
+#ifdef MLP_CLOCKPROBE
+#pragma unroll
+        for (int t = 0; t < NT; ++t) { WeightStream<P, MLP_NSLOT>::dummy_sink(denc[t][0]); WeightStream<P, MLP_NSLOT>::dummy_sink(denc[t][1]); }
+        MLP_PROBE(probe_t3);
+        probe_acc[1] += probe_t3 - probe_t2;
+#endif
         BReg c[NT][8];
         auto OC = [&](int fb, int t, const f32x16& acc, int half) {
             c[t][2 * fb + half] = to_breg_half<P, true>(acc, half);
@@ -591,6 +680,11 @@
         dense<P, 8, 1, L::START[9]>(ws, bias0 + L::BIAS_OFF[9] * 4,
             [&](int kg, int t) -> BReg { return c[t][kg]; }, ORGB, prev_of(dc, OC)).flush(ORGB);
         if constexpr (TRAIN) mask_flush<P, F8>(dump, macc, 7, sub0, lane, sacc);
+#ifdef MLP_CLOCKPROBE
+#pragma unroll
+        for (int t = 0; t < NT; ++t) asm volatile("" ::"v"(r[t]), "v"(g[t]), "v"(bl[t]));
+#endif
+        MLP_PROBE(probe_t4);
         f32x4 o[NT];
 #pragma unroll
         for (int t = 0; t < NT; ++t) {
@@ -602,6 +696,10 @@
                 if (h == 0 && m[t] < s.M) *reinterpret_cast<f32x4*>(rgbo + m[t] * 4) = o[t];
             }
         }
+#ifdef MLP_CLOCKPROBE
+        MLP_PROBE(probe_t5);
+        probe_acc[2] += probe_t5 - probe_t4; probe_acc[3] += probe_t5 - probe_t0; probe_acc[4] += 1;
+#endif
         if constexpr (FUSED) {
             const int S = s.S;
             const int spr = S >> 5;
@@ -694,6 +792,12 @@
         reinterpret_cast<uint64_t*>(rgbo)[0] = __builtin_readcyclecounter() - probe_c0;
         reinterpret_cast<uint64_t*>(rgbo)[1] = __builtin_amdgcn_s_memrealtime() - probe_r0;
     }
+    if (blockIdx.x == 0 && threadIdx.x == 0) {
+#pragma unroll
+        for (int i = 0; i < 5; ++i) mlp_probe_phase[i] = probe_acc[i];
+        mlp_probe_phase[5] = __builtin_readcyclecounter() - probe_c0;
+        mlp_probe_phase[6] = __builtin_amdgcn_s_memrealtime() - probe_r0;
+    }
 #endif
 }
 
@@ -1076,17 +1180,18 @@
 
 int allow_dynamic_lds(const void* fn, size_t lds) { return nerf_host::allow_dynamic_lds(fn, lds); }
 
-template <class P, class Lay, bool TRAIN = false, bool F8 = false, class K, class... Extra>
+template <class P, class Lay, bool TRAIN = false, bool F8 = false, bool DIRTAB = false, class K, class... Extra>
 int launch(K kernel, const void* packed, const nerf_amd_samples& s, float* out, hipStream_t st, Extra... extra) {
     constexpr int TS = P::NW * P::NT * 32;
     const int64_t n_tiles = (s.M + TS - 1) / TS;
     if (n_tiles == 0) return 0;
-    const size_t lds = F8 ? lds_total_train_f8<P>() : (TRAIN ? lds_total_train<P>() : lds_total<P>());
+    const size_t lds = DIRTAB ? lds_total_dirtab<P>() : (F8 ? lds_total_train_f8<P>() : (TRAIN ? lds_total_train<P>() : lds_total<P>()));
     if (int e = allow_dynamic_lds(reinterpret_cast<const void*>(kernel), lds)) return e;
     hipLaunchKernelGGL(kernel, dim3(grid_for(n_tiles)), dim3(P::NW * 64), lds, st, packed, s, out, extra...);
     return (int)hipGetLastError();
 }
 const ActDump NO_DUMP{nullptr, 0ull, nullptr, 0ull};
+[[maybe_unused]] const char* const NO_TABLE = nullptr;
 
 using PB16 = PBF16W;
 
@@ -1105,12 +1210,33 @@
 int mlp_launch_mip(const void* packed, int precision, const nerf_amd_samples& s, float* rgbo, hipStream_t st) {
     const FusedComposite off{nullptr, nullptr, nullptr, 0, 0.0f, 1.0f};
     if (s.ipe) {
-        if (precision == NERF_AMD_BF16) return launch<PB16, MipLayout>(mip_kernel<PB16, false, true>, packed, s, rgbo, st, off, NO_DUMP);
-        return launch<PF32, MipLayout>(mip_kernel<PF32, false, true>, packed, s, rgbo, st, off, NO_DUMP);
-    }
-    if (precision == NERF_AMD_BF16) return launch<PB16, MipLayout>(mip_kernel<PB16, false>, packed, s, rgbo, st, off, NO_DUMP);
-    return launch<PF32, MipLayout>(mip_kernel<PF32, false>, packed, s, rgbo, st, off, NO_DUMP);
-}
+        if (precision == NERF_AMD_BF16) return launch<PB16, MipLayout>(mip_kernel<PB16, false, true>, packed, s, rgbo, st, off, NO_DUMP, NO_TABLE);
+        return launch<PF32, MipLayout>(mip_kernel<PF32, false, true>, packed, s, rgbo, st, off, NO_DUMP, NO_TABLE);
+    }
+    if (precision == NERF_AMD_BF16) return launch<PB16, MipLayout>(mip_kernel<PB16, false>, packed, s, rgbo, st, off, NO_DUMP, NO_TABLE);
+    return launch<PF32, MipLayout>(mip_kernel<PF32, false>, packed, s, rgbo, st, off, NO_DUMP, NO_TABLE);
+}
+size_t mlp_mip_dir_table_bytes(int64_t n_rays) { return n_rays > 0 ? (size_t)n_rays * DIR_TABLE_RAY_BYTES : 0; }
+int mlp_launch_mip_dir_table(const nerf_amd_samples& s, void* table, hipStream_t st) {
+    const int64_t n_rays = (s.M + s.S - 1) / s.S;
+    if (n_rays == 0) return 0;
+    hipLaunchKernelGGL(mip_dir_table_kernel<PB16>, dim3((unsigned)((n_rays + 255) / 256)), dim3(256), 0, st, s, n_rays, reinterpret_cast<char*>(table));
+    return (int)hipGetLastError();
+}
+int mlp_launch_mip_dirtab(const void* packed, const nerf_amd_samples& s, float* rgbo, void* table, hipStream_t st) {
+    const FusedComposite off{nullptr, nullptr, nullptr, 0, 0.0f, 1.0f};
+#ifdef MLP_NO_DIRTAB
+    return launch<PB16, MipLayout>(mip_kernel<PB16, false>, packed, s, rgbo, st, off, NO_DUMP, NO_TABLE);
+#endif
+    if (int e = mlp_launch_mip_dir_table(s, table, st)) return e;
+    return launch<PB16, MipLayout, false, false, true>(mip_kernel<PB16, false, false, false, false, true>, packed, s, rgbo, st, off, NO_DUMP,
+                                                       reinterpret_cast<const char*>(table));
+}
+#ifdef MLP_CLOCKPROBE
+extern "C" int nerf_amd_clockprobe_read(unsigned long long* out8) {
+    return (int)hipMemcpyFromSymbol(out8, HIP_SYMBOL(mlp_probe_phase), 8 * sizeof(unsigned long long));
+}
+#endif
 int mlp_launch_mip128(const void* packed, int precision, const nerf_amd_samples& s, float* rgbo, hipStream_t st) {
     if (precision == NERF_AMD_BF16) return launch<PB16, MipLayout128>(mip128_kernel<PB16>, packed, s, rgbo, st);
     return launch<PF32, MipLayout128>(mip128_kernel<PF32>, packed, s, rgbo, st);
@@ -1118,8 +1244,8 @@
 int mlp_launch_mip_composite(const void* packed, int precision, const nerf_amd_samples& s, float* rgb, float* depth, float* weights,
                              int white_bkg, float near, float far, hipStream_t st) {
     const FusedComposite fc{rgb, depth, weights, white_bkg, near, far};
-    if (precision == NERF_AMD_BF16) return launch<PB16, MipLayout>(mip_kernel<PB16, false, false, false, true>, packed, s, (float*)nullptr, st, fc, NO_DUMP);
-    return launch<PF32, MipLayout>(mip_kernel<PF32, false, false, false, true>, packed, s, (float*)nullptr, st, fc, NO_DUMP);
+    if (precision == NERF_AMD_BF16) return launch<PB16, MipLayout>(mip_kernel<PB16, false, false, false, true>, packed, s, (float*)nullptr, st, fc, NO_DUMP, NO_TABLE);
+    return launch<PF32, MipLayout>(mip_kernel<PF32, false, false, false, true>, packed, s, (float*)nullptr, st, fc, NO_DUMP, NO_TABLE);
 }
 #endif
 #if MLP_TU == 0 || MLP_TU == 1
@@ -1169,16 +1295,16 @@
     const FusedComposite off{nullptr, nullptr, nullptr, 0, 0.0f, 1.0f};
     if (precision == NERF_AMD_BF16_F8) {
         const ActDump d8 = make_dump(dump, NERF_AMD_BF16, s.M, MIP_DUMP_SLOTS);
-        if (s.ipe) return launch<PB16, MipLayout, true, true>(mip_kernel<PB16, true, true, true>, packed, s, rgbo, st, off, d8);
-        return launch<PB16, MipLayout, true, true>(mip_kernel<PB16, true, false, true>, packed, s, rgbo, st, off, d8);
+        if (s.ipe) return launch<PB16, MipLayout, true, true>(mip_kernel<PB16, true, true, true>, packed, s, rgbo, st, off, d8, NO_TABLE);
+        return launch<PB16, MipLayout, true, true>(mip_kernel<PB16, true, false, true>, packed, s, rgbo, st, off, d8, NO_TABLE);
     }
     const ActDump d = make_dump(dump, precision, s.M, MIP_DUMP_SLOTS);
     if (s.ipe) {
-        if (precision == NERF_AMD_BF16) return launch<PB16, MipLayout, true>(mip_kernel<PB16, true, true>, packed, s, rgbo, st, off, d);
-        return launch<PF32, MipLayout, true>(mip_kernel<PF32, true, true>, packed, s, rgbo, st, off, d);
-    }
-    if (precision == NERF_AMD_BF16) return launch<PB16, MipLayout, true>(mip_kernel<PB16, true>, packed, s, rgbo, st, off, d);
-    return launch<PF32, MipLayout, true>(mip_kernel<PF32, true>, packed, s, rgbo, st, off, d);
+        if (precision == NERF_AMD_BF16) return launch<PB16, MipLayout, true>(mip_kernel<PB16, true, true>, packed, s, rgbo, st, off, d, NO_TABLE);
+        return launch<PF32, MipLayout, true>(mip_kernel<PF32, true, true>, packed, s, rgbo, st, off, d, NO_TABLE);
+    }
+    if (precision == NERF_AMD_BF16) return launch<PB16, MipLayout, true>(mip_kernel<PB16, true>, packed, s, rgbo, st, off, d, NO_TABLE);
+    return launch<PF32, MipLayout, true>(mip_kernel<PF32, true>, packed, s, rgbo, st, off, d, NO_TABLE);
 }
 
 #endif
diff --git a/nerf_amd/ops.py b/nerf_amd/ops.py
--- a/nerf_amd/ops.py
+++ b/nerf_amd/ops.py
@@ -216,9 +216,22 @@
     return out
 
 
-def mip_forward_samples(packed, precision, s: Samples, shape, device) -> torch.Tensor:
+def mip_forward_samples(packed, precision, s: Samples, shape, device, dir_table: bool = True) -> torch.Tensor:
     out = torch.empty(tuple(shape) + (4,), dtype=torch.float32, device=device)
+    if dir_table and s.mode != 0 and s.M > 0:
+        need = lib.nerf_amd_mip_forward_workspace_bytes((s.M + s.S - 1) // s.S)
+        ws = scratch("mip_dir_table", need, device)
+        check(lib.nerf_amd_mip_forward_ws(_ptr(packed), _prop_prec(None, precision, packed), C.byref(s), _ptr(out), _ptr(ws), need, _stream()),
+              "nerf_amd_mip_forward_ws")
+        return out
     check(lib.nerf_amd_mip_forward(_ptr(packed), _prop_prec(None, precision, packed), C.byref(s), _ptr(out), _stream()), "nerf_amd_mip_forward")
+    return out
+
+
+def mip_dir_table(s: Samples, device) -> torch.Tensor:
+    n = (s.M + s.S - 1) // s.S
+    out = torch.empty((n, 2, 16), dtype=torch.bfloat16, device=device)
+    check(lib.nerf_amd_mip_dir_table(C.byref(s), _ptr(out), _stream()), "nerf_amd_mip_dir_table")
     return out
 
 
```

After: 9.284 million, median of 6. No clear change (+1.0%).
